# wischmcj/pyQSM

Measured on AMD Instinct MI355X. Metric: Mpoints/s DBSCAN (1M-pt synthetic forest, eps=0.1, min_neighbors=10), higher is better.
Workload: dtype f64; 1 GPU; 1000000-point synthetic tree cloud (configs[1]), DBSCAN eps=0.1 min_neighbors=10, 20 clusters; replicas at N>1; points_per_gpu=1000000, parallelism=replicas x1

## Files before the change

### include/pyqsm_hip.h

```cpp
#ifndef PYQSM_HIP_H
#define PYQSM_HIP_H

#include <stddef.h>
#include <stdint.h>

#ifdef __cplusplus
extern "C" {
#endif

#define PYQSM_OK 0
#define PYQSM_EINVAL (-1)
#define PYQSM_EHIP (-2)
#define PYQSM_ENODEV (-3)
#define PYQSM_ERANGE (-4)
#define PYQSM_ENOMEM (-5)
#define PYQSM_ENOCONV (-6)

#define PYQSM_MISS_PRIM 0xFFFFFFFFu


int pyqsm_device_count(void);
int pyqsm_init(int device);
int pyqsm_shutdown(void);
const char* pyqsm_last_error(void);
const char* pyqsm_version(void);
int pyqsm_sync(int device);
void* pyqsm_stream(int device);

int pyqsm_dev_malloc(int device, size_t bytes, void** out);
int pyqsm_dev_free(int device, void* p);
int pyqsm_h2d(int device, void* dst_dev, const void* src_host, size_t bytes);
int pyqsm_d2h(int device, void* dst_host, const void* src_dev, size_t bytes);
void pyqsm_free(void* p);
void* pyqsm_host_alloc(size_t bytes);

int pyqsm_prof_enable(int device, int on);
int pyqsm_prof_reset(int device);
int pyqsm_prof_get(int device, const char* name, double* total_ms, int64_t* launches);

int pyqsm_cast_rays(const float* verts, int64_t V, const int32_t* tris, int64_t T,
                    const float* rays, int64_t R,
                    float* t_hit, uint32_t* prim_id, float* uv, int32_t device);

int pyqsm_expand_tris_dev(const float* verts_dev, int64_t V, const int32_t* tris_dev,
                          int64_t T, float* tri12_dev, int32_t device);
int pyqsm_cast_rays_dev(const float* tri12_dev, int64_t T, const float* rays_dev, int64_t R,
                        float* t_hit_dev, uint32_t* prim_id_dev, float* uv_dev,
                        int32_t device);

int pyqsm_list_intersections(const float* verts, int64_t V, const int32_t* tris, int64_t T,
                             const float* rays, int64_t R, int32_t* counts,
                             uint32_t* ray_ids, uint32_t* prim_ids, float* t, float* uv,
                             int64_t hits_cap, int64_t* n_hits, int32_t device);

int pyqsm_point_mesh_distance(const float* verts, int64_t V, const int32_t* tris, int64_t T,
                              const float* qry, int64_t Q, float* dist, uint32_t* prim,
                              int32_t device);

int pyqsm_cast_rays_multi(const float* verts, int64_t V, const int32_t* tris, int64_t T,
                          const float* rays, int64_t R,
                          float* t_hit, uint32_t* prim_id, float* uv, int32_t n_devices);

int pyqsm_shard_bounds(int64_t n, int32_t world, int32_t rank, int64_t* begin, int64_t* end);

#define PYQSM_COMM_ID_BYTES 128
int pyqsm_comm_unique_id(uint8_t* id);
int pyqsm_comm_init_rank(const uint8_t* id, int32_t world, int32_t rank, int32_t device);
int pyqsm_comm_finalize(void);
int pyqsm_comm_info(int32_t* world, int32_t* rank, int32_t* device);
int pyqsm_comm_broadcast_dev(void* buf_dev, int64_t bytes, int32_t root);
int pyqsm_comm_all_gather_dev(const void* send_dev, void* recv_dev, int64_t bytes_per_rank);
int pyqsm_comm_all_reduce_max(double* value);

int pyqsm_dbscan(const double* xyz, int64_t n, double eps, int32_t min_pts,
                 int64_t* labels, uint8_t* is_core, int32_t device);
int pyqsm_dbscan_dev(const double* xyz_dev, int64_t n, double eps, int32_t min_pts,
                     int64_t* labels_dev, uint8_t* is_core_dev, int64_t* n_clusters,
                     int32_t device);
int pyqsm_dbscan_ex(const double* xyz, int64_t n, double eps, int32_t min_pts,
                    int32_t radius_inclusive, int64_t* labels, uint8_t* is_core, int32_t device);
int pyqsm_dbscan_dev_ex(const double* xyz_dev, int64_t n, double eps, int32_t min_pts,
                        int32_t radius_inclusive, int64_t* labels_dev, uint8_t* is_core_dev,
                        int64_t* n_clusters, int32_t device);

int pyqsm_knn(const double* xyz, int64_t n, int32_t k, int32_t exclude_self,
              int32_t* idx, double* d2, int32_t device);
int pyqsm_knn_dev(const double* xyz_dev, int64_t n, int32_t k, int32_t exclude_self,
                  int32_t* idx_dev, double* d2_dev, int32_t device);

int pyqsm_ransac(const double* pts, int64_t n, const int64_t* triples, int64_t H,
                 int32_t shape, double thresh, double center[3], double axis[3],
                 double* radius, int64_t* inliers, int64_t* n_inliers, int64_t* best,
                 int32_t device);
int pyqsm_ransac_models(const double* pts, int64_t n, const int64_t* triples, int64_t H,
                        double* models, int32_t device);
int pyqsm_ransac_count(const double* pts, int64_t n, const double* models, int64_t H,
                       int32_t shape, double thresh, int32_t* counts, int32_t device);
int pyqsm_ransac_batch(const double* pts, int64_t n, const int64_t* seg_start, int64_t n_seg,
                       const int64_t* triples, int64_t H, int32_t shape, double thresh,
                       double* centers, double* axes, double* radii, int64_t* inliers,
                       int64_t* n_inliers, int64_t* best, int32_t device);

int pyqsm_lbc_solve(const int32_t* indptr, const int32_t* indices, const double* vals,
                    int64_t n, const double* wl, const double* wh, const double* pts,
                    double rtol, int32_t max_it, double* out, int32_t* iters,
                    double* resid, int32_t device);
int pyqsm_spmv3(const int32_t* indptr, const int32_t* indices, const double* vals,
                int64_t n, const double* x, double* y, int32_t device);
int pyqsm_clamp(double* pts, int64_t n, const double lo[3], const double hi[3],
                int32_t device);

int pyqsm_ball_query(const double* xyz, int64_t n, const double center[3], double radius,
                     int64_t* out_idx, int64_t* count, int32_t device);
int pyqsm_radius_mark(const double* src, int64_t n, const double* qry, int64_t m, double radius,
                      int32_t k_cap, uint8_t* mark, int32_t* counts, int32_t device);
int pyqsm_radius_knn(const double* src, int64_t n, const double* qry, int64_t m, double radius,
                     int32_t k, int64_t* idx, double* dist, int32_t device);
int pyqsm_radius_reduce(const double* src, int64_t n, const double* qry, int64_t m, double radius, int32_t k,
                        const double* values, int32_t F, int32_t reducer, int64_t empty_row, double* out,
                        int32_t* counts, int32_t device);
int pyqsm_radius_label(const double* src, int64_t n, const double* qry, int64_t m,
                       const int32_t* qry_label, double radius, int32_t k_cap, int32_t* label,
                       int32_t* counts, int32_t device);
int pyqsm_grow_clusters(const double* src, int64_t n, const int32_t* owner_in, const double* seed_xyz,
                        const int32_t* seed_label, int64_t m, int32_t n_clusters, double radius,
                        int32_t k_cap, int32_t cycles, int32_t min_new, int32_t* owner_out,
                        int32_t* cycle_out, int32_t* finished, int64_t* stats, int32_t device);

#define PYQSM_ADJ_SAME_CLOUD 1
#define PYQSM_ADJ_WITNESS 2
#define PYQSM_ADJ_NO_CACHE 4
int pyqsm_cluster_adjacency(const double* src, const int32_t* src_label, int64_t n, int32_t n_src_labels,
                            const double* tgt, const int32_t* tgt_label, int64_t m, int32_t n_tgt_labels,
                            double threshold, int32_t flags, int64_t capacity, int32_t* a, int32_t* b,
                            double* min_d2, int64_t* pairs, int64_t* src_idx, int64_t* tgt_idx, int64_t* count,
                            int64_t* stats, int32_t device);

#define PYQSM_ALPHA_BOUNDARY 1
#define PYQSM_ALPHA_DEFAULT_MAX_TESTS 4000000000000LL
int pyqsm_alpha_area(const int32_t* ij, int64_t n, const int64_t* seg_start, int64_t n_seg, uint64_t a2,
                     int64_t max_tests, int32_t flags, int64_t* twice_area, int64_t* n_live, int64_t* n_boundary,
                     int64_t** edges, int64_t* stats, int32_t device);

int pyqsm_fps(const double* xyz, int64_t n, int64_t num_samples, int64_t start_index,
              int32_t* out_idx, int32_t device);

int pyqsm_pc_laplacian(const double* xyz, int64_t n, int32_t k, double moll,
                       int64_t* nnz, int32_t** indptr, int32_t** indices, double** vals,
                       double* mass, int32_t device);
int pyqsm_pc_laplacian_seg(const double* xyz, int64_t n, const int64_t* seg_start, int64_t n_seg,
                           int32_t k, double moll, int64_t* nnz, int32_t** indptr,
                           int32_t** indices, double** vals, double* mass, int32_t device);

int pyqsm_extract_skeleton(const double* xyz, int64_t n, const int64_t* seg_start, int64_t n_seg,
                           int32_t k, double moll, int32_t max_iter, double termination_ratio,
                           double contraction_factor, double attraction_factor,
                           double max_contraction, double max_attraction, const double* lo,
                           const double* hi, double rtol, int32_t solver_max_it, double* out_pts,
                           double* total_shift, double* steps, int32_t* n_steps,
                           int32_t* solve_iters, double* solve_resid, uint8_t* solve_ok,
                           int32_t* n_solves, int32_t device);

int pyqsm_extreme_points(const double* xyz, int64_t n, const double* dirs, int32_t n_dirs,
                         int64_t* idx, int32_t device);
int pyqsm_outside_halfspaces(const double* xyz, int64_t n, const double* eq, int32_t n_planes,
                             double margin, int64_t* idx, int64_t* count, int32_t device);

int pyqsm_mean_f64(const double* v, int64_t n, double* out);

int pyqsm_voxel_down_sample(const double* xyz, int64_t n, const double* colors, double voxel_size,
                            int64_t* m, double** out_xyz, double** out_colors, int64_t* inverse,
                            int64_t* offsets, int64_t* members, int32_t device);
int pyqsm_stat_outlier(const double* xyz, int64_t n, int32_t nb_neighbors, double std_ratio,
                       int64_t* keep, int64_t* n_keep, double* avg, double* stats, int32_t device);
int pyqsm_clean_cloud(const double* xyz, int64_t n, double voxel_size, double neighbors, double ratio,
                      int32_t iters, int64_t* m, double** out_xyz, int32_t device);

int pyqsm_estimate_normals(const double* xyz, int64_t n, double radius, int32_t max_nn,
                           const double* prev_normals, double* normals, int32_t device);
int pyqsm_orient_normals_tangent_plane(const double* xyz, int64_t n, const double* normals, int32_t k,
                                       double* oriented, int32_t* rounds, int32_t device);
int pyqsm_stem_cloud(const double* xyz, int64_t n, const double* prev_normals, double crop_offset,
                     double radius, int32_t max_nn, int32_t orient_k, double angle_cutoff,
                     int64_t* keep, double* normals, int64_t* m, int32_t device);

#define PYQSM_KMEANS_MAX_K 8
#define PYQSM_KMEANS_MAX_Q 4
#define PYQSM_SILHOUETTE_MAX_K 65536
int pyqsm_kmeans(const double* xyz, int64_t m, int32_t k, int32_t iters, const double* init,
                 double* centroids, int32_t* labels, int32_t device);
int pyqsm_silhouette(const double* xyz, int64_t m, const int32_t* labels, int32_t k, double* score,
                     int32_t* n_present, double* samples, int32_t device);
int pyqsm_kmeans_select(const double* xyz, int64_t m, int32_t k0, int32_t nk, int32_t iters,
                        const double* init, int32_t* labels, double* scores, int32_t* present,
                        int32_t device);
int pyqsm_kmeans_select_dev(const double* xyz_dev, int64_t m, int32_t k0, int32_t nk, int32_t iters,
                            const double* init, int32_t* labels, double* scores, int32_t* present,
                            int32_t device);
int pyqsm_ball_excl_dev(const double* xyz_dev, int64_t n, const uint8_t* found_dev, const double center[3],
                        double radius, int64_t* idx_dev, double* out_xyz_dev, int64_t* count,
                        int32_t device);
int pyqsm_mark_found_dev(uint8_t* found_dev, int64_t n, const int64_t* idx, int64_t cnt, int32_t device);

int pyqsm_geometric_features(const double* xyz, int64_t n, double radius, int32_t max_k, int32_t metric,
                             const int32_t* feature_ids, int32_t n_features, double* out, int32_t* counts,
                             int32_t device);
int pyqsm_smooth_values(const double* xyz, int64_t n, const double* qry, int64_t m, const double* values,
                        int32_t F, int32_t k, int32_t reducer, double* out, int32_t* idx, int32_t device);

#define PYQSM_FOREST_MAX_FEATURES 64
#define PYQSM_FOREST_MAX_CLASSES 32
#define PYQSM_FOREST_MAX_TREE_NODES 4194304u
int pyqsm_forest_create(const int64_t* tree_offsets, const int32_t* left, const int32_t* right,
                        const int32_t* feature, const double* threshold, const uint8_t* missing_left,
                        const double* value, int32_t T, int32_t C, int32_t F, int32_t device, void** forest);
int pyqsm_forest_free(void* forest);
int pyqsm_forest_info(const void* forest, int64_t info[8]);
int pyqsm_forest_stage(void* forest, int32_t staged_nodes);
int pyqsm_forest_predict(const void* forest, const float* X, int64_t n, double* proba, int32_t* label,
                         int32_t* leaves);

#define PYQSM_VOX_INVERT 1
int pyqsm_voxel_grid_create(const double* xyz, int64_t n, const double* colors, double voxel_size,
                            int32_t device, void** grid);
int pyqsm_voxel_grid_free(void* grid);
int pyqsm_voxel_grid_info(const void* grid, double origin[3], double* voxel_size, int64_t dims[3],
                          int64_t* n_voxels, int64_t* device_bytes);
int pyqsm_voxel_grid_voxels(const void* grid, int32_t* grid_index, double* colors);
int pyqsm_voxel_grid_query(const void* grid, const double* qry, int64_t m, int32_t flags,
                           uint8_t* included, int32_t* row, int64_t* idx, int64_t* count);
int pyqsm_voxel_grid_query_dev(const void* grid, const double* qry_dev, int64_t m, int32_t flags,
                               uint8_t* included_dev, int32_t* row_dev, int64_t* idx_dev, int64_t* count);

int pyqsm_skeletal_forest(const double* xyz, int64_t m, int32_t k, int32_t* edges, double* d2, int64_t* n_edges,
                          int32_t* rounds, int32_t device);
int pyqsm_skeletal_forest_dev(const double* xyz_dev, int64_t m, int32_t k, int32_t* edges_dev, double* d2_dev,
// ... 17 lines not shown
```

### pyqsm_amd/_lib.py

```python
from __future__ import annotations

import ctypes
import os

_HERE = os.path.dirname(os.path.abspath(__file__))
LIB_PATH = os.path.join(_HERE, "libpyqsm_hip.so")

i64, i32, u32, dbl = ctypes.c_int64, ctypes.c_int32, ctypes.c_uint32, ctypes.c_double
vp = ctypes.c_void_p

SIGNATURES = {
    "pyqsm_device_count": (ctypes.c_int, []),
    "pyqsm_init": (ctypes.c_int, [ctypes.c_int]),
    "pyqsm_shutdown": (ctypes.c_int, []),
    "pyqsm_last_error": (ctypes.c_char_p, []),
    "pyqsm_version": (ctypes.c_char_p, []),
    "pyqsm_sync": (ctypes.c_int, [ctypes.c_int]),
    "pyqsm_stream": (vp, [ctypes.c_int]),
    "pyqsm_dev_malloc": (ctypes.c_int, [ctypes.c_int, ctypes.c_size_t, ctypes.POINTER(vp)]),
    "pyqsm_dev_free": (ctypes.c_int, [ctypes.c_int, vp]),
    "pyqsm_h2d": (ctypes.c_int, [ctypes.c_int, vp, vp, ctypes.c_size_t]),
    "pyqsm_d2h": (ctypes.c_int, [ctypes.c_int, vp, vp, ctypes.c_size_t]),
    "pyqsm_free": (None, [vp]),
    "pyqsm_host_alloc": (vp, [ctypes.c_size_t]),
    "pyqsm_prof_enable": (ctypes.c_int, [ctypes.c_int, ctypes.c_int]),
    "pyqsm_prof_reset": (ctypes.c_int, [ctypes.c_int]),
    "pyqsm_prof_get": (ctypes.c_int, [ctypes.c_int, ctypes.c_char_p, ctypes.POINTER(dbl),
                                      ctypes.POINTER(i64)]),
    "pyqsm_cast_rays": (ctypes.c_int, [vp, i64, vp, i64, vp, i64, vp, vp, vp, i32]),
    "pyqsm_expand_tris_dev": (ctypes.c_int, [vp, i64, vp, i64, vp, i32]),
    "pyqsm_cast_rays_dev": (ctypes.c_int, [vp, i64, vp, i64, vp, vp, vp, i32]),
    "pyqsm_list_intersections": (ctypes.c_int, [vp, i64, vp, i64, vp, i64, vp, vp, vp, vp, vp,
                                                i64, ctypes.POINTER(i64), i32]),
    "pyqsm_point_mesh_distance": (ctypes.c_int, [vp, i64, vp, i64, vp, i64, vp, vp, i32]),
    "pyqsm_cast_rays_multi": (ctypes.c_int, [vp, i64, vp, i64, vp, i64, vp, vp, vp, i32]),
    "pyqsm_shard_bounds": (ctypes.c_int, [i64, i32, i32, ctypes.POINTER(i64), ctypes.POINTER(i64)]),
    "pyqsm_comm_unique_id": (ctypes.c_int, [vp]),
    "pyqsm_comm_init_rank": (ctypes.c_int, [vp, i32, i32, i32]),
    "pyqsm_comm_finalize": (ctypes.c_int, []),
    "pyqsm_comm_info": (ctypes.c_int, [ctypes.POINTER(i32), ctypes.POINTER(i32),
                                       ctypes.POINTER(i32)]),
    "pyqsm_comm_broadcast_dev": (ctypes.c_int, [vp, i64, i32]),
    "pyqsm_comm_all_gather_dev": (ctypes.c_int, [vp, vp, i64]),
    "pyqsm_comm_all_reduce_max": (ctypes.c_int, [ctypes.POINTER(dbl)]),
    "pyqsm_dbscan": (ctypes.c_int, [vp, i64, dbl, i32, vp, vp, i32]),
    "pyqsm_dbscan_dev": (ctypes.c_int, [vp, i64, dbl, i32, vp, vp, ctypes.POINTER(i64), i32]),
    "pyqsm_dbscan_ex": (ctypes.c_int, [vp, i64, dbl, i32, i32, vp, vp, i32]),
    "pyqsm_dbscan_dev_ex": (ctypes.c_int, [vp, i64, dbl, i32, i32, vp, vp, ctypes.POINTER(i64), i32]),
    "pyqsm_knn": (ctypes.c_int, [vp, i64, i32, i32, vp, vp, i32]),
    "pyqsm_knn_dev": (ctypes.c_int, [vp, i64, i32, i32, vp, vp, i32]),
    "pyqsm_ransac": (ctypes.c_int, [vp, i64, vp, i64, i32, dbl, vp, vp, ctypes.POINTER(dbl), vp,
                                    ctypes.POINTER(i64), ctypes.POINTER(i64), i32]),
    "pyqsm_ransac_models": (ctypes.c_int, [vp, i64, vp, i64, vp, i32]),
    "pyqsm_ransac_count": (ctypes.c_int, [vp, i64, vp, i64, i32, dbl, vp, i32]),
    "pyqsm_ransac_batch": (ctypes.c_int, [vp, i64, vp, i64, vp, i64, i32, dbl, vp, vp, vp, vp, vp, vp, i32]),
    "pyqsm_lbc_solve": (ctypes.c_int, [vp, vp, vp, i64, vp, vp, vp, dbl, i32, vp,
                                       ctypes.POINTER(i32), vp, i32]),
    "pyqsm_spmv3": (ctypes.c_int, [vp, vp, vp, i64, vp, vp, i32]),
    "pyqsm_clamp": (ctypes.c_int, [vp, i64, vp, vp, i32]),
    "pyqsm_ball_query": (ctypes.c_int, [vp, i64, vp, dbl, vp, ctypes.POINTER(i64), i32]),
    "pyqsm_radius_mark": (ctypes.c_int, [vp, i64, vp, i64, dbl, i32, vp, vp, i32]),
    "pyqsm_radius_label": (ctypes.c_int, [vp, i64, vp, i64, vp, dbl, i32, vp, vp, i32]),
    "pyqsm_grow_clusters": (ctypes.c_int, [vp, i64, vp, vp, vp, i64, i32, dbl, i32, i32, i32, vp, vp, vp, vp,
                                           i32]),
    "pyqsm_radius_knn": (ctypes.c_int, [vp, i64, vp, i64, dbl, i32, vp, vp, i32]),
    "pyqsm_cluster_adjacency": (ctypes.c_int, [vp, vp, i64, i32, vp, vp, i64, i32, dbl, i32, i64, vp, vp, vp, vp,
                                               vp, vp, ctypes.POINTER(i64), vp, i32]),
    "pyqsm_alpha_area": (ctypes.c_int, [vp, i64, vp, i64, ctypes.c_uint64, i64, i32, vp, vp, vp,
                                        ctypes.POINTER(vp), vp, i32]),
    "pyqsm_fps": (ctypes.c_int, [vp, i64, i64, i64, vp, i32]),
    "pyqsm_pc_laplacian": (ctypes.c_int, [vp, i64, i32, dbl, ctypes.POINTER(i64),
                                          ctypes.POINTER(vp), ctypes.POINTER(vp),
                                          ctypes.POINTER(vp), vp, i32]),
    "pyqsm_extract_skeleton": (ctypes.c_int, [vp, i64, vp, i64, i32, dbl, i32, dbl, dbl, dbl, dbl, dbl, vp, vp,
                                              dbl, i32, vp, vp, vp, vp, vp, vp, vp, ctypes.POINTER(i32), i32]),
    "pyqsm_pc_laplacian_seg": (ctypes.c_int, [vp, i64, vp, i64, i32, dbl, ctypes.POINTER(i64),
                                              ctypes.POINTER(vp), ctypes.POINTER(vp),
                                              ctypes.POINTER(vp), vp, i32]),
    "pyqsm_voxel_down_sample": (ctypes.c_int, [vp, i64, vp, dbl, ctypes.POINTER(i64), ctypes.POINTER(vp),
                                               ctypes.POINTER(vp), vp, vp, vp, i32]),
    "pyqsm_stat_outlier": (ctypes.c_int, [vp, i64, i32, dbl, vp, ctypes.POINTER(i64), vp, vp, i32]),
    "pyqsm_clean_cloud": (ctypes.c_int, [vp, i64, dbl, dbl, dbl, i32, ctypes.POINTER(i64),
                                         ctypes.POINTER(vp), i32]),
    "pyqsm_estimate_normals": (ctypes.c_int, [vp, i64, dbl, i32, vp, vp, i32]),
    "pyqsm_orient_normals_tangent_plane": (ctypes.c_int, [vp, i64, vp, i32, vp, ctypes.POINTER(i32), i32]),
    "pyqsm_stem_cloud": (ctypes.c_int, [vp, i64, vp, dbl, dbl, i32, i32, dbl, vp, vp, ctypes.POINTER(i64),
                                        i32]),
    "pyqsm_mean_f64": (ctypes.c_int, [vp, i64, ctypes.POINTER(dbl)]),
    "pyqsm_extreme_points": (ctypes.c_int, [vp, i64, vp, i32, vp, i32]),
    "pyqsm_outside_halfspaces": (ctypes.c_int, [vp, i64, vp, i32, dbl, vp, ctypes.POINTER(i64), i32]),
    "pyqsm_kmeans": (ctypes.c_int, [vp, i64, i32, i32, vp, vp, vp, i32]),
    "pyqsm_silhouette": (ctypes.c_int, [vp, i64, vp, i32, ctypes.POINTER(dbl), ctypes.POINTER(i32), vp, i32]),
    "pyqsm_kmeans_select": (ctypes.c_int, [vp, i64, i32, i32, i32, vp, vp, vp, vp, i32]),
    "pyqsm_kmeans_select_dev": (ctypes.c_int, [vp, i64, i32, i32, i32, vp, vp, vp, vp, i32]),
    "pyqsm_ball_excl_dev": (ctypes.c_int, [vp, i64, vp, vp, dbl, vp, vp, ctypes.POINTER(i64), i32]),
    "pyqsm_mark_found_dev": (ctypes.c_int, [vp, i64, vp, i64, i32]),
    "pyqsm_geometric_features": (ctypes.c_int, [vp, i64, dbl, i32, i32, vp, i32, vp, vp, i32]),
    "pyqsm_smooth_values": (ctypes.c_int, [vp, i64, vp, i64, vp, i32, i32, i32, vp, vp, i32]),
    "pyqsm_forest_create": (ctypes.c_int, [vp, vp, vp, vp, vp, vp, vp, i32, i32, i32, i32, ctypes.POINTER(vp)]),
    "pyqsm_forest_free": (ctypes.c_int, [vp]),
    "pyqsm_forest_info": (ctypes.c_int, [vp, vp]),
    "pyqsm_forest_stage": (ctypes.c_int, [vp, i32]),
    "pyqsm_forest_predict": (ctypes.c_int, [vp, vp, i64, vp, vp, vp]),
    "pyqsm_radius_reduce": (ctypes.c_int, [vp, i64, vp, i64, dbl, i32, vp, i32, i32, i64, vp, vp, i32]),
    "pyqsm_voxel_grid_create": (ctypes.c_int, [vp, i64, vp, dbl, i32, ctypes.POINTER(vp)]),
    "pyqsm_voxel_grid_free": (ctypes.c_int, [vp]),
    "pyqsm_voxel_grid_info": (ctypes.c_int, [vp, vp, ctypes.POINTER(dbl), vp, ctypes.POINTER(i64),
                                             ctypes.POINTER(i64)]),
    "pyqsm_voxel_grid_voxels": (ctypes.c_int, [vp, vp, vp]),
    "pyqsm_voxel_grid_query": (ctypes.c_int, [vp, vp, i64, i32, vp, vp, vp, ctypes.POINTER(i64)]),
    "pyqsm_voxel_grid_query_dev": (ctypes.c_int, [vp, vp, i64, i32, vp, vp, vp, ctypes.POINTER(i64)]),
    "pyqsm_skeletal_forest": (ctypes.c_int, [vp, i64, i32, vp, vp, ctypes.POINTER(i64), ctypes.POINTER(i32), i32]),
    "pyqsm_skeletal_forest_dev": (ctypes.c_int, [vp, i64, i32, vp, vp, ctypes.POINTER(i64), ctypes.POINTER(i32),
                                                 i32]),
    "pyqsm_collapse_chains": (ctypes.c_int, [vp, i64, i64, vp, vp, vp, vp, vp, i32]),
    "pyqsm_collapse_chains_dev": (ctypes.c_int, [vp, i64, i64, vp, vp, vp, vp, vp, i32]),
    "pyqsm_chain_radii": (ctypes.c_int, [vp, i64, vp, i64, vp, vp, i64, vp, i32]),
    "pyqsm_cylinder_surfaces": (ctypes.c_int, [vp, i64, vp, vp, ctypes.POINTER(vp), ctypes.POINTER(i64), i32]),
}

_lib = None


class PyQSMHipError(RuntimeError):

    def __init__(self, code: int, message: str):
        super().__init__(f"libpyqsm_hip error {code}: {message}")
        self.code = code


def load() -> ctypes.CDLL:
    global _lib
    if _lib is not None:
        return _lib
    if not os.path.exists(LIB_PATH):
        raise ImportError(
            f"{LIB_PATH} not found: the HIP library has not been built and there is no CPU "
            "fallback. Build it with `make -C pyqsm_amd/csrc`.")
    lib = ctypes.CDLL(LIB_PATH)
    for name, (res, args) in SIGNATURES.items():
        fn = getattr(lib, name)
        fn.restype = res
        fn.argtypes = args
    _lib = lib
    return lib


def check(code: int) -> None:
    if code != 0:
        msg = load().pyqsm_last_error()
        raise PyQSMHipError(code, msg.decode("utf-8", "replace") if msg else "")


def device_count() -> int:
    return int(load().pyqsm_device_count())


def logical_device_count() -> int:
    fake = os.environ.get("PYQSM_MULTI_FAKE_RANKS", "")
    return int(fake) if fake.isdigit() and int(fake) > 0 else device_count()


def physical_device(logical: int) -> int:
    fake = os.environ.get("PYQSM_MULTI_FAKE_RANKS", "")
    if fake.isdigit() and int(fake) > 0:
        return int(logical) % max(1, device_count())
    return int(logical)


def require_gpu(device: int = 0) -> None:
    check(load().pyqsm_init(int(device)))
```

### pyqsm_amd/csrc/dbscan.hip

```cpp
#include "grid.hpp"

#include <atomic>
#include <chrono>
#include <optional>
#include <vector>

namespace pyqsm {

static constexpr int kNoRoot = 0x7FFFFFFF;

__device__ __forceinline__ double sqdist(double ax, double ay, double az, double bx, double by,
                                         double bz) {
  double t0 = ax - bx, t1 = ay - by, t2 = az - bz;
  double d = t0 * t0;
  d = d + t1 * t1;
  d = d + t2 * t2;
  return d;
}


#define FOR_STENCIL(c, st, start, q, body)                         \
  for (int dz__ = -1; dz__ <= 1; ++dz__)                           \
    for (int dy__ = -1; dy__ <= 1; ++dy__) {                       \
      const int row__ = (c) + dy__ * (st).nx + dz__ * (st).nxy;    \
      const int qb__ = (start)[row__ - 1], qe__ = (start)[row__ + 2]; \
      for (int q = qb__; q < qe__; ++q) {                          \
        body                                                       \
      }                                                            \
    }

struct TileLds {
  double x[4][64], y[4][64], z[4][64];
};

static constexpr int kStragglers = 6;
static constexpr int kMaxChunks = 3;
static constexpr int kRestSegs = 64;
__device__ constexpr int kRunOrder[9] = {4, 3, 5, 1, 7, 0, 2, 6, 8};

template <class CO>
__global__ __launch_bounds__(256) void k_core_tiled(int n, const GridPlan* __restrict__ plan,
                                                    const int32_t* __restrict__ start,
                                                    const int32_t* __restrict__ cell_of, CO co, double r2,
                                                    int min_pts, uint8_t* __restrict__ core,
                                                    int32_t* __restrict__ rest,
                                                    int32_t* __restrict__ rest_cnt , int seg_cap,
                                                    int* __restrict__ parent, int* __restrict__ min_orig,
                                                    int32_t* __restrict__ flag , int max_chunks,
                                                    unsigned long long* __restrict__ tests ,
    unsigned long long* __restrict__ st ) {
  __shared__ TileLds L;
  stamped(st, [&] {
  const int lane = threadIdx.x & 63, w = __builtin_amdgcn_readfirstlane(threadIdx.x >> 6);
  const int p0 = (blockIdx.x * 4 + w) * 64;
  if (p0 >= n || !plan->ok) return;
  const Stencil st = plan_stencil(plan);
  const int ncell = plan->ncell;
  const int p = p0 + lane;
  const bool live = p < n;
  double x = 0.0, y = 0.0, z = 0.0;
  if (live) co.get(p, x, y, z);
  const Tile t = wave_tile(p0, n, st, ncell, start, cell_of);
  int cnt = 0;
  bool deferred = false;
  int chunks = 0;
  int staged = 0;
  if (t.total > kTileMax) {
    const int mycell = live ? cell_of[p] : -1;
    unsigned long long todo = __ballot(live);
    while (todo) {
      const int lead = __ffsll(todo) - 1;
      const int c = __builtin_amdgcn_readlane(mycell, lead);
      const bool mine = mycell == c;
      todo &= ~__ballot(mine);
      for (int dz = -1; dz <= 1; ++dz)
        for (int dy = -1; dy <= 1; ++dy) {
          const int row = c + dy * st.nx + dz * st.nxy;
          const int qb = __builtin_amdgcn_readfirstlane(start[row - 1]);
          const int qe = __builtin_amdgcn_readfirstlane(start[row + 2]);
          for (int base = qb; base < qe; base += 64) {
            const int q = base + lane;
            const int m = qe - base < 64 ? qe - base : 64;
            if (q < qe) co.get(q, L.x[w][lane], L.y[w][lane], L.z[w][lane]);
            __builtin_amdgcn_wave_barrier();
            staged += m;
            if (mine)
              for (int j = 0; j < m; ++j)
                cnt += sqdist(x, y, z, L.x[w][j], L.y[w][j], L.z[w][j]) <= r2;
            __builtin_amdgcn_wave_barrier();
          }
        }
    }
  } else {
#pragma unroll
    for (int ri = 0; ri < 9; ++ri) {
      const int r = kRunOrder[ri];
      for (int base = t.qb[r]; base < t.qe[r] && !deferred; base += 64) {
        const int q = base + lane;
        const int m = t.qe[r] - base < 64 ? t.qe[r] - base : 64;
        if (q < t.qe[r]) co.get(q, L.x[w][lane], L.y[w][lane], L.z[w][lane]);
        __builtin_amdgcn_wave_barrier();
        staged += m;
#pragma unroll 4
        for (int j = 0; j < m; ++j)
          cnt += sqdist(x, y, z, L.x[w][j], L.y[w][j], L.z[w][j]) <= r2;
        __builtin_amdgcn_wave_barrier();
        const unsigned long long und = __ballot(live && cnt < min_pts);
        ++chunks;
        if ((__popcll(und) <= kStragglers || chunks >= max_chunks) &&
            !(ri == 8 && base + 64 >= t.qe[r])) {
          if (und != 0) {
            int slot = 0;
            const int lead = __ffsll(und) - 1;
            const int seg = blockIdx.x % kRestSegs;
            if (lane == lead) slot = atomicAdd(rest_cnt + seg, __popcll(und));
            slot = __shfl(slot, lead, 64);
            if (live && cnt < min_pts) {
              rest[size_t(seg) * seg_cap + slot + __popcll(und & ((1ull << lane) - 1ull))] = p;
              cnt = -1;
            }
          }
          deferred = true;
          break;
        }
      }
    }
  }
  if (live && cnt >= 0) {
    core[p] = cnt >= min_pts;
    co.mark_core(p, cnt >= min_pts);
  }
  if (live) {
    parent[p] = p;
    min_orig[p] = 0x7F7F7F7F;
    flag[p] = 0;
    if (p == n - 1) flag[n] = 0;
  }
  if (tests && lane == 0) atomicAdd(tests + (blockIdx.x & 255), static_cast<unsigned long long>(staged));
  });
}

struct Runs9 {
  int qb[9];
  int pre[10];
  __device__ __forceinline__ int at(int g) const {
    int q = qb[0] + g;
#pragma unroll
    for (int r = 1; r < 9; ++r) q = g >= pre[r] ? qb[r] + (g - pre[r]) : q;
    return q;
  }
};
__device__ __forceinline__ Runs9 stencil_runs(int c, Stencil st, const int32_t* __restrict__ start) {
  Runs9 t;
  int qe[9];
#pragma unroll
  for (int r = 0; r < 9; ++r) {
    const int row = c + (kRunOrder[r] % 3 - 1) * st.nx + (kRunOrder[r] / 3 - 1) * st.nxy;
    t.qb[r] = start[row - 1];
    qe[r] = start[row + 2];
  }
  t.pre[0] = 0;
#pragma unroll
  for (int r = 0; r < 9; ++r) {
    t.qb[r] = __builtin_amdgcn_readfirstlane(t.qb[r]);
    t.pre[r + 1] = t.pre[r] + (__builtin_amdgcn_readfirstlane(qe[r]) - t.qb[r]);
  }
  return t;
}

template <class CO>
__global__ __launch_bounds__(256) void k_core_rest(const int32_t* __restrict__ rest,
                                                   const int32_t* __restrict__ rest_cnt ,
                                                   int seg_cap, const GridPlan* __restrict__ plan,
                                                   const int32_t* __restrict__ start,
                                                   const int32_t* __restrict__ cell_of, CO co, double r2,
                                                   int min_pts, uint8_t* __restrict__ core,
    unsigned long long* __restrict__ st ) {
  stamped(st, [&] {
  if (!plan->ok) return;
  const Stencil st = plan_stencil(plan);
  const int lane = threadIdx.x & 63;
  const int mine = rest_cnt[lane];
  int incl = mine;
#pragma unroll
  for (int off = 1; off < 64; off <<= 1) {
    const int v = __shfl_up(incl, off, 64);
    if (lane >= off) incl += v;
  }
  const int m = __shfl(incl, 63, 64);
  for (int i = blockIdx.x * 4 + (threadIdx.x >> 6); i < m; i += gridDim.x * 4) {
    const int seg = __popcll(__ballot(incl <= i));
    const int before = __shfl(incl - mine, seg, 64);
    const int p = rest[size_t(seg) * seg_cap + (i - before)];
    double x, y, z;
    co.get(p, x, y, z);
    const int c = __builtin_amdgcn_readfirstlane(cell_of[p]);
    const Runs9 t = stencil_runs(c, st, start);
    int cnt = 0;
    for (int g0 = 0; g0 < t.pre[9] && cnt < min_pts; g0 += 64) {
      const int g = g0 + lane;
      const bool hit = g < t.pre[9] && co.d2(t.at(g), x, y, z) <= r2;
      cnt += __popcll(__ballot(hit));
    }
    if (lane == 0) {
      core[p] = cnt >= min_pts;
      co.mark_core(p, cnt >= min_pts);
    }
  }
  });
}


__device__ __forceinline__ int ld_parent(const int* parent, int i) {
  return __hip_atomic_load(parent + i, __ATOMIC_RELAXED, __HIP_MEMORY_SCOPE_AGENT);
}
__device__ __forceinline__ void st_parent(int* parent, int i, int v) {
  __hip_atomic_store(parent + i, v, __ATOMIC_RELAXED, __HIP_MEMORY_SCOPE_AGENT);
}

__device__ __forceinline__ unsigned link_prio(int x) { return unsigned(x) * 0x9E3779B1u; }

__device__ __forceinline__ int find_root(int* parent, int x) {
  int cur = ld_parent(parent, x);
  if (cur != x) {
    int prev = x, next;
    while (cur != (next = ld_parent(parent, cur))) {
      st_parent(parent, prev, next);
      prev = cur;
      cur = next;
    }
  }
  return cur;
}

__device__ __forceinline__ void unite(int* parent, int a, int b) {
  int ra = find_root(parent, a), rb = find_root(parent, b);
  while (ra != rb) {
    if (link_prio(ra) < link_prio(rb)) {
      int t = ra;
      ra = rb;
      rb = t;
    }
    const int old = atomicCAS(parent + ra, ra, rb);
    if (old == ra) break;
    ra = find_root(parent, old);
    rb = find_root(parent, rb);
  }
}


__global__ __launch_bounds__(1024) void k_sub_rep(int n, const int32_t* __restrict__ sub_of,
                                                 const uint8_t* __restrict__ core,
                                                 const int32_t* __restrict__ order,
                                                 int* __restrict__ parent,
                                                 const int32_t* __restrict__ cell_of,
                                                 int4* __restrict__ rec,
                                                 int* __restrict__ run_min,
                                                 int4* __restrict__ list,
                                                 int32_t* __restrict__ list_cnt, const GridPlan* __restrict__ plan,
                                                 int4* __restrict__ list_xyz,
    unsigned long long* __restrict__ st ) {
  stamped(st, [&] {
  if (!plan->ok) return;
  const int nx = plan->nx, ny = plan->ny;
  const int lane = threadIdx.x & 63, w = threadIdx.x >> 6;
  const int base = blockIdx.x * 1024 + w * 64;
  const int p = base + lane;
  const bool live = p < n;
  int sid = 0, s = n, e = n, ord = 0x7FFFFFFF, cell = 0;
  bool c = false;
  const bool c_prev = base >= 64 && p - 64 < n && core[p - 64];
  const bool c_next = p + 64 < n && core[p + 64];
  const int o_next = c_next ? order[p + 64] : 0x7FFFFFFF;
  if (live) {
    sid = sub_of[p];
    c = core[p];
    if (c) ord = order[p];
    cell = cell_of[p];
    const int2 run = *reinterpret_cast<const int2*>(rec + sid);
    s = run.x;
    e = run.x + run.y;
  }
  const unsigned long long cb = __ballot(c);
  int lead = -1;
  const int s0 = __shfl(s, 0, 64);
  if (s0 < base && s0 >= base - 64) {
    const unsigned long long f = __ballot(c_prev && base - 64 + lane >= s0);
    if (f) lead = base - 64 + __ffsll(f) - 1;
  } else {
    for (int q0 = s0; q0 < base; q0 += 64) {
      const int q = q0 + lane;
      const unsigned long long f = __ballot(q < base && core[q]);
      if (f) {
        lead = q0 + __ffsll(f) - 1;
        break;
      }
    }
  }
  int rep = -1;
  if (c) {
    if (s < base && lead >= 0) {
      rep = lead;
    } else {
      const int lo = s > base ? s - base : 0;
      rep = base + __ffsll(cb & (~0ull << lo)) - 1;
    }
    parent[p] = rep;
  }
  const bool is_rep = c && rep == p;
  int mn = ord;
  const int seg_end = e - base < 64 ? e - base : 64;
#pragma unroll
  for (int off = 1; off < 64; off <<= 1) {
    const int o = __shfl_down(mn, off, 64);
    if (lane + off < seg_end) mn = o < mn ? o : mn;
  }
  const unsigned long long tail = __ballot(is_rep && e > base + 64);
  if (tail) {
    const int t = __ffsll(tail) - 1;
    const int et = __shfl(e, t, 64);
    int m2 = base + 64 + lane < et ? o_next : 0x7FFFFFFF;
    for (int q = base + 128 + lane; q < et; q += 64)
      if (core[q]) m2 = min(m2, order[q]);
#pragma unroll
    for (int off = 32; off > 0; off >>= 1) {
      const int o = __shfl_xor(m2, off, 64);
      m2 = o < m2 ? o : m2;
    }
    if (lane == t) mn = min(mn, m2);
  }
  if (is_rep) {
    rec[sid].z = rep;
    run_min[rep] = mn;
  }
  __shared__ int wcount[16], wbase[16];
  const unsigned long long b = __ballot(is_rep);
  if (lane == 0) wcount[w] = __popcll(b);
  __syncthreads();
  if (threadIdx.x == 0) {
    int tot = 0;
    for (int k = 0; k < 16; ++k) tot += wcount[k];
    int base2 = tot ? atomicAdd(list_cnt, tot) : 0;
    for (int k = 0; k < 16; ++k) {
      wbase[k] = base2;
      base2 += wcount[k];
    }
  }
  __syncthreads();
  if (is_rep) {
    const int slot = wbase[w] + __popcll(b & ((1ull << lane) - 1ull));
    const int c1 = cell;
    list[slot] = make_int4(rep, c1, sid, e - rep);
    list_xyz[slot] = make_int4(c1 % nx, (c1 / nx) % ny, c1 / (nx * ny), sid & 7);
  }
  });
}

__constant__ signed char kSubOffsets[62][3] = {{1,0,0}, {-1,1,0}, {0,1,0}, {1,1,0}, {-1,-1,1}, {0,-1,1}, {1,-1,1}, {-1,0,1}, {0,0,1}, {1,0,1}, {-1,1,1}, {0,1,1}, {1,1,1}, {2,0,0}, {-2,1,0}, {2,1,0}, {-2,2,0}, {-1,2,0}, {0,2,0}, {1,2,0}, {2,2,0}, {-2,-2,1}, {-1,-2,1}, {0,-2,1}, {1,-2,1}, {2,-2,1}, {-2,-1,1}, {2,-1,1}, {-2,0,1}, {2,0,1}, {-2,1,1}, {2,1,1}, {-2,2,1}, {-1,2,1}, {0,2,1}, {1,2,1}, {2,2,1}, {-2,-2,2}, {-1,-2,2}, {0,-2,2}, {1,-2,2}, {2,-2,2}, {-2,-1,2}, {-1,-1,2}, {0,-1,2}, {1,-1,2}, {2,-1,2}, {-2,0,2}, {-1,0,2}, {0,0,2}, {1,0,2}, {2,0,2}, {-2,1,2}, {-1,1,2}, {0,1,2}, {1,1,2}, {2,1,2}, {-2,2,2}, {-1,2,2}, {0,2,2}, {1,2,2}, {2,2,2}};

__global__ __launch_bounds__(256) void k_flatten_reps(const int4* __restrict__ list,
                                                      const int32_t* __restrict__ m_ptr,
                                                      int* __restrict__ parent, int max_steps,
                                                      int4* __restrict__ rec ) {
  const int m = *m_ptr;
  int s = blockIdx.x * 256 + threadIdx.x;
  if (s >= m) return;
  const int4 me = list[s];
  const int p = me.x;
  int r = p, steps = 0;
  for (int nx = parent[r]; nx != r && steps < max_steps; nx = parent[r], ++steps) r = nx;
  parent[p] = r;
  if (rec) {
    int* const word = reinterpret_cast<int*>(rec + (me.z & ~7)) + 3;
    const int old = atomicCAS(word, 0, r + 1);
    if (old != 0 && old != r + 1 && old != -1) *word = -1;
  }
}

static constexpr int kSubPerWave = 4;

struct SubNbr {
  int q0, n2, rep;
};
__device__ __forceinline__ SubNbr sub_neighbour(bool active, const int4 at, int dx, int dy, int dz, int nx, int ny,
                                                const int32_t* __restrict__ start,
                                                const int4* __restrict__ rec) {
  const int gx = 2 * (at.x - 1) + (at.w & 1) - dx, gy = 2 * (at.y - 1) + ((at.w >> 1) & 1) - dy,
            gz = 2 * (at.z - 1) + ((at.w >> 2) & 1) - dz;
  const int c2 = (((gz >> 1) + 1) * ny + ((gy >> 1) + 1)) * nx + ((gx >> 1) + 1);
  const int oct = (gx & 1) | ((gy & 1) << 1) | ((gz & 1) << 2);
  SubNbr out{0, 0, -1};
  int b2 = 0, e2 = 0;
  if (active) {
    b2 = start[c2];
    e2 = start[c2 + 1];
  }
  if (e2 != b2) {
    const int4 r = rec[b2 * 8 + oct];
    if (r.y > 0) {
      out.q0 = r.x;
      out.n2 = r.y;
      out.rep = r.z;
    }
  }
  return out;
}

template <class CO>
__global__ __launch_bounds__(256) void k_hook_sub(const int4* __restrict__ list,
                                                  const int4* __restrict__ list_xyz,
                                                  const int32_t* __restrict__ m_ptr,
                                                  const GridPlan* __restrict__ plan, const int32_t* __restrict__ start,
                                                  const int4* __restrict__ rec, CO co, double r2,
                                                  const uint8_t* __restrict__ core,
                                                  int* __restrict__ parent,
    unsigned long long* __restrict__ st ) {
  stamped(st, [&] {
  if (!plan->ok) return;
  const int nx = plan->nx, ny = plan->ny;
  const int m = *m_ptr;
  const int k = threadIdx.x & 63;
  const int t = k & 15, grp = k >> 4;
  const int o_dx = t < 13 ? kSubOffsets[t][0] : 0, o_dy = t < 13 ? kSubOffsets[t][1] : 0,
            o_dz = t < 13 ? kSubOffsets[t][2] : 0;
  for (int s0 = (blockIdx.x * 4 + (threadIdx.x >> 6)) * kSubPerWave; s0 < m; s0 += gridDim.x * 4 * kSubPerWave) {
    const bool live = s0 + grp < m;
    const int4 me = list[min(s0 + grp, m - 1)], at = list_xyz[min(s0 + grp, m - 1)];
    const SubNbr nb2 = sub_neighbour(live && t < 13, at, o_dx, o_dy, o_dz, nx, ny, start, rec);
    const int p = me.x, n1 = me.w;
    unsigned todo = unsigned(__ballot(nb2.rep >= 0) >> (16 * grp)) & 0xFFFFu;
    int base = 0, hooked = -1;
    while (__ballot(todo != 0)) {
      const int src = (k & 48) + (todo ? __ffs(todo) - 1 : 0);
      const int qb = __shfl(nb2.q0, src, 64), nb = __shfl(nb2.n2, src, 64), rb = __shfl(nb2.rep, src, 64);
      const int sh = nb > 1 ? 32 - __clz(nb - 1) : 0;
      const int pairs = n1 << sh;
      const int idx = base + t;
      const int j = idx & ((1 << sh) - 1);
      bool hit = false;
      if (todo && idx < pairs && j < nb) hit = co.core_pair_within(p + (idx >> sh), qb + j, core, r2);
      const bool found = ((__ballot(hit) >> (16 * grp)) & 0xFFFFull) != 0;
      if (found) {
        hooked = rb;
        todo = 0;
      } else if (todo) {
        base += 16;
        if (base >= pairs) {
          todo &= todo - 1;
          base = 0;
        }
      }
    }
    if (hooked >= 0 && t == 0) parent[p] = parent[hooked];
  }
  });
}

template <class CO>
__device__ __forceinline__ bool wave_pair_within(const CO& co, int p, int n1, int qb, int nb, int k,
                                                 const uint8_t* __restrict__ core, double r2) {
  const int sh = nb > 1 ? 32 - __clz(nb - 1) : 0;
  const int pairs = n1 << sh;
  bool found = false;
  for (int base = 0; base < pairs && !found; base += 64) {
    const int idx = base + k;
    const int j = idx & ((1 << sh) - 1);
    bool hit = false;
    if (idx < pairs && j < nb) hit = co.core_pair_within(p + (idx >> sh), qb + j, core, r2);
    found = __ballot(hit) != 0;
  }
  return found;
}

template <class CO>
__device__ __forceinline__ void seam_unite(const int4 me, const int4 at, int k, int o_dx, int o_dy, int o_dz,
                                           int nx, int ny, const int32_t* __restrict__ start,
                                           const int4* __restrict__ rec, const CO& co, double r2,
                                           const uint8_t* __restrict__ core, int* parent) {
  const SubNbr nb2 = sub_neighbour(k < 62, at, o_dx, o_dy, o_dz, nx, ny, start, rec);
  const int p = me.x, n1 = me.w, rep2 = nb2.rep;
  const int* vparent = parent;
  int a1 = 0, a2 = 0;
  if (rep2 >= 0) {
    a1 = vparent[p];
    a2 = vparent[rep2];
  }
  bool need = rep2 >= 0 && !(a1 == a2 || a2 == p || a1 == rep2);
  int root2 = -1;
  if (need) {
    int ra = a1, rb = a2;
    for (;;) {
      const int pa = ld_parent(parent, ra), pb = ld_parent(parent, rb);
      if (pa == ra && pb == rb) break;
      ra = pa;
      rb = pb;
    }
    need = ra != rb;
    root2 = rb;
  }
  unsigned long long todo = __ballot(need);
  while (todo) {
    const int src = __ffsll(todo) - 1;
    todo &= todo - 1;
    const int qb = __shfl(nb2.q0, src, 64), nb = __shfl(nb2.n2, src, 64), rb = __shfl(rep2, src, 64);
    const int tree = __shfl(root2, src, 64);
    if (wave_pair_within(co, p, n1, qb, nb, k, core, r2)) {
      if (k == 0) unite(parent, p, rb);
      todo &= ~__ballot(root2 == tree);
    }
  }
}

template <class CO>
__global__ __launch_bounds__(256) void k_union_sub(const int4* __restrict__ list,
                                                   const int4* __restrict__ list_xyz,
                                                   const int32_t* __restrict__ m_ptr,
                                                   const GridPlan* __restrict__ plan, const int32_t* __restrict__ start,
                                                   const int4* __restrict__ rec, CO co, double r2,
                                                   const uint8_t* __restrict__ core, int* parent,
                                                   unsigned long long* __restrict__ seam_cnt ,
    unsigned long long* __restrict__ st ) {
  stamped(st, [&] {
  if (!plan->ok) return;
  const int nx = plan->nx, ny = plan->ny;
  const int m = *m_ptr;
  const int k = threadIdx.x & 63;
  const int t = k & 15, grp = k >> 4;
  const int o_dx = k < 62 ? kSubOffsets[k][0] : 0, o_dy = k < 62 ? kSubOffsets[k][1] : 0,
            o_dz = k < 62 ? kSubOffsets[k][2] : 0;
  const int c_off = t < 9 ? (t % 3 - 1) + (t / 3 - 1) * nx : 0;
  const int layer = nx * ny;
  for (int s0 = (blockIdx.x * 4 + (threadIdx.x >> 6)) * kSubPerWave; s0 < m; s0 += gridDim.x * 4 * kSubPerWave) {
    const bool live = s0 + grp < m;
    const int4 me = list[min(s0 + grp, m - 1)];
    const int* vparent = parent;
    const int r_s = vparent[me.x];
    const int c2 = me.y + c_off;
    int b2[2] = {0, 0}, e2[2] = {0, 0}, word[2] = {0, 0};
    if (live && t < 9) {
#pragma unroll
      for (int l = 0; l < 2; ++l) {
        b2[l] = start[c2 - l * layer];
        e2[l] = start[c2 - l * layer + 1];
      }
    }
#pragma unroll
    for (int l = 0; l < 2; ++l)
      if (e2[l] != b2[l]) word[l] = rec[b2[l] * 8].w;
    const unsigned long long seams =
        __ballot((word[0] != 0 && word[0] != r_s + 1) || (word[1] != 0 && word[1] != r_s + 1));
    if (!seams) continue;
    for (int u = 0; u < kSubPerWave; ++u) {
      if (!((seams >> (16 * u)) & 0xFFFFull)) continue;
      if (seam_cnt && k == 0) atomicAdd(seam_cnt, 1ull);
      seam_unite(list[s0 + u], list_xyz[s0 + u], k, o_dx, o_dy, o_dz, nx, ny, start, rec, co, r2, core, parent);
    }
  }
  });
}

template <class CO>
__global__ __launch_bounds__(256) void k_union_points(int n, Stencil st,
                                                      const int32_t* __restrict__ start,
                                                      const int32_t* __restrict__ cell_of, CO co, double r2,
                                                      const uint8_t* __restrict__ core, int* parent) {
  int p = blockIdx.x * 256 + threadIdx.x;
  if (p >= n || !core[p]) return;
  double x, y, z;
  co.get(p, x, y, z);
  const int c = cell_of[p];
  const volatile int* vparent = parent;
  int rp = find_root(parent, p);
  FOR_STENCIL(c, st, start, q, {
    if (q < p && core[q] && co.d2(q, x, y, z) <= r2) {
      if (vparent[q] != rp) {
        unite(parent, p, q);
        rp = find_root(parent, p);
      }
    }
  })
}

__global__ __launch_bounds__(256) void k_flatten(int n, const uint8_t* __restrict__ core,
                                                 int* __restrict__ parent, const GridPlan* __restrict__ plan) {
  int p = blockIdx.x * 256 + threadIdx.x;
  if (!plan->ok || p >= n || !core[p]) return;
  int r = p;
  for (int nx = parent[r]; nx != r; nx = parent[r]) r = nx;
  parent[p] = r;
}

template <int kThreads>
__device__ __forceinline__ void block_append(bool take, int value, int32_t* __restrict__ list,
                                             int32_t* __restrict__ cnt) {
  constexpr int kWaves = kThreads / 64;
  __shared__ int wcount[kWaves], wbase[kWaves];
  const unsigned long long b = __ballot(take);
  const int lane = threadIdx.x & 63, w = threadIdx.x >> 6;
  if (lane == 0) wcount[w] = __popcll(b);
  __syncthreads();
  if (threadIdx.x == 0) {
    int tot = 0;
    for (int k = 0; k < kWaves; ++k) tot += wcount[k];
    int base = tot ? atomicAdd(cnt, tot) : 0;
    for (int k = 0; k < kWaves; ++k) {
      wbase[k] = base;
      base += wcount[k];
    }
  }
  __syncthreads();
  if (take) list[wbase[w] + __popcll(b & ((1ull << lane) - 1ull))] = value;
}

static constexpr int kFlagsThreads = 256, kFlagsPer = 16, kFlagsPerBlock = kFlagsThreads * kFlagsPer;
__device__ __forceinline__ void flags_role(int b, int n, const uint8_t* __restrict__ core,
                                           int32_t* __restrict__ rest, int32_t* __restrict__ rest_cnt) {
  constexpr int kWaves = kFlagsThreads / 64;
  __shared__ int fcount[kWaves], fbase[kWaves];
  const int lane = threadIdx.x & 63, w = threadIdx.x >> 6;
  const int p0 = b * kFlagsPerBlock + threadIdx.x;
  unsigned take = 0;
#pragma unroll
  for (int k = 0; k < kFlagsPer; ++k) {
    const int p = p0 + k * kFlagsThreads;
    take |= unsigned(p < n && !core[p]) << k;
  }
  int mine = __popc(take);
#pragma unroll
  for (int off = 32; off > 0; off >>= 1) mine += __shfl_xor(mine, off, 64);
  if (lane == 0) fcount[w] = mine;
  __syncthreads();
  if (threadIdx.x == 0) {
    int tot = 0;
    for (int k = 0; k < kWaves; ++k) tot += fcount[k];
    int base = tot ? atomicAdd(rest_cnt, tot) : 0;
    for (int k = 0; k < kWaves; ++k) {
      fbase[k] = base;
      base += fcount[k];
    }
  }
  __syncthreads();
  int at = fbase[w];
#pragma unroll
  for (int k = 0; k < kFlagsPer; ++k) {
    const bool t = (take >> k) & 1u;
    const unsigned long long bal = __ballot(t);
    if (t) rest[at + __popcll(bal & ((1ull << lane) - 1ull))] = p0 + k * kFlagsThreads;
    at += __popcll(bal);
  }
}

__global__ __launch_bounds__(kFlagsThreads) void k_noncore_list(int n, const uint8_t* __restrict__ core,
                                                                int32_t* __restrict__ rest,
                                                                int32_t* __restrict__ rest_cnt,
                                                                const GridPlan* __restrict__ plan) {
  if (!plan->ok) return;
  flags_role(blockIdx.x, n, core, rest, rest_cnt);
}

__global__ __launch_bounds__(256) void k_point_min(int n, const uint8_t* __restrict__ core,
                                                   const int* __restrict__ parent,
                                                   const int32_t* __restrict__ order,
                                                   int* __restrict__ min_orig,
                                                   int32_t* __restrict__ roots,
                                                   int32_t* __restrict__ roots_cnt,
                                                   const GridPlan* __restrict__ plan) {
  int p = blockIdx.x * 256 + threadIdx.x;
  const bool is_c = plan->ok && p < n && core[p];
  if (is_c) atomicMin(min_orig + parent[p], order[p]);
  block_append<256>(is_c && parent[p] == p, p, roots, roots_cnt);
}

static constexpr int kRepRootThreads = kFlagsThreads;
static_assert(kRepRootThreads == 256, "gl, the grid of the representatives' blocks, is cut in 256s");
__global__ __launch_bounds__(kRepRootThreads) void k_rep_root(const int4* __restrict__ list,
                                                  const int32_t* __restrict__ m_ptr,
                                                  int* __restrict__ parent,
                                                  const int* __restrict__ run_min,
                                                  int* __restrict__ min_orig,
                                                  int32_t* __restrict__ roots,
                                                  int32_t* __restrict__ roots_cnt, int rep_blocks, int n,
                                                  const uint8_t* __restrict__ core, int32_t* __restrict__ rest,
                                                  int32_t* __restrict__ rest_cnt,
                                                  const GridPlan* __restrict__ plan) {
  if (int(blockIdx.x) >= rep_blocks) {
    if (plan->ok) flags_role(blockIdx.x - rep_blocks, n, core, rest, rest_cnt);
    return;
  }
  const int m = *m_ptr;
  int s = blockIdx.x * kRepRootThreads + threadIdx.x;
  const bool active = s < m;
  int p = -1, r = -1, v = 0x7FFFFFFF;
  if (active) {
    p = list[s].x;
    r = p;
    for (int nx = parent[r]; nx != r; nx = parent[r]) r = nx;
    if (r != p) parent[p] = r;
    v = run_min[p];
  }
  const volatile int* vmin = min_orig;
  const int lane = threadIdx.x & 63;
  unsigned long long rem = __ballot(active);
  while (rem) {
    const int lead = __ffsll(rem) - 1;
    const int r0 = __shfl(r, lead, 64);
    const bool mine = active && r == r0;
    int mn = mine ? v : 0x7FFFFFFF;
#pragma unroll
    for (int off = 32; off > 0; off >>= 1) {
      const int o = __shfl_xor(mn, off, 64);
      mn = o < mn ? o : mn;
    }
    if (lane == lead && mn < vmin[r0]) atomicMin(min_orig + r0, mn);
    rem &= ~__ballot(mine);
  }
  block_append<256>(active && r == p, p, roots, roots_cnt);
}

static constexpr int kRankCap = 4096;
static constexpr int kNumberThreads = 1024;

__global__ __launch_bounds__(kNumberThreads) void k_number(int n, const int32_t* __restrict__ roots,
                                                           const int32_t* __restrict__ roots_cnt,
                                                           int* __restrict__ min_orig,
                                                           uint32_t* __restrict__ bits ,
                                                           int32_t* __restrict__ wpre ,
                                                           int32_t* __restrict__ done ,
                                                           const GridPlan* __restrict__ plan,
    unsigned long long* __restrict__ st ) {
  stamped(st, [&] {
  if (!plan->ok) return;
  const int R = *roots_cnt;
  const int t = threadIdx.x;
  if (R <= kRankCap) {
    if (blockIdx.x != 0) return;
    __shared__ unsigned long long key[kRankCap];
    int P = 2;
    while (P < R) P <<= 1;
    for (int i = t; i < P; i += kNumberThreads) {
      unsigned long long k = ~0ull;
      if (i < R) {
        const int r = roots[i];
        k = (static_cast<unsigned long long>(min_orig[r]) << 32) | static_cast<uint32_t>(r);
      }
      key[i] = k;
    }
    __syncthreads();
    for (int k = 2; k <= P; k <<= 1)
      for (int j = k >> 1; j > 0; j >>= 1) {
        for (int i = t; i < P; i += kNumberThreads) {
          const int l = i ^ j;
          if (l > i) {
            const unsigned long long a = key[i], b = key[l];
            if ((a > b) == ((i & k) == 0)) {
              key[i] = b;
              key[l] = a;
            }
          }
        }
        __syncthreads();
      }
    for (int i = t; i < R; i += kNumberThreads) min_orig[static_cast<uint32_t>(key[i])] = i;
    return;
  }
  for (int i = blockIdx.x * kNumberThreads + t; i < R; i += gridDim.x * kNumberThreads) {
    const int v = min_orig[roots[i]];
    __hip_atomic_fetch_or(bits + (v >> 5), 1u << (v & 31), __ATOMIC_RELAXED, __HIP_MEMORY_SCOPE_AGENT);
  }
  __shared__ int last;
  __threadfence();
  __syncthreads();
  if (t == 0) last = atomicAdd(done, 1) == int(gridDim.x) - 1;
  __syncthreads();
  if (!last) return;
  __threadfence();
  __shared__ int wsum[kNumberThreads / 64];
  const int lane = t & 63, wv = t >> 6;
  const int nw = n / 32 + 1;
  int carry = 0;
  for (int w0 = 0; w0 < nw; w0 += 16 * kNumberThreads) {
    const int i0 = w0 + 16 * t;
    int cnt[16], sum = 0;
#pragma unroll
    for (int k = 0; k < 16; ++k) {
      cnt[k] = i0 + k < nw ? __popc(__hip_atomic_load(bits + i0 + k, __ATOMIC_RELAXED, __HIP_MEMORY_SCOPE_AGENT)) : 0;
      sum += cnt[k];
    }
    int incl = sum;
#pragma unroll
    for (int off = 1; off < 64; off <<= 1) {
      const int o = __shfl_up(incl, off, 64);
      if (lane >= off) incl += o;
    }
    if (lane == 63) wsum[wv] = incl;
    __syncthreads();
    int before = carry, total = 0;
    for (int k = 0; k < kNumberThreads / 64; ++k) {
      before += k < wv ? wsum[k] : 0;
      total += wsum[k];
    }
    int run = before + incl - sum;
#pragma unroll
    for (int k = 0; k < 16; ++k)
      if (i0 + k < nw) {
        wpre[i0 + k] = run;
        run += cnt[k];
      }
    carry += total;
    __syncthreads();
  }
  });
}

__device__ __forceinline__ int cluster_number(int v, int n_roots, const uint32_t* __restrict__ bits,
                                              const int32_t* __restrict__ wpre) {
  if (n_roots <= kRankCap) return v;
  return wpre[v >> 5] + __popc(bits[v >> 5] & ((1u << (v & 31)) - 1u));
}

static constexpr int kLabelThreads = 256;
template <class CO>
__global__ __launch_bounds__(kLabelThreads) void k_labels(int n, const int32_t* __restrict__ rest,
                                                          const int32_t* __restrict__ rest_cnt,
                                                          const GridPlan* __restrict__ plan,
                                                          const int32_t* __restrict__ start,
                                                          const int32_t* __restrict__ cell_of, CO co, double r2,
                                                          const uint8_t* __restrict__ core,
                                                          const int* __restrict__ parent,
                                                          const int* __restrict__ min_orig,
                                                          const int32_t* __restrict__ roots_cnt,
                                                          const uint32_t* __restrict__ bits,
                                                          const int32_t* __restrict__ wpre,
                                                          const int32_t* __restrict__ order,
                                                          int64_t* __restrict__ labels,
                                                          uint8_t* __restrict__ is_core,
    unsigned long long* __restrict__ st ) {
  stamped(st, [&] {
  if (!plan->ok) return;
  constexpr int kWaves = kLabelThreads / 64;
  const int n_roots = *roots_cnt;
  const int lane = threadIdx.x & 63;
  {
    const int p = blockIdx.x * kLabelThreads + threadIdx.x;
    const bool is_c = p < n && core[p];
    if (is_c) {
      const int v = min_orig[parent[parent[p]]];
      labels[order[p]] = int64_t(cluster_number(v, n_roots, bits, wpre));
    }
    if (p < n && is_core) is_core[order[p]] = is_c;
  }
  const int m = *rest_cnt;
  const Stencil sten = plan_stencil(plan);
  const int first = blockIdx.x * kWaves + __builtin_amdgcn_readfirstlane(threadIdx.x >> 6);
  for (int i = first; i < m; i += gridDim.x * kWaves) {
    const int p = rest[i];
    double x, y, z;
    co.get(p, x, y, z);
    const int c = __builtin_amdgcn_readfirstlane(cell_of[p]);
    const Runs9 t = stencil_runs(c, sten, start);
    int best = kNoRoot;
    for (int g0 = 0; g0 < t.pre[9]; g0 += 64) {
      const int g = g0 + lane;
      if (g < t.pre[9]) {
        const int q = t.at(g);
        if (core[q] && co.d2(q, x, y, z) <= r2) {
          const int mo = min_orig[parent[parent[q]]];
          best = mo < best ? mo : best;
        }
      }
    }
#pragma unroll
    for (int off = 32; off > 0; off >>= 1) {
      const int o = __shfl_xor(best, off, 64);
      best = o < best ? o : best;
    }
    if (lane == 0)
      labels[order[p]] = best == kNoRoot ? int64_t(-1) : int64_t(cluster_number(best, n_roots, bits, wpre));
  }
  });
}

static int cluster_binned(Ctx* c, int64_t n, double eps, int32_t min_pts, bool radius_inclusive, const DevGrid& g,
                          const SubCells& sub, const GridPlan* d_plan, int64_t* labels, uint8_t* is_core,
                          const int32_t** count_out) {
  const bool fine = g.cell <= eps * (1.0 + 1.0 / 524288.0);
  const int N = int(n);
  const dim3 grid(ceil_div(n, 256)), block(256);
  const Stencil st{g.nx, g.nx * g.ny};
  const double r2 = radius_inclusive ? eps * eps : nextafter(eps * eps, 0.0);
  uint8_t* core;
  int *parent, *min_orig;
  int32_t* flag;
  PQ_TRY(c->arena.get(size_t(n), &core));
  PQ_TRY(c->arena.get(size_t(n), &parent));
  PQ_TRY(c->arena.get(size_t(n), &min_orig));
  PQ_TRY(c->arena.get(size_t(n) + 1, &flag));
  uint32_t* const bits = reinterpret_cast<uint32_t*>(flag);
  int32_t *roots, *wpre;
  PQ_TRY(c->arena.get(size_t(n), &roots));
  PQ_TRY(c->arena.get(size_t(n / 32) + 1, &wpre));
  int4* list;
  int32_t* list_cnt;
  int* run_min;
  PQ_TRY(c->arena.get(size_t(n), &run_min));
  PQ_TRY(c->arena.get(size_t(n), &list));
  int4* list_xyz;
  PQ_TRY(c->arena.get(size_t(n), &list_xyz));
  list_cnt = sub.zeroed4;
  int32_t* const roots_cnt = list_cnt + 1;
  int32_t* rest;
  const int core_blocks = int(ceil_div(n, 256));
  const int seg_cap = ceil_div(core_blocks, kRestSegs) * 256;
  PQ_TRY(c->arena.get(std::max<size_t>(size_t(n), size_t(seg_cap) * kRestSegs), &rest));
  int32_t* const rest_segs = list_cnt + 4;
  {
    StampScope ps(c, "dbscan_core");
    unsigned long long* d_tests = nullptr;
    if (c->prof >= 2) {
      PQ_TRY(c->arena.get(256, &d_tests));
      PQ_HIP(hipMemsetAsync(d_tests, 0, 256 * 8, c->stream));
    }
    const int max_chunks = std::min(32, std::max(kMaxChunks, (kMaxChunks * min_pts + 9) / 10));
    {
      const StampKernel pk(c, "k_core_tiled", grid.x);
      on_coords(g, [&](auto co) {
        hipLaunchKernelGGL(k_core_tiled<decltype(co)>, grid, block, 0, c->stream, N, d_plan, g.start, g.cell_of, co, r2,
                           min_pts, core, rest, rest_segs, seg_cap, parent, min_orig, flag, max_chunks, d_tests,
                           pk.slots);
      });
    }
    if (d_tests) {
      unsigned long long h[256];
      PQ_HIP(hipMemcpyAsync(h, d_tests, sizeof(h), hipMemcpyDeviceToHost, c->stream));
      PQ_HIP(hipStreamSynchronize(c->stream));
      unsigned long long tot = 0;
      for (unsigned long long v : h) tot += v;
      c->timers["core_pair_tests"].launches += int64_t(tot) * 64;
    }
    const dim3 gr(std::min<int64_t>(8192, ceil_div(n, 64)));
    unsigned long long* const st_rest = stamp_slots(c, gr.x);
    on_coords(g, [&](auto co) {
      hipLaunchKernelGGL(k_core_rest<decltype(co)>, gr, block, 0, c->stream, rest, rest_segs, seg_cap, d_plan, g.start,
                         g.cell_of, co, r2, min_pts, core, st_rest);
    });
    PQ_HIP(hipGetLastError());
    if (getenv("PYQSM_DBSCAN_TRACE")) {
      int32_t h[kRestSegs];
      PQ_HIP(hipMemcpyAsync(h, rest_segs, sizeof(h), hipMemcpyDeviceToHost, c->stream));
      PQ_HIP(hipStreamSynchronize(c->stream));
      long long tot = 0;
      for (int32_t v : h) tot += v;
      fprintf(stderr, "core pass: %lld stragglers\n", tot);
    }
  }
  {
    StampScope ps(c, "dbscan_union");
    const dim3 gf(ceil_div(n, kFlagsPerBlock));
    if (fine) {
      hipLaunchKernelGGL(k_sub_rep, dim3(ceil_div(n, 1024)), dim3(1024), 0, c->stream, N, sub.sub_of, core,
                         g.order, parent, g.cell_of, sub.rec, run_min, list, list_cnt, d_plan, list_xyz,
                         stamp_slots(c, ceil_div(n, 1024)));
      {
        int per_cu[2] = {16, 32};
        if (const char* e_cu = getenv("PYQSM_UNION_BLOCKS_PER_CU")) {
          per_cu[0] = per_cu[1] = atoi(e_cu);
          if (const char* comma = strchr(e_cu, ',')) per_cu[1] = atoi(comma + 1);
        }
        const int64_t full = ceil_div(n, 4 * kSubPerWave);
        const dim3 gh(per_cu[0] > 0 ? std::min<int64_t>(full, int64_t(c->cu_count) * per_cu[0]) : full),
            gu(per_cu[1] > 0 ? std::min<int64_t>(full, int64_t(c->cu_count) * per_cu[1]) : full),
            gl(ceil_div(n, 256));
        const bool trace = getenv("PYQSM_DBSCAN_TRACE") != nullptr;
        {
          const StampKernel pk(c, "k_hook_sub", gh.x);
          on_coords(g, [&](auto co) {
            hipLaunchKernelGGL(k_hook_sub<decltype(co)>, gh, block, 0, c->stream, list, list_xyz, list_cnt, d_plan,
                               g.start, sub.rec, co, r2, core, parent, pk.slots);
          });
        }
        if (trace) {
          int32_t m = 0;
          PQ_HIP(hipMemcpyAsync(&m, list_cnt, 4, hipMemcpyDeviceToHost, c->stream));
          PQ_HIP(hipStreamSynchronize(c->stream));
          std::vector<int32_t> hp(static_cast<size_t>(n), 0);
          std::vector<int4> hl(static_cast<size_t>(m), make_int4(0, 0, 0, 0));
          PQ_HIP(hipMemcpy(hp.data(), parent, size_t(n) * 4, hipMemcpyDeviceToHost));
          PQ_HIP(hipMemcpy(hl.data(), list, size_t(m) * 16, hipMemcpyDeviceToHost));
          std::vector<int64_t> hist(66, 0);
          int64_t roots = 0;
          for (int32_t s2 = 0; s2 < m; ++s2) {
            int d = 0, r = hl[size_t(s2)].x;
            while (hp[size_t(r)] != r && d < 65) {
              r = hp[size_t(r)];
              ++d;
            }
            hist[size_t(d)]++;
            roots += d == 0;
          }
          fprintf(stderr, "hook pass: %d sub-cells, %lld roots; chain depth histogram:", m, (long long)roots);
          for (int d = 0; d < 66; ++d)
            if (hist[size_t(d)]) fprintf(stderr, " %d:%lld", d, (long long)hist[size_t(d)]);
          fprintf(stderr, "\n");
        }
        static const int jump = [] {
          const char* e = getenv("PYQSM_FLATTEN_JUMP");
          return e ? atoi(e) : 12;
        }();
        if (jump > 0)
          hipLaunchKernelGGL(k_flatten_reps, gl, block, 0, c->stream, list, list_cnt, parent, jump,
                             static_cast<int4*>(nullptr));
        hipLaunchKernelGGL(k_flatten_reps, gl, block, 0, c->stream, list, list_cnt, parent, 0x7fffffff, sub.rec);
        unsigned long long* d_seams = nullptr;
        if (trace) {
          PQ_TRY(c->arena.get(1, &d_seams));
          PQ_HIP(hipMemsetAsync(d_seams, 0, 8, c->stream));
        }
        {
          const StampKernel pk(c, "k_union_sub", gu.x);
          on_coords(g, [&](auto co) {
            hipLaunchKernelGGL(k_union_sub<decltype(co)>, gu, block, 0, c->stream, list, list_xyz, list_cnt, d_plan,
                               g.start, sub.rec, co, r2, core, parent, d_seams, pk.slots);
          });
        }
        if (trace) {
          unsigned long long h = 0;
          PQ_HIP(hipMemcpyAsync(&h, d_seams, 8, hipMemcpyDeviceToHost, c->stream));
          PQ_HIP(hipStreamSynchronize(c->stream));
          fprintf(stderr, "seam union: %llu sub-cells took the 62-offset path\n", h);
        }
        hipLaunchKernelGGL(k_rep_root, dim3(gl.x + gf.x), dim3(kRepRootThreads), 0, c->stream, list, list_cnt, parent,
                           run_min, min_orig, roots, roots_cnt, int(gl.x), N, core, rest, list_cnt + 3, d_plan);
      }
      PQ_HIP(hipGetLastError());
    } else {
      PQ_TRY(stamp_mark(c));
      on_coords(g, [&](auto co) {
        hipLaunchKernelGGL(k_union_points<decltype(co)>, grid, block, 0, c->stream, N, st, g.start, g.cell_of, co,
                           r2, core, parent);
      });
      hipLaunchKernelGGL(k_flatten, grid, block, 0, c->stream, N, core, parent, d_plan);
      hipLaunchKernelGGL(k_point_min, grid, block, 0, c->stream, N, core, parent, g.order, min_orig, roots,
                         roots_cnt, d_plan);
      hipLaunchKernelGGL(k_noncore_list, gf, dim3(kFlagsThreads), 0, c->stream, N, core, rest,
                         list_cnt + 3, d_plan);
    }
    const dim3 gn(std::min<int64_t>(ceil_div(n, kNumberThreads), c->cu_count));
    hipLaunchKernelGGL(k_number, gn, dim3(kNumberThreads), 0, c->stream, N, roots, roots_cnt, min_orig, bits, wpre,
                       list_cnt + 2, d_plan, stamp_slots(c, gn.x));
    PQ_HIP(hipGetLastError());
  }
  {
    StampScope ps(c, "dbscan_label");
    const dim3 gb(ceil_div(n, kLabelThreads));
    unsigned long long* const st_labels = stamp_slots(c, gb.x);
    on_coords(g, [&](auto co) {
      hipLaunchKernelGGL(k_labels<decltype(co)>, gb, dim3(kLabelThreads), 0, c->stream, N, rest, list_cnt + 3, d_plan,
                         g.start, g.cell_of, co, r2, core, parent, min_orig, roots_cnt, bits, wpre, g.order, labels,
                         is_core, st_labels);
    });
    PQ_HIP(hipGetLastError());
    if (getenv("PYQSM_DBSCAN_TRACE")) {
      int32_t h = 0;
      PQ_HIP(hipMemcpyAsync(&h, list_cnt + 3, 4, hipMemcpyDeviceToHost, c->stream));
      PQ_HIP(hipStreamSynchronize(c->stream));
      fprintf(stderr, "label pass: %d non-core points listed\n", h);
    }
  }
  *count_out = roots_cnt;
  return 0;
}


static constexpr double kPlanPollMs = 20.0;
static int wait_plan(Ctx* c, const GridPlan* h_plan, unsigned seq) {
  const volatile unsigned* const s = &h_plan->seq;
  const auto t0 = std::chrono::steady_clock::now();
  while (*s != seq) {
    if (std::chrono::duration<double, std::milli>(std::chrono::steady_clock::now() - t0).count() > kPlanPollMs) {
      PQ_HIP(hipStreamSynchronize(c->stream));
      if (*s != seq) return fail(PYQSM_EHIP, "DBSCAN: the grid plan was not written (sequence %u)", seq);
      break;
    }
  }
  std::atomic_thread_fence(std::memory_order_acquire);
  return 0;
}

static int dbscan_device(Ctx* c, const double* xyz, int64_t n, double eps, int32_t min_pts,
                         bool radius_inclusive, int64_t* labels, uint8_t* is_core, int64_t* n_clusters) {
  if (!(eps > 0) || !std::isfinite(eps)) return fail(PYQSM_EINVAL, "eps must be positive");
  if (n == 0) {
    if (n_clusters) *n_clusters = 0;
    return 0;
  }
  const double cell = eps * (1.0 + 1.0 / 1048576.0);
  const int64_t max_cells = int64_t(1) << 28;
  if (!c->plan_pinned) {
    PQ_HIP(hipHostMalloc(&c->plan_pinned, 2 * sizeof(GridPlan), hipHostMallocMapped | hipHostMallocCoherent));
    memset(c->plan_pinned, 0, 2 * sizeof(GridPlan));
  }
  GridPlan* const h_plan = static_cast<GridPlan*>(c->plan_pinned);
  GridPlan* h_plan_dev;
  PQ_HIP(hipHostGetDevicePointer(reinterpret_cast<void**>(&h_plan_dev), c->plan_pinned, 0));
  if (++c->plan_seq == 0) c->plan_seq = 1;
  const unsigned seq = c->plan_seq;
  GridPlan* d_plan;
  int32_t* zeroed;
  PQ_TRY(c->arena.get(2, &d_plan));
  PQ_TRY(c->arena.get(size_t(octant_zeroed_ints()), &zeroed));
  const char* plan_env = getenv("PYQSM_DBSCAN_PLAN");
  const char* bin_env = getenv("PYQSM_DBSCAN_BIN");
  const char* f32_env = getenv("PYQSM_COORD_F32");
  const bool speculate = c->plan_hint.valid && !(plan_env && !strcmp(plan_env, "host")) && !bin_env &&
                         !(f32_env && !strcmp(f32_env, "0")) && n <= (int64_t(1) << 25);
  const PlanHint hint = speculate ? c->plan_hint : PlanHint{};
  DevGrid g;
  SubCells sub;
  const int32_t* count = nullptr;
  std::optional<StampScope> bin_scope(std::in_place, c, "dbscan_bin");
  PQ_TRY(plan_grid_device(c, xyz, n, cell, max_cells, hint, d_plan, h_plan_dev, seq, zeroed, octant_zeroed_ints()));
  const Arena::Mark mark = c->arena.mark();
  if (speculate) {
    PQ_TRY(bin_octants_planned(c, xyz, n, cell, hint, d_plan, zeroed, &g, &sub));
    bin_scope.reset();
    PQ_TRY(cluster_binned(c, n, eps, min_pts, radius_inclusive, g, sub, d_plan, labels, is_core, &count));
  }
  PQ_TRY(wait_plan(c, h_plan, seq));
  const bool hit = speculate && h_plan[0].ok;
  if (!hit) {
    c->arena.rewind(mark);
    PlanHint next;
    if (!bin_scope) bin_scope.emplace(c, "dbscan_bin");
    PQ_TRY(stamp_mark(c));
    PQ_TRY(bin_octants_host(c, xyz, n, cell, max_cells, h_plan[0], zeroed, &h_plan[1], d_plan + 1, &g, &sub, &next));
    PQ_TRY(stamp_mark(c));
    bin_scope.reset();
    if (next.valid) c->plan_hint = next;
    PQ_TRY(cluster_binned(c, n, eps, min_pts, radius_inclusive, g, sub, d_plan + 1, labels, is_core, &count));
  }
  if (c->prof >= 1) {
    c->timers["dbscan_f32_records"].launches += g.p4 ? 1 : 0;
    c->timers[hit ? "dbscan_plan_hit" : "dbscan_plan_miss"].launches += 1;
  }
  if (n_clusters) {
    int32_t h = 0;
    PQ_HIP(hipMemcpyAsync(&h, count, 4, hipMemcpyDeviceToHost, c->stream));
    PQ_HIP(hipStreamSynchronize(c->stream));
    *n_clusters = h;
  }
  return 0;
}

}

using namespace pyqsm;

extern "C" {

int pyqsm_dbscan_dev_ex(const double* xyz_dev, int64_t n, double eps, int32_t min_pts,
                        int32_t radius_inclusive, int64_t* labels_dev, uint8_t* is_core_dev,
                        int64_t* n_clusters, int32_t device) {
  PQ_API_RANGE("pyqsm_dbscan_dev");
  if (n < 0) return fail(PYQSM_EINVAL, "negative size");
  if (n > 0 && (!xyz_dev || !labels_dev)) return fail(PYQSM_EINVAL, "pyqsm_dbscan_dev: NULL pointer");
  Ctx* c = ctx_for(device);
  if (!c) return PYQSM_ENODEV;
  std::lock_guard<std::mutex> lk(c->mu);
  c->arena.reset();
  StampScope ps(c, "dbscan_total");
  return dbscan_device(c, xyz_dev, n, eps, min_pts, radius_inclusive != 0, labels_dev, is_core_dev,
                       n_clusters);
}

int pyqsm_dbscan_dev(const double* xyz_dev, int64_t n, double eps, int32_t min_pts,
                     int64_t* labels_dev, uint8_t* is_core_dev, int64_t* n_clusters,
                     int32_t device) {
  return pyqsm_dbscan_dev_ex(xyz_dev, n, eps, min_pts, 1, labels_dev, is_core_dev, n_clusters, device);
}

int pyqsm_dbscan(const double* xyz, int64_t n, double eps, int32_t min_pts, int64_t* labels,
                 uint8_t* is_core, int32_t device) {
  return pyqsm_dbscan_ex(xyz, n, eps, min_pts, 1, labels, is_core, device);
}

int pyqsm_dbscan_ex(const double* xyz, int64_t n, double eps, int32_t min_pts, int32_t radius_inclusive,
                    int64_t* labels, uint8_t* is_core, int32_t device) {
  PQ_API_RANGE("pyqsm_dbscan");
  if (n < 0) return fail(PYQSM_EINVAL, "negative size");
  if (n == 0) return 0;
  if (!xyz || !labels) return fail(PYQSM_EINVAL, "pyqsm_dbscan: NULL pointer");
  Ctx* c = ctx_for(device);
  if (!c) return PYQSM_ENODEV;
  std::lock_guard<std::mutex> lk(c->mu);
  c->arena.reset();
  double* d_xyz;
  int64_t* d_lab;
  uint8_t* d_core;
  PQ_TRY(c->arena.get(size_t(n) * 3, &d_xyz));
  PQ_TRY(c->arena.get(size_t(n), &d_lab));
  PQ_TRY(c->arena.get(size_t(n), &d_core));
  PQ_HIP(hipMemcpyAsync(d_xyz, xyz, size_t(n) * 24, hipMemcpyHostToDevice, c->stream));
  PQ_TRY(dbscan_device(c, d_xyz, n, eps, min_pts, radius_inclusive != 0, d_lab, d_core, nullptr));
  PQ_HIP(hipMemcpyAsync(labels, d_lab, size_t(n) * 8, hipMemcpyDeviceToHost, c->stream));
  if (is_core) PQ_HIP(hipMemcpyAsync(is_core, d_core, size_t(n), hipMemcpyDeviceToHost, c->stream));
  PQ_HIP(hipStreamSynchronize(c->stream));
  return 0;
}

}
```

### pyqsm_amd/csrc/grid.hip

```cpp
#include "grid.hpp"

#include <atomic>
#include <cmath>
#include <type_traits>

namespace pyqsm {

__device__ __forceinline__ unsigned long long ord_key(double x) {
  unsigned long long b = static_cast<unsigned long long>(__double_as_longlong(x));
  return (b >> 63) ? ~b : (b | 0x8000000000000000ull);
}
static double ord_val(unsigned long long k) {
  unsigned long long b = (k >> 63) ? (k & 0x7FFFFFFFFFFFFFFFull) : ~k;
  double d;
  memcpy(&d, &b, 8);
  return d;
}

static constexpr int kBoxVals = 7;
__global__ __launch_bounds__(256) void k_bbox(const double* __restrict__ xyz, int64_t n,
                                              unsigned long long* __restrict__ part ,
    unsigned long long* __restrict__ st ) {
  __shared__ unsigned long long red[4][6];
  __shared__ int red_f32[4];
// ... 773 lines not shown
  __shared__ int32_t wsum[16];
  if (plan) {
    if (!plan->ok) return;
    nbk = plan->nbk;
  }
  const int per = (nbk + 1023) / 1024;
  const int b0 = threadIdx.x * per;
  int32_t v[16], s = 0;
  for (int k = 0; k < per; ++k) {
    v[k] = b0 + k < nbk ? tot[b0 + k] : 0;
    s += v[k];
  }
  const int lane = threadIdx.x & 63, w = threadIdx.x >> 6;
  int32_t incl = s;
#pragma unroll
  for (int off = 1; off < 64; off <<= 1) {
    const int32_t t = __shfl_up(incl, off, 64);
    if (lane >= off) incl += t;
  }
  if (lane == 63) wsum[w] = incl;
  __syncthreads();
  int32_t run = incl - s;
  for (int q = 0; q < w; ++q) run += wsum[q];
  for (int k = 0; k < per; ++k) {
    if (b0 + k < nbk) bstart[b0 + k] = run;
    run += v[k];
  }
  if (threadIdx.x == 1023) bstart[nbk] = run;
}

template <bool F32>
__global__ __launch_bounds__(256) void k_bk_scatter(const double* __restrict__ xyz, int64_t n, int nbk,
                                                    int bits, const int32_t* __restrict__ key_tmp,
                                                    const int32_t* __restrict__ tot,
                                                    int32_t* __restrict__ cursor ,
                                                    int32_t* __restrict__ bstart ,
                                                    int fused,
                                                    typename BkRec<F32>::type* __restrict__ bucketed,
                                                    int32_t* __restrict__ keyb ,
                                                    const GridPlan* __restrict__ plan) {
  extern __shared__ __attribute__((aligned(16))) int32_t h[];
  const int64_t base = int64_t(blockIdx.x) * kBkPts;
  using Coord = typename std::conditional<F32, float, double>::type;
  int key[kBkPts / 256], lr[kBkPts / 256];
  Coord px[kBkPts / 256], py[kBkPts / 256], pz[kBkPts / 256];
#pragma unroll
  for (int k = 0; k < kBkPts / 256; ++k) {
    const int64_t i = base + k * 256 + threadIdx.x;
    key[k] = -1;
    px[k] = py[k] = pz[k] = Coord(0);
    if (i < n) {
      key[k] = key_tmp[i];
      px[k] = Coord(xyz[3 * i]);
      py[k] = Coord(xyz[3 * i + 1]);
      pz[k] = Coord(xyz[3 * i + 2]);
    }
  }
  if (plan) {
    if (!plan->ok) return;
    nbk = plan->nbk;
    bits = plan->bits;
  }
  int32_t* pre = h + nbk;
  __shared__ int32_t wsum[4];
  for (int b = threadIdx.x; b < nbk; b += 256) h[b] = 0;
  if (fused) {
    constexpr int kPer = kBkFusedScan / 256;
    const int b0 = threadIdx.x * kPer;
    int32_t v[kPer], s = 0;
#pragma unroll
    for (int k = 0; k < kPer; ++k) {
      v[k] = b0 + k < nbk ? tot[b0 + k] : 0;
      s += v[k];
    }
    const int lane = threadIdx.x & 63, w = threadIdx.x >> 6;
    int32_t incl = s;
#pragma unroll
    for (int off = 1; off < 64; off <<= 1) {
      const int32_t t = __shfl_up(incl, off, 64);
      if (lane >= off) incl += t;
    }
    if (lane == 63) wsum[w] = incl;
    __syncthreads();
    int32_t run = incl - s;
    for (int q = 0; q < w; ++q) run += wsum[q];
#pragma unroll
    for (int k = 0; k < kPer; ++k) {
      if (b0 + k < nbk) {
        pre[b0 + k] = run;
        if (blockIdx.x == 0) bstart[b0 + k] = run;
      }
      run += v[k];
    }
    if (blockIdx.x == 0 && threadIdx.x == 255) bstart[nbk] = run;
  }
  __syncthreads();
#pragma unroll
  for (int k = 0; k < kBkPts / 256; ++k) {
    lr[k] = key[k] >= 0 ? atomicAdd(&h[key[k] >> (3 + bits)], 1) : 0;
  }
  __syncthreads();
  for (int bb = 0; bb < nbk; bb += 16 * 256) {
    int32_t v[16], a[16];
#pragma unroll
    for (int k = 0; k < 16; ++k) {
      const int b = bb + k * 256 + threadIdx.x;
      v[k] = b < nbk ? h[b] : 0;
    }
#pragma unroll
    for (int k = 0; k < 16; ++k) {
      a[k] = 0;
      if (v[k]) a[k] = atomicAdd(&cursor[bb + k * 256 + threadIdx.x], v[k]);
    }
#pragma unroll
    for (int k = 0; k < 16; ++k) {
      const int b = bb + k * 256 + threadIdx.x;
      if (v[k]) h[b] = (fused ? pre[b] : bstart[b]) + a[k];
    }
  }
  __syncthreads();
#pragma unroll
  for (int k = 0; k < kBkPts / 256; ++k) {
    if (key[k] < 0) continue;
    const int64_t i = base + k * 256 + threadIdx.x;
    const int pos = h[key[k] >> (3 + bits)] + lr[k];
    keyb[pos] = key[k];
    if constexpr (F32) {
      bucketed[pos] = make_float4(px[k], py[k], pz[k], __int_as_float(int(i)));
    } else {
      PointRec r;
      r.x = px[k];
      r.y = py[k];
      r.z = pz[k];
      r.idx = int(i);
      r.key = key[k];
      bucketed[pos] = r;
    }
  }
}

__device__ __forceinline__ int bytes_below(unsigned long long x, int o) {
  x &= (1ull << (8 * o)) - 1ull;
  x = (x & 0x00FF00FF00FF00FFull) + ((x >> 8) & 0x00FF00FF00FF00FFull);
  x = (x & 0x0000FFFF0000FFFFull) + ((x >> 16) & 0x0000FFFF0000FFFFull);
  return int((x + (x >> 32)) & 0xFFFFull);
}

template <int BITS>
struct BkLds {
  unsigned long long oct[1 << BITS];
  int32_t cnt[1 << BITS];
  uint32_t big[(1 << BITS) / 32];
  int32_t wsum[16];
  int32_t any_big;
  int32_t btot[8], bbase[8];
  int32_t bw[(1 << BITS) / 512][8];
};

__device__ __forceinline__ uint32_t bk_word(int lk, int rr, int r8) {
  return (uint32_t(lk) << 16) | (uint32_t(rr < 255 ? rr : 255) << 8) | uint32_t(r8);
}

template <bool F32>
static constexpr int kBkGrp = F32 ? 2 : 1;

template <int BITS, bool F32>
__global__ __launch_bounds__((1 << BITS) / 8, BITS == 12 ? 6 : 4) void k_bk_sort(
    int64_t ncell1 , const int32_t* __restrict__ bstart,
    const typename BkRec<F32>::type* __restrict__ bucketed, const int32_t* __restrict__ keyb,
    uint32_t* __restrict__ word_tmp, int32_t* __restrict__ rank_tmp, int32_t* __restrict__ start,
    int32_t* __restrict__ order, int32_t* __restrict__ cell_of, int32_t* __restrict__ sub_of,
    double* __restrict__ sx, double* __restrict__ sy, double* __restrict__ sz,
    float4* __restrict__ p4 , int4* __restrict__ rec,
    PointRec* __restrict__ keyed ,
    const GridPlan* __restrict__ plan ,
    unsigned long long* __restrict__ st ) {
  constexpr int CELLS = 1 << BITS, T = CELLS / 8, CAP = T * kBkPer, G = kBkGrp<F32>;
  using Rec = typename BkRec<F32>::type;
  static_assert(kBkPer % G == 0, "whole groups");
  __shared__ BkLds<BITS> L;
  stamped(st, [&] {
  const int bk = blockIdx.x, t = threadIdx.x;
  if (!plan->ok || bk >= plan->nbk) return;
  ncell1 = int64_t(plan->ncell) + 1;
  const int s = bstart[bk], e = bstart[bk + 1];
  const int64_t c0 = int64_t(bk) << BITS;
  if (s == e) {
#pragma unroll
    for (int k = 0; k < 2; ++k) {
      const int64_t cidx = c0 + int64_t(k * T + t) * 4;
      if (cidx + 3 < ncell1) {
        *reinterpret_cast<int4*>(start + cidx) = make_int4(s, s, s, s);
      } else {
        for (int u = 0; u < 4; ++u)
          if (cidx + u < ncell1) start[cidx + u] = s;
      }
    }
    return;
  }
  if (e - s <= 64) {
    int32_t* const cells = L.cnt;
    const int m = e - s;
    if (t < 64) {
      const bool live = t < m;
      const int lk = live ? keyb[s + t] & (8 * CELLS - 1) : 0;
      Rec p = {};
      if (live) p = bucketed[s + t];
      int below_key = 0, below_cell = 0;
      unsigned long long oc = 0ull;
      for (int q = 0; q < m; ++q) {
        const int kq = __builtin_amdgcn_readlane(lk, q);
        below_key += (kq < lk || (kq == lk && q < t)) ? 1 : 0;
        below_cell += (kq >> 3) < (lk >> 3) ? 1 : 0;
        if ((kq >> 3) == (lk >> 3)) oc += 1ull << (8 * (kq & 7));
      }
      if (live) {
        const int cl = lk >> 3, o = lk & 7, b = s + below_cell, f = s + below_key;
        cells[t] = cl;
        cell_of[f] = int(c0) + cl;
        sub_of[f] = b * 8 + o;
        if constexpr (F32) {
          order[f] = __float_as_int(p.w);
          p4[f] = make_float4(p.x, p.y, p.z, 0.f);
        } else {
          order[f] = p.idx;
          sx[f] = p.x;
          sy[f] = p.y;
          sz[f] = p.z;
        }
        if (below_key == below_cell) {
          int r2 = b;
#pragma unroll
          for (int o2 = 0; o2 < 8; ++o2) {
            const int cnt = int((oc >> (8 * o2)) & 255ull);
            rec[size_t(b) * 8 + o2] = make_int4(r2, cnt, -1, 0);
            r2 += cnt;
          }
        }
      }
    }
    __syncthreads();
    int32_t pre[8] = {s, s, s, s, s, s, s, s};
    for (int q = 0; q < m; ++q) {
      const int d = cells[q] - 8 * t;
#pragma unroll
      for (int k = 0; k < 8; ++k) pre[k] += d < k ? 1 : 0;
    }
    const int64_t cidx = c0 + 8 * t;
    if (cidx + 7 < ncell1) {
      *reinterpret_cast<int4*>(start + cidx) = make_int4(pre[0], pre[1], pre[2], pre[3]);
      *reinterpret_cast<int4*>(start + cidx + 4) = make_int4(pre[4], pre[5], pre[6], pre[7]);
    } else {
#pragma unroll
      for (int k = 0; k < 8; ++k)
        if (cidx + k < ncell1) start[cidx + k] = pre[k];
    }
    return;
  }
  uint32_t wd[kBkPer];
#pragma unroll
  for (int k = 0; k < kBkPer; ++k) {
    const int j = s + k * T + t;
    wd[k] = j < e ? uint32_t(keyb[j]) : 0u;
  }
  Rec cur[G] = {};
#pragma unroll
  for (int k = 0; k < G; ++k) {
    const int j = s + k * T + t;
    if (j < e) cur[k] = bucketed[j];
  }
#pragma unroll
  for (int k = 0; k < 8; ++k) {
    L.oct[k * T + t] = 0ull;
    L.cnt[k * T + t] = 0;
  }
  if (t < CELLS / 32) L.big[t] = 0u;
  if (t == 0) L.any_big = 0;
  __syncthreads();
  auto rank_of = [&](uint32_t ky, int j) {
    const int lk = int(ky) & (8 * CELLS - 1), cl = lk >> 3, o = lk & 7;
    const int rr = atomicAdd(&L.cnt[cl], 1);
    const int r8 = int((atomicAdd(&L.oct[cl], 1ull << (8 * o)) >> (8 * o)) & 255ull);
    if (rr >= 255) rank_tmp[j] = rr;
    return bk_word(lk, rr, r8);
  };
#pragma unroll
  for (int k = 0; k < kBkPer; ++k) {
    const int j = s + k * T + t;
    if (j < e) wd[k] = rank_of(wd[k], j);
  }
  for (int base = s + CAP; base < e; base += CAP) {
    uint32_t kk[kBkPer];
#pragma unroll
    for (int k = 0; k < kBkPer; ++k) {
      const int j = base + k * T + t;
      kk[k] = j < e ? uint32_t(keyb[j]) : 0u;
    }
#pragma unroll
    for (int k = 0; k < kBkPer; ++k) {
      const int j = base + k * T + t;
      if (j < e) word_tmp[j] = rank_of(kk[k], j);
    }
  }
  __syncthreads();
  int32_t v[8], tot = 0;
  {
    const int4 a = *reinterpret_cast<const int4*>(&L.cnt[8 * t]);
    const int4 b = *reinterpret_cast<const int4*>(&L.cnt[8 * t + 4]);
    v[0] = a.x; v[1] = a.y; v[2] = a.z; v[3] = a.w;
    v[4] = b.x; v[5] = b.y; v[6] = b.z; v[7] = b.w;
#pragma unroll
    for (int k = 0; k < 8; ++k) tot += v[k];
  }
  const int lane = t & 63, w = t >> 6;
  int32_t incl = tot;
#pragma unroll
  for (int off = 1; off < 64; off <<= 1) {
    const int32_t u = __shfl_up(incl, off, 64);
    if (lane >= off) incl += u;
  }
  if (lane == 63) L.wsum[w] = incl;
  __syncthreads();
  int32_t run = incl - tot;
  for (int q = 0; q < w; ++q) run += L.wsum[q];
  int32_t pre[8];
#pragma unroll
  for (int k = 0; k < 8; ++k) {
    pre[k] = run;
    run += v[k];
  }
  {
    const int64_t cidx = c0 + 8 * t;
    if (cidx + 7 < ncell1) {
      *reinterpret_cast<int4*>(start + cidx) = make_int4(s + pre[0], s + pre[1], s + pre[2], s + pre[3]);
      *reinterpret_cast<int4*>(start + cidx + 4) = make_int4(s + pre[4], s + pre[5], s + pre[6], s + pre[7]);
    } else {
#pragma unroll
      for (int k = 0; k < 8; ++k)
        if (cidx + k < ncell1) start[cidx + k] = s + pre[k];
    }
  }
#pragma unroll
  for (int k = 0; k < 8; ++k) {
    const int cl = 8 * t + k;
    L.cnt[cl] = pre[k];
    if (v[k] == 0) continue;
    const int b = s + pre[k];
    if (v[k] > kBkBig) {
      atomicOr(&L.big[cl >> 5], 1u << (cl & 31));
      L.any_big = 1;
      continue;
    }
    const unsigned long long c64 = L.oct[cl];
    int r2 = b;
#pragma unroll
    for (int o = 0; o < 8; ++o) {
      const int cnt = int((c64 >> (8 * o)) & 255ull);
      rec[size_t(b) * 8 + o] = make_int4(r2, cnt, -1, 0);
      r2 += cnt;
    }
  }
  __syncthreads();
  auto place = [&](const Rec& p, uint32_t w, int j) {
    const int lk = int(w >> 16), cl = lk >> 3, o = lk & 7, arr = int((w >> 8) & 255u);
    const int b = s + L.cnt[cl];
    if ((L.big[cl >> 5] >> (cl & 31)) & 1u) {
      PointRec q;
      q.x = p.x;
      q.y = p.y;
      q.z = p.z;
      q.key = int(c0 << 3) + lk;
      if constexpr (F32)
        q.idx = __float_as_int(p.w);
      else
        q.idx = p.idx;
      keyed[b + (arr < 255 ? arr : rank_tmp[j])] = q;
      return;
    }
    const int f = b + bytes_below(L.oct[cl], o) + int(w & 255u);
    cell_of[f] = int(c0) + cl;
    sub_of[f] = b * 8 + o;
    if constexpr (F32) {
      order[f] = __float_as_int(p.w);
      p4[f] = make_float4(p.x, p.y, p.z, 0.f);
    } else {
      order[f] = p.idx;
      sx[f] = p.x;
      sy[f] = p.y;
      sz[f] = p.z;
    }
  };
#pragma unroll
  for (int g = 0; g < kBkPer / G; ++g) {
    if (s + g * G * T >= e) break;
    Rec nxt[G] = {};
    if (g + 1 < kBkPer / G) {
#pragma unroll
      for (int k = 0; k < G; ++k) {
        const int j = s + ((g + 1) * G + k) * T + t;
        if (j < e) nxt[k] = bucketed[j];
      }
    }
#pragma unroll
    for (int k = 0; k < G; ++k) {
      const int j = s + (g * G + k) * T + t;
      if (j < e) place(cur[k], wd[g * G + k], j);
    }
#pragma unroll
    for (int k = 0; k < G; ++k) cur[k] = nxt[k];
  }
  for (int base = s + CAP; base < e; base += CAP) {
#pragma unroll
    for (int g = 0; g < kBkPer / G; ++g) {
      if (base + g * G * T >= e) break;
      Rec r[G] = {};
      uint32_t w[G];
#pragma unroll
      for (int k = 0; k < G; ++k) {
        const int j = base + (g * G + k) * T + t;
        w[k] = 0u;
        if (j < e) {
          r[k] = bucketed[j];
          w[k] = word_tmp[j];
        }
      }
#pragma unroll
      for (int k = 0; k < G; ++k) {
        const int j = base + (g * G + k) * T + t;
        if (j < e) place(r[k], w[k], j);
      }
    }
  }
  __syncthreads();
  if (!L.any_big) return;
  for (int wd = 0; wd < CELLS / 32; ++wd) {
    for (uint32_t bm = L.big[wd]; bm; bm &= bm - 1u) {
      const int cl = wd * 32 + __ffs(bm) - 1;
      const int b = s + L.cnt[cl], e2 = s + (cl + 1 < CELLS ? L.cnt[cl + 1] : e - s);
      int loc[8] = {0, 0, 0, 0, 0, 0, 0, 0};
      for (int q = b + t; q < e2; q += T) {
        const int oq = keyed[q].key & 7;
#pragma unroll
        for (int k = 0; k < 8; ++k) loc[k] += oq == k;
      }
      if (t < 8) L.btot[t] = 0;
      __syncthreads();
#pragma unroll
      for (int k = 0; k < 8; ++k) {
        int cnt = loc[k];
        for (int off = 32; off > 0; off >>= 1) cnt += __shfl_down(cnt, off, 64);
        if (lane == 0 && cnt) atomicAdd(&L.btot[k], cnt);
      }
      __syncthreads();
      if (t == 0) {
        int r2 = b;
        for (int k = 0; k < 8; ++k) {
          L.bbase[k] = r2;
          rec[size_t(b) * 8 + k] = make_int4(r2, L.btot[k], -1, 0);
          r2 += L.btot[k];
        }
      }
      __syncthreads();
      for (int q0 = b; q0 < e2; q0 += T) {
        const int q = q0 + t;
        const bool live = q < e2;
        PointRec pr;
        pr.key = 0;
        if (live) pr = keyed[q];
        const int o = pr.key & 7;
        int before = 0;
#pragma unroll
        for (int k = 0; k < 8; ++k) {
          const unsigned long long m = __ballot(live && o == k);
          if (lane == 0) L.bw[w][k] = __popcll(m);
          if (o == k) before = __popcll(m & ((1ull << lane) - 1ull));
        }
        __syncthreads();
        if (live) {
          int f = L.bbase[o] + before;
          for (int ww = 0; ww < w; ++ww) f += L.bw[ww][o];
          order[f] = pr.idx;
          cell_of[f] = pr.key >> 3;
          sub_of[f] = b * 8 + o;
          if (p4) {
            p4[f] = make_float4(float(pr.x), float(pr.y), float(pr.z), 0.f);
          } else {
            sx[f] = pr.x;
            sy[f] = pr.y;
            sz[f] = pr.z;
          }
        }
        __syncthreads();
        if (t < 8) {
          int add = 0;
          for (int ww = 0; ww < T / 64; ++ww) add += L.bw[ww][t];
          L.bbase[t] += add;
        }
        __syncthreads();
      }
    }
// ... 180 lines not shown
}

static bool bucketed_fits(const DevGrid& g) {
  const int bits = g.ncell + 1 <= (int64_t(kBkMax) << 12) ? 12 : 13;
  const int64_t nbk = (g.ncell + (int64_t(1) << bits)) >> bits;
  const char* env = getenv("PYQSM_GRID_BIN");
  return nbk <= kBkMax && !(env && !strcmp(env, "atomic"));
}

static void enqueue_bk_a(Ctx* c, int mode, bool f32, const double* xyz, int64_t n, const GridParams& gp,
                         const int raw[3], AxisMap am, int64_t nbk, int bits, int32_t* key_tmp, int32_t* tot,
                         int32_t* cursor, int32_t* bstart, void* bucketed, int32_t* keyb, const GridPlan* d_plan) {
  const dim3 ga(ceil_div(n, kBkPts)), blk(256);
  const size_t lds = size_t(nbk) * 4;
  const int fused = nbk <= kBkFusedScan;
#define PQ_BK_HIST(MODE)                                                                                         \
  hipLaunchKernelGGL(k_bk_hist<MODE>, ga, blk, lds, c->stream, xyz, n, gp, raw[0], raw[1], raw[2], am, int(nbk), \
                     bits, key_tmp, tot, d_plan)
  if (mode == 0)
    PQ_BK_HIST(0);
  else if (mode == 1)
    PQ_BK_HIST(1);
  else
    PQ_BK_HIST(2);
#undef PQ_BK_HIST
  if (!fused) hipLaunchKernelGGL(k_bk_scan, dim3(1), dim3(1024), 0, c->stream, int(nbk), tot, bstart, d_plan);
  if (f32)
    hipLaunchKernelGGL(k_bk_scatter<true>, ga, blk, fused ? 2 * lds : lds, c->stream, xyz, n, int(nbk), bits,
                       key_tmp, tot, cursor, bstart, fused, static_cast<float4*>(bucketed), keyb, d_plan);
  else
    hipLaunchKernelGGL(k_bk_scatter<false>, ga, blk, fused ? 2 * lds : lds, c->stream, xyz, n, int(nbk), bits,
                       key_tmp, tot, cursor, bstart, fused, static_cast<PointRec*>(bucketed), keyb, d_plan);
}

template <int BITS, bool F32>
static void launch_bk_sort_plain(Ctx* c, int64_t nbk, const int32_t* bstart, const void* bucketed, const int32_t* keyb,
                                 uint32_t* word_tmp, int32_t* rank_tmp, DevGrid* g) {
  hipLaunchKernelGGL((k_bk_sort_plain<BITS, F32>), dim3(unsigned(nbk)), dim3((1 << BITS) / 8), 0, c->stream,
                     g->ncell + 1, bstart, static_cast<const typename BkRec<F32>::type*>(bucketed), keyb, word_tmp,
                     rank_tmp, g->start, g->order, g->cell_of, g->sx, g->sy, g->sz, g->p4, g->occ_part);
}

static int build_grid_bucketed(Ctx* c, const double* xyz, int64_t n, DevGrid* g) {
  const int bits = g->ncell + 1 <= (int64_t(kBkMax) << 12) ? 12 : 13;
  const int64_t nbk = (g->ncell + (int64_t(1) << bits)) >> bits;
  const bool f32 = g->p4 != nullptr;
  int32_t *tot, *bstart, *cursor, *key_tmp, *keyb, *rank_tmp;
  uint32_t* word_tmp;
  void* bucketed;
  PQ_TRY(c->arena.get(size_t(nbk) * 2, &tot));
  cursor = tot + nbk;
  PQ_TRY(c->arena.get(size_t(nbk) + 1, &bstart));
  PQ_TRY(c->arena.get(size_t(n), &key_tmp));
  PQ_TRY(c->arena.get(size_t(n), &keyb));
  PQ_TRY(c->arena.get(size_t(n), &word_tmp));
  PQ_TRY(c->arena.get(size_t(n), &rank_tmp));
  if (f32) {
    float4* b4;
    PQ_TRY(c->arena.get(size_t(n), &b4));
    bucketed = b4;
  } else {
    PointRec* b8;
    PQ_TRY(c->arena.get(size_t(n), &b8));
    bucketed = b8;
  }
  g->occ_blocks = int(nbk);
  PQ_TRY(c->arena.get(size_t(nbk), &g->occ_part));
  PQ_HIP(hipMemsetAsync(tot, 0, size_t(nbk) * 8, c->stream));
  const int raw[3] = {0, 0, 0};
  enqueue_bk_a(c, 2, f32, xyz, n, grid_params(*g), raw, AxisMap{nullptr, nullptr, nullptr}, nbk, bits, key_tmp, tot,
               cursor, bstart, bucketed, keyb, nullptr);
  if (bits == 12) {
    if (f32)
      launch_bk_sort_plain<12, true>(c, nbk, bstart, bucketed, keyb, word_tmp, rank_tmp, g);
    else
      launch_bk_sort_plain<12, false>(c, nbk, bstart, bucketed, keyb, word_tmp, rank_tmp, g);
  } else {
    if (f32)
      launch_bk_sort_plain<13, true>(c, nbk, bstart, bucketed, keyb, word_tmp, rank_tmp, g);
    else
      launch_bk_sort_plain<13, false>(c, nbk, bstart, bucketed, keyb, word_tmp, rank_tmp, g);
  }
  PQ_HIP(hipGetLastError());
  return 0;
}


__device__ __forceinline__ double ord_val_dev(unsigned long long k) {
  const unsigned long long b = (k >> 63) ? (k & 0x7FFFFFFFFFFFFFFFull) : ~k;
  return __longlong_as_double(static_cast<long long>(b));
}

__device__ void write_plan(const unsigned long long* box, const PlanIn& in, GridPlan* __restrict__ plan) {
  GridPlan p;
  bool ok = in.hint.valid != 0;
  for (int a = 0; a < 3; ++a) {
    p.mn[a] = ord_val_dev(box[a]);
    p.mx[a] = ord_val_dev(box[3 + a]);
    ok = ok && isfinite(p.mn[a]) && isfinite(p.mx[a]);
  }
  p.all_f32 = box[6] != 0 ? 1 : 0;
  ok = ok && p.all_f32;
  double tot = 1.0;
  int raw[3];
  for (int a = 0; a < 3; ++a) {
    const double d = floor((p.mx[a] - p.mn[a]) / in.cell) + 1.0;
    if (!(d < 2.0e9)) ok = false;
    raw[a] = ok ? int(d) : 0;
    tot *= d + 2.0;
  }
  ok = ok && tot <= double(in.max_cells);
  p.inv_cell = 1.0 / in.cell;
  p.rx = raw[0];
  p.ry = raw[1];
  p.rz = raw[2];
  p.nx = raw[0] + 2;
  p.ny = raw[1] + 2;
  p.nz = raw[2] + 2;
  const int64_t ncell = ok ? int64_t(p.nx) * p.ny * p.nz : 0;
  const int64_t nbk = (ncell + 4096) >> 12;
  ok = ok && ncell + 1 <= (int64_t(kBkMax) << 12) && ncell <= in.hint.ncell && nbk <= in.hint.nbk &&
       (nbk <= kBkFusedScan) == (in.hint.fused != 0);
  p.ncell = ok ? int(ncell) : 0;
  p.nbk = ok ? int(nbk) : 0;
  p.bits = 12;
  p.ok = ok ? 1 : 0;
  p.seq = in.seq;
  *plan = p;
  if (in.host) {
    p.seq = 0;
    *in.host = p;
    __threadfence_system();
    *reinterpret_cast<volatile unsigned*>(&in.host->seq) = in.seq;
  }
}

int plan_grid_device(Ctx* c, const double* xyz, int64_t n, double cell, int64_t max_cells, const PlanHint& hint,
                     GridPlan* d_plan, GridPlan* h_plan, unsigned seq, int32_t* zero_buf, int zero_n) {
  if (n <= 0) return fail(PYQSM_EINVAL, "bounding box of an empty cloud");
  const int blocks = int(std::min<int64_t>(ceil_div(n, 256), int64_t(c->cu_count) * 4));
  unsigned long long *d_box = nullptr, *d_part = nullptr;
  PQ_TRY(c->arena.get(kBoxVals, &d_box));
  PQ_TRY(c->arena.get(size_t(blocks) * kBoxVals, &d_part));
  hipLaunchKernelGGL(k_bbox, dim3(blocks), dim3(256), 0, c->stream, xyz, n, d_part, stamp_slots(c, blocks));
  hipLaunchKernelGGL(k_bbox_fold, dim3(1), dim3(256), 0, c->stream, d_part, blocks, d_box, zero_buf, zero_n,
                     PlanIn{cell, max_cells, hint, h_plan, seq}, d_plan);
  PQ_HIP(hipGetLastError());
  return 0;
}

int octant_zeroed_ints() { return 2 * kBkMax + 5 + kZeroedExtra; }

template <int BITS, bool F32>
static void launch_bk_sort(Ctx* c, int64_t ncell, int64_t nbk, const int32_t* bstart, const void* bucketed,
                           const int32_t* keyb, uint32_t* word_tmp, int32_t* rank_tmp, PointRec* keyed,
                           const GridPlan* d_plan, DevGrid* g, SubCells* sub) {
  unsigned long long* const st_sort = stamp_slots(c, nbk);
  hipLaunchKernelGGL((k_bk_sort<BITS, F32>), dim3(unsigned(nbk)), dim3((1 << BITS) / 8), 0, c->stream, ncell + 1, bstart,
                     static_cast<const typename BkRec<F32>::type*>(bucketed), keyb, word_tmp, rank_tmp, g->start, g->order,
                     g->cell_of, sub->sub_of, g->sx, g->sy, g->sz, g->p4, sub->rec, keyed, d_plan, st_sort);
}

static int enqueue_bucketed(Ctx* c, const double* xyz, int64_t n, const GridParams& gp, const int raw[3],
                            AxisMap am, bool mapped, int64_t ncell, int64_t nbk, int bits, bool f32,
                            int32_t* zeroed, const GridPlan* d_plan, DevGrid* g, SubCells* sub) {
  int32_t *cell_tmp, *keyb, *rank_tmp, *bstart;
  uint32_t* word_tmp;
  int32_t *tot = zeroed, *cursor = zeroed + kBkMax;
  PointRec* keyed;
  void* bucketed;
  g->p4 = nullptr;
  g->sx = g->sy = g->sz = nullptr;
  sub->sub_cnt = sub->sub_beg = nullptr;
  PQ_TRY(c->arena.get(size_t(ncell) + 1, &g->start));
  PQ_TRY(c->arena.get(size_t(n), &g->order));
  PQ_TRY(c->arena.get(size_t(n), &g->cell_of));
  if (f32) {
    float4* b4;
    PQ_TRY(c->arena.get(size_t(n), &g->p4));
    PQ_TRY(c->arena.get(size_t(n), &b4));
    bucketed = b4;
  } else {
    PointRec* b8;
    PQ_TRY(c->arena.get(size_t(n), &g->sx));
    PQ_TRY(c->arena.get(size_t(n), &g->sy));
    PQ_TRY(c->arena.get(size_t(n), &g->sz));
    PQ_TRY(c->arena.get(size_t(n), &b8));
    bucketed = b8;
  }
  PQ_TRY(c->arena.get(size_t(n), &cell_tmp));
  PQ_TRY(c->arena.get(size_t(n), &keyb));
  PQ_TRY(c->arena.get(size_t(n), &word_tmp));
  PQ_TRY(c->arena.get(size_t(n), &rank_tmp));
  PQ_TRY(c->arena.get(size_t(n), &keyed));
  PQ_TRY(c->arena.get(size_t(n), &sub->sub_of));
  PQ_TRY(c->arena.get(size_t(n) * 8, &sub->rec));
  PQ_TRY(c->arena.get(size_t(nbk) + 1, &bstart));
  enqueue_bk_a(c, mapped ? 1 : 0, f32, xyz, n, gp, raw, am, nbk, bits, cell_tmp, tot, cursor, bstart, bucketed, keyb,
               d_plan);
  if (bits == 12) {
    if (f32)
      launch_bk_sort<12, true>(c, ncell, nbk, bstart, bucketed, keyb, word_tmp, rank_tmp, keyed, d_plan, g, sub);
    else
      launch_bk_sort<12, false>(c, ncell, nbk, bstart, bucketed, keyb, word_tmp, rank_tmp, keyed, d_plan, g, sub);
  } else {
    if (f32)
      launch_bk_sort<13, true>(c, ncell, nbk, bstart, bucketed, keyb, word_tmp, rank_tmp, keyed, d_plan, g, sub);
    else
      launch_bk_sort<13, false>(c, ncell, nbk, bstart, bucketed, keyb, word_tmp, rank_tmp, keyed, d_plan, g, sub);
  }
  PQ_HIP(hipGetLastError());
  return 0;
}

int bin_octants_planned(Ctx* c, const double* xyz, int64_t n, double cell, const PlanHint& hint,
                        const GridPlan* d_plan, int32_t* zeroed, DevGrid* g, SubCells* sub) {
  g->minx = g->miny = g->minz = 0.0;
  g->cell = cell;
  g->inv_cell = 1.0 / cell;
  g->nx = g->ny = g->nz = 0;
  g->ncell = hint.ncell;
  sub->zeroed4 = zeroed + 2 * kBkMax + 1;
  const int raw[3] = {0, 0, 0};
  return enqueue_bucketed(c, xyz, n, GridParams{}, raw, AxisMap{nullptr, nullptr, nullptr}, false, hint.ncell,
                          hint.nbk, 12, true, zeroed, d_plan, g, sub);
}

static int upload_plan(Ctx* c, const GridPlan& p, GridPlan* h_up, GridPlan* d_plan) {
  *h_up = p;
  PQ_HIP(hipMemcpyAsync(d_plan, h_up, sizeof(GridPlan), hipMemcpyHostToDevice, c->stream));
  return 0;
}

int bin_octants_host(Ctx* c, const double* xyz, int64_t n, double min_cell, int64_t max_cells, const GridPlan& box,
                     int32_t* zeroed, GridPlan* h_up, GridPlan* d_plan, DevGrid* g, SubCells* sub,
                     PlanHint* hint_out) {
  *hint_out = PlanHint{};
  if (n <= 0) return fail(PYQSM_EINVAL, "build_grid_octants: empty cloud");
  if (n > (int64_t(1) << 27)) return fail(PYQSM_ERANGE, "octant sub-cells: more than 2^27 points");
  if (max_cells > (int64_t(1) << 28)) max_cells = int64_t(1) << 28;
  if (!(min_cell > 0) || !std::isfinite(min_cell))
    return fail(PYQSM_EINVAL, "cell edge must be positive and finite");
  double mn[3], mx[3];
  for (int a = 0; a < 3; ++a) {
    mn[a] = box.mn[a];
    mx[a] = box.mx[a];
    if (!std::isfinite(mn[a]) || !std::isfinite(mx[a])) return fail(PYQSM_EINVAL, "point coordinates must be finite");
  }
  bool all_f32 = box.all_f32 != 0;
  sub->zeroed4 = zeroed + 2 * kBkMax + 1;
  GridPlan hp{};
  {
    const char* f32_env = getenv("PYQSM_COORD_F32");
    if (f32_env && !strcmp(f32_env, "0")) all_f32 = false;
  }
  const char* bin_env = getenv("PYQSM_DBSCAN_BIN");
  if (bin_env && !strcmp(bin_env, "2pass")) {
    const double bbox[6] = {mn[0], mn[1], mn[2], mx[0], mx[1], mx[2]};
    PQ_TRY(build_grid(c, xyz, n, min_cell, max_cells, g, bbox));
    int32_t* zeroed4 = sub->zeroed4;
    PQ_TRY(subsort_octants(c, g, n, sub));
    sub->zeroed4 = zeroed4;
    hp.nx = g->nx;
    hp.ny = g->ny;
    hp.nz = g->nz;
    hp.ncell = int(g->ncell);
    hp.ok = 1;
    return upload_plan(c, hp, h_up, d_plan);
  }
  const dim3 grid(ceil_div(n, 256)), blk(256);
  double cell = min_cell;
  int raw[3], dims[3];
  AxisMap am{nullptr, nullptr, nullptr};
  bool mapped = false;
  for (;;) {
    double tot = 1.0;
    bool ok = true;
    for (int a = 0; a < 3; ++a) {
      const double d = std::floor((mx[a] - mn[a]) / cell) + 1.0;
      if (!(d < 2.0e9)) ok = false;
      raw[a] = ok ? int(d) : 0;
      dims[a] = raw[a] + 2;
      tot *= d + 2.0;
    }
    if (ok && tot <= double(max_cells)) break;
    const int64_t raw_sum = ok ? int64_t(raw[0]) + raw[1] + raw[2] : int64_t(1) << 40;
    if (raw_sum <= (int64_t(1) << 27)) {
      GridParams gp{mn[0], mn[1], mn[2], 1.0 / cell, 0, 0, 0};
      int32_t* occ[3];
      int32_t* map[3];
      for (int a = 0; a < 3; ++a) {
        PQ_TRY(c->arena.get(size_t(raw[a]) + 1, &occ[a]));
        PQ_TRY(c->arena.get(size_t(raw[a]) + 1, &map[a]));
        PQ_HIP(hipMemsetAsync(occ[a], 0, (size_t(raw[a]) + 1) * 4, c->stream));
      }
      hipLaunchKernelGGL(k_axis_occ, grid, blk, 0, c->stream, xyz, n, gp, raw[0], raw[1], raw[2], occ[0],
                         occ[1], occ[2]);
      double ctot = 1.0;
      for (int a = 0; a < 3; ++a) {
        hipLaunchKernelGGL(k_axis_keep, dim3(ceil_div(raw[a] + 1, 256)), blk, 0, c->stream, raw[a], occ[a],
                           map[a]);
        PQ_HIP(hipGetLastError());
        PQ_TRY(exclusive_scan_i32(c, map[a], int64_t(raw[a]) + 1));
        int32_t kept = 0;
        PQ_HIP(hipMemcpyAsync(&kept, map[a] + raw[a], 4, hipMemcpyDeviceToHost, c->stream));
        PQ_HIP(hipStreamSynchronize(c->stream));
        hipLaunchKernelGGL(k_axis_shift, dim3(ceil_div(raw[a], 256)), blk, 0, c->stream, raw[a], map[a]);
        dims[a] = kept + 2;
        ctot *= double(dims[a]);
      }
      PQ_HIP(hipGetLastError());
      if (ctot <= double(max_cells)) {
        am = AxisMap{map[0], map[1], map[2]};
        mapped = true;
        break;
      }
    }
    cell *= 2.0;
  }
  g->minx = mn[0];
  g->miny = mn[1];
  g->minz = mn[2];
  g->cell = cell;
  g->inv_cell = 1.0 / cell;
  g->nx = dims[0];
  g->ny = dims[1];
  g->nz = dims[2];
  g->ncell = int64_t(dims[0]) * dims[1] * dims[2];
  const int bits = g->ncell + 1 <= (int64_t(kBkMax) << 12) ? 12 : 13;
  const int64_t nbk = (g->ncell + (int64_t(1) << bits)) >> bits;
  const bool bucketed_path = nbk <= kBkMax && !(bin_env && !strcmp(bin_env, "atomic"));
  for (int a = 0; a < 3; ++a) {
    hp.mn[a] = mn[a];
    hp.mx[a] = mx[a];
  }
  hp.inv_cell = g->inv_cell;
  hp.nx = dims[0];
  hp.ny = dims[1];
  hp.nz = dims[2];
  hp.rx = raw[0];
  hp.ry = raw[1];
  hp.rz = raw[2];
  hp.ncell = int(g->ncell);
  hp.nbk = int(nbk);
  hp.bits = bits;
  hp.all_f32 = all_f32 && bucketed_path;
  hp.ok = 1;
  PQ_TRY(upload_plan(c, hp, h_up, d_plan));
  const GridParams gp = grid_params(*g);
  if (bucketed_path) {
    PQ_TRY(enqueue_bucketed(c, xyz, n, gp, raw, am, mapped, g->ncell, nbk, bits, hp.all_f32, zeroed, d_plan, g, sub));
    if (!mapped && cell == min_cell && bits == 12 && hp.all_f32) {
      int64_t ncell_h = std::min<int64_t>(g->ncell + g->ncell / 16, (int64_t(kBkMax) << 12) - 1);
      if (nbk <= kBkFusedScan) ncell_h = std::min<int64_t>(ncell_h, (int64_t(kBkFusedScan) << 12) - 1);
      hint_out->valid = 1;
      hint_out->ncell = int(ncell_h);
      hint_out->nbk = int((ncell_h + 4096) >> 12);
      hint_out->fused = nbk <= kBkFusedScan;
    }
    return 0;
  }
  int32_t *cell_tmp, *rank_tmp, *big_list, *big_cnt = zeroed + 2 * kBkMax;
  PointRec* keyed;
  g->p4 = nullptr;
  PQ_TRY(c->arena.get(size_t(g->ncell) + 1, &g->start));
  PQ_TRY(c->arena.get(size_t(n), &g->order));
  PQ_TRY(c->arena.get(size_t(n), &g->cell_of));
  PQ_TRY(c->arena.get(size_t(n), &g->sx));
  PQ_TRY(c->arena.get(size_t(n), &g->sy));
  PQ_TRY(c->arena.get(size_t(n), &g->sz));
  PQ_TRY(c->arena.get(size_t(n), &cell_tmp));
  PQ_TRY(c->arena.get(size_t(n), &rank_tmp));
  PQ_TRY(c->arena.get(size_t(n), &keyed));
  PQ_TRY(c->arena.get(size_t(n) * 8, &sub->sub_cnt));
  PQ_TRY(c->arena.get(size_t(n) * 8, &sub->sub_beg));
  PQ_TRY(c->arena.get(size_t(n), &sub->sub_of));
  PQ_TRY(c->arena.get(size_t(n) * 8, &sub->rec));
  PQ_TRY(c->arena.get(size_t(n) / kBigCell + 2, &big_list));
  PQ_HIP(hipMemsetAsync(g->start, 0, (size_t(g->ncell) + 1) * 4, c->stream));
  if (mapped)
    hipLaunchKernelGGL(k_cell_count_oct<true>, grid, blk, 0, c->stream, xyz, n, gp, raw[0], raw[1], raw[2],
                       am, g->start, cell_tmp, rank_tmp);
  else
    hipLaunchKernelGGL(k_cell_count_oct<false>, grid, blk, 0, c->stream, xyz, n, gp, raw[0], raw[1], raw[2],
                       am, g->start, cell_tmp, rank_tmp);
  PQ_HIP(hipGetLastError());
  PQ_TRY(exclusive_scan_i32(c, g->start, g->ncell + 1));
  hipLaunchKernelGGL(k_scatter_keys, grid, blk, 0, c->stream, xyz, n, g->start, cell_tmp, rank_tmp, keyed);
  hipLaunchKernelGGL(k_order_cells, grid, blk, 0, c->stream, int(n), g->start, keyed, g->order,
                     g->cell_of, sub->sub_of, g->sx, g->sy, g->sz, sub->sub_cnt, sub->sub_beg, sub->rec,
                     big_list, big_cnt);
  PQ_HIP(hipGetLastError());
  hipLaunchKernelGGL(k_order_big, dim3(unsigned(std::min<int64_t>(n / kBigCell + 1, 2048))), blk, 0,
                     c->stream, big_list, big_cnt, g->start, keyed, g->order, g->cell_of, sub->sub_of,
                     g->sx, g->sy, g->sz, g->p4, sub->sub_cnt, sub->sub_beg, sub->rec, d_plan);
  PQ_HIP(hipGetLastError());
  return 0;
}


struct Pyr {
  int fnx, fny, fnz, cnx, cny, cnz, factor;
};

__device__ __forceinline__ int coarse_of(const Pyr& P, int f) {
  const int fx = f % P.fnx, fy = (f / P.fnx) % P.fny, fz = f / (P.fnx * P.fny);
  auto m = [&](int i, int fn, int cn) {
    if (i <= 0) return 0;
    if (i >= fn - 1) return cn - 1;
    return (i - 1) / P.factor + 1;
  };
  const int cx = m(fx, P.fnx, P.cnx), cy = m(fy, P.fny, P.cny), cz = m(fz, P.fnz, P.cnz);
  return (cz * P.cny + cy) * P.cnx + cx;
}

__global__ __launch_bounds__(256) void k_pyr_counts(Pyr P, const int32_t* __restrict__ fstart,
                                                    int32_t* __restrict__ ccount,
                                                    int32_t* __restrict__ foff) {
  const int C = blockIdx.x * 256 + threadIdx.x;
  if (C >= P.cnx * P.cny * P.cnz) return;
  const int cx = C % P.cnx, cy = (C / P.cnx) % P.cny, cz = C / (P.cnx * P.cny);
  int run = 0;
  if (cx >= 1 && cy >= 1 && cz >= 1 && cx <= P.cnx - 2 && cy <= P.cny - 2 && cz <= P.cnz - 2) {
    const int x0 = (cx - 1) * P.factor + 1, y0 = (cy - 1) * P.factor + 1, z0 = (cz - 1) * P.factor + 1;
    if (P.factor == 4) {
#pragma unroll
      for (int dz = 0; dz < 4; ++dz)
#pragma unroll
        for (int dy = 0; dy < 4; ++dy) {
          const int z = z0 + dz, y = y0 + dy;
          if (z > P.fnz - 2 || y > P.fny - 2) continue;
          const int f0 = (z * P.fny + y) * P.fnx + x0;
          const int nxr = min(4, P.fnx - 1 - x0);
          int s[5];
#pragma unroll
          for (int u = 0; u < 5; ++u) s[u] = fstart[f0 + min(u, nxr)];
#pragma unroll
          for (int u = 0; u < 4; ++u)
            if (u < nxr) foff[f0 + u] = run + (s[u] - s[0]);
          run += s[4] - s[0];
        }
    } else {
      for (int z = z0; z < z0 + P.factor && z <= P.fnz - 2; ++z)
        for (int y = y0; y < y0 + P.factor && y <= P.fny - 2; ++y)
          for (int x = x0; x < x0 + P.factor && x <= P.fnx - 2; ++x) {
            const int f = (z * P.fny + y) * P.fnx + x;
            foff[f] = run;
            run += fstart[f + 1] - fstart[f];
          }
    }
  }
  ccount[C] = run;
}

__global__ __launch_bounds__(256) void k_pyr_scatter(int n, Pyr P, const int32_t* __restrict__ fstart,
                                                     const int32_t* __restrict__ cstart,
                                                     const int32_t* __restrict__ foff,
                                                     const int32_t* __restrict__ f_cell_of,
                                                     const int32_t* __restrict__ f_order,
                                                     const double* __restrict__ fx,
                                                     const double* __restrict__ fy,
                                                     const double* __restrict__ fz,
                                                     const float4* __restrict__ fp4,
                                                     int32_t* __restrict__ order,
                                                     int32_t* __restrict__ cell_of,
                                                     double* __restrict__ sx,
                                                     double* __restrict__ sy,
                                                     double* __restrict__ sz, float4* __restrict__ p4) {
  const int p = blockIdx.x * 256 + threadIdx.x;
  if (p >= n) return;
  const int f = f_cell_of[p];
  const int C = coarse_of(P, f);
  const int q = cstart[C] + foff[f] + (p - fstart[f]);
  order[q] = f_order[p];
  cell_of[q] = C;
  if (fp4) {
    p4[q] = fp4[p];
  } else {
    sx[q] = fx[p];
    sy[q] = fy[p];
    sz[q] = fz[p];
  }
}

int coarsen_grid(Ctx* c, const DevGrid& fine, int64_t n, int factor, DevGrid* g) {
  if (factor < 2) return fail(PYQSM_EINVAL, "coarsen_grid: factor must be >= 2");
  Pyr P;
  P.factor = factor;
  P.fnx = fine.nx;
  P.fny = fine.ny;
  P.fnz = fine.nz;
  P.cnx = (fine.nx - 2 + factor - 1) / factor + 2;
  P.cny = (fine.ny - 2 + factor - 1) / factor + 2;
  P.cnz = (fine.nz - 2 + factor - 1) / factor + 2;
  *g = fine;
  g->occ_part = nullptr;
  g->occ_blocks = 0;
  g->nx = P.cnx;
  g->ny = P.cny;
  g->nz = P.cnz;
  g->cell = fine.cell * factor;
  g->inv_cell = 1.0 / g->cell;
  g->ncell = int64_t(P.cnx) * P.cny * P.cnz;
  int32_t* foff = nullptr;
  PQ_TRY(c->arena.get(size_t(fine.ncell) + 1, &foff));
  PQ_TRY(c->arena.get(size_t(g->ncell) + 1, &g->start));
  PQ_TRY(c->arena.get(size_t(n), &g->order));
  PQ_TRY(c->arena.get(size_t(n), &g->cell_of));
  if (fine.p4) {
    PQ_TRY(c->arena.get(size_t(n), &g->p4));
  } else {
    PQ_TRY(c->arena.get(size_t(n), &g->sx));
    PQ_TRY(c->arena.get(size_t(n), &g->sy));
    PQ_TRY(c->arena.get(size_t(n), &g->sz));
  }
  PQ_HIP(hipMemsetAsync(g->start + g->ncell, 0, 4, c->stream));
  hipLaunchKernelGGL(k_pyr_counts, dim3(ceil_div(g->ncell, 256)), dim3(256), 0, c->stream, P,
                     fine.start, g->start, foff);
  PQ_HIP(hipGetLastError());
  PQ_TRY(exclusive_scan_i32(c, g->start, g->ncell + 1));
  hipLaunchKernelGGL(k_pyr_scatter, dim3(ceil_div(n, 256)), dim3(256), 0, c->stream, int(n), P,
                     fine.start, g->start, foff, fine.cell_of, fine.order, fine.sx, fine.sy, fine.sz,
                     static_cast<const float4*>(fine.p4), g->order, g->cell_of, g->sx, g->sy, g->sz, g->p4);
  PQ_HIP(hipGetLastError());
  return 0;
}

int count_occupied(Ctx* c, const DevGrid& g, int64_t* occupied) {
  if (g.occ_part) {
    std::vector<int32_t> h(size_t(g.occ_blocks));
    PQ_HIP(hipMemcpyAsync(h.data(), g.occ_part, h.size() * 4, hipMemcpyDeviceToHost, c->stream));
    PQ_HIP(hipStreamSynchronize(c->stream));
    int64_t t = 0;
    for (int32_t v : h) t += v;
    *occupied = t;
    return 0;
  }
  int32_t* d = nullptr;
  PQ_TRY(c->arena.get(1, &d));
  PQ_HIP(hipMemsetAsync(d, 0, 4, c->stream));
  const int blocks = int(std::min<int64_t>(ceil_div(g.ncell, 256), int64_t(c->cu_count) * 8));
  hipLaunchKernelGGL(k_count_occupied, dim3(blocks), dim3(256), 0, c->stream, g.start, g.ncell, d);
  PQ_HIP(hipGetLastError());
  int32_t h = 0;
  PQ_HIP(hipMemcpyAsync(&h, d, 4, hipMemcpyDeviceToHost, c->stream));
  PQ_HIP(hipStreamSynchronize(c->stream));
  *occupied = h;
  return 0;
}

// ... 84 lines not shown
```

### pyqsm_amd/csrc/grid.hpp

```cpp
#pragma once
#include "common.hpp"

namespace pyqsm {

struct DevGrid {
  double minx, miny, minz;
  double inv_cell;
  double cell;
  int nx, ny, nz;
  int64_t ncell;
  int32_t* start;
  int32_t* order;
  int32_t* cell_of;
  double *sx, *sy, *sz;
  float4* p4 = nullptr;
  int32_t* occ_part = nullptr;
  int occ_blocks = 0;
};

struct GridParams {
  double minx, miny, minz, inv_cell;
  int nx, ny, nz;
};
inline GridParams grid_params(const DevGrid& g) { return GridParams{g.minx, g.miny, g.minz, g.inv_cell, g.nx, g.ny, g.nz}; }

__device__ __forceinline__ void clamped_cell(const GridParams& g, double x, double y, double z, int* cx, int* cy,
                                             int* cz) {
  const double fx = floor((x - g.minx) * g.inv_cell), fy = floor((y - g.miny) * g.inv_cell),
               fz = floor((z - g.minz) * g.inv_cell);
  *cx = int(fmin(fmax(fx, 0.0), double(g.nx - 3))) + 1;
  *cy = int(fmin(fmax(fy, 0.0), double(g.ny - 3))) + 1;
  *cz = int(fmin(fmax(fz, 0.0), double(g.nz - 3))) + 1;
}

__device__ __forceinline__ int cell_index(const GridParams& g, double x, double y, double z) {
  int cx, cy, cz;
  clamped_cell(g, x, y, z, &cx, &cy, &cz);
  return (cz * g.ny + cy) * g.nx + cx;
}

struct StencilRuns {
  int qb[9], qe[9];
};

__device__ __forceinline__ void point_stencil_runs(const GridParams& g, const int32_t* __restrict__ start, double x,
                                                   double y, double z, StencilRuns* rr) {
  int cx, cy, cz;
  clamped_cell(g, x, y, z, &cx, &cy, &cz);
  int w = 0;
  for (int dz = -1; dz <= 1; ++dz)
    for (int dy = -1; dy <= 1; ++dy, ++w) {
      const int zz = cz + dz, yy = cy + dy;
      rr->qb[w] = rr->qe[w] = 0;
      if (zz < 0 || zz >= g.nz || yy < 0 || yy >= g.ny) continue;
      const int x0 = cx - 1 < 0 ? 0 : cx - 1, x1 = cx + 1 >= g.nx ? g.nx - 1 : cx + 1;
      const int row = (zz * g.ny + yy) * g.nx;
      rr->qb[w] = start[row + x0];
      rr->qe[w] = start[row + x1 + 1];
    }
}

int build_grid(Ctx* c, const double* xyz, int64_t n, double min_cell, int64_t max_cells,
               DevGrid* g, const double* bbox = nullptr, bool f32_records = false);

int cloud_bbox(Ctx* c, const double* xyz, int64_t n, double mn[3], double mx[3], bool* all_f32 = nullptr,
               int32_t* zero_buf = nullptr, int zero_n = 0);
int robust_box(Ctx* c, const double* xyz, int64_t n, int budget, double box[6], int64_t* outside);

int probe_occupancy(Ctx* c, const double* xyz, int64_t n, const double box[6], double cell,
                    double* cell_used, double* per_cell);

struct Stencil {
  int nx, nxy;
};

__device__ __forceinline__ double sqdist3(double ax, double ay, double az, double bx, double by, double bz) {
  const double t0 = ax - bx, t1 = ay - by, t2 = az - bz;
  double d = t0 * t0;
  d = d + t1 * t1;
  d = d + t2 * t2;
  return d;
}
struct CoordsF64 {
  const double *x, *y, *z;
  __device__ __forceinline__ void get(int q, double& a, double& b, double& c) const {
    a = x[q];
    b = y[q];
    c = z[q];
  }
  __device__ __forceinline__ double d2(int q, double px, double py, double pz) const {
    return sqdist3(px, py, pz, x[q], y[q], z[q]);
  }
  __device__ __forceinline__ double d2(int a, int q) const {
    return sqdist3(x[a], y[a], z[a], x[q], y[q], z[q]);
  }
  __device__ __forceinline__ void mark_core(int, bool) const {}
  __device__ __forceinline__ bool core_pair_within(int a, int q, const uint8_t* __restrict__ core, double r2) const {
    return core[a] && core[q] && d2(a, q) <= r2;
  }
};
struct CoordsF32 {
  float4* p;
  __device__ __forceinline__ void get(int q, double& a, double& b, double& c) const {
    const float4 v = p[q];
    a = double(v.x);
    b = double(v.y);
    c = double(v.z);
  }
  __device__ __forceinline__ double d2(int q, double px, double py, double pz) const {
    const float4 v = p[q];
    return sqdist3(px, py, pz, double(v.x), double(v.y), double(v.z));
  }
  __device__ __forceinline__ double d2(int a, int q) const {
    const float4 u = p[a], v = p[q];
    return sqdist3(double(u.x), double(u.y), double(u.z), double(v.x), double(v.y), double(v.z));
  }
  __device__ __forceinline__ void mark_core(int q, bool is_core) const {
    reinterpret_cast<float*>(p)[size_t(q) * 4 + 3] = is_core ? 1.0f : 0.0f;
  }
  __device__ __forceinline__ bool core_pair_within(int a, int q, const uint8_t* __restrict__, double r2) const {
    const float4 u = p[a], v = p[q];
    return u.w != 0.0f && v.w != 0.0f &&
           sqdist3(double(u.x), double(u.y), double(u.z), double(v.x), double(v.y), double(v.z)) <= r2;
  }
};


static constexpr int kTileMax = 16384;

struct Tile {
  int qb[9], qe[9];
  int total;
};

__device__ __forceinline__ Tile wave_tile(int p0, int n, Stencil st, int ncell,
                                          const int32_t* __restrict__ start,
                                          const int32_t* __restrict__ cell_of) {
  Tile t;
  const int plast = p0 + 63 < n ? p0 + 63 : n - 1;
  const int c_first = __builtin_amdgcn_readfirstlane(cell_of[p0]);
  const int c_last = __builtin_amdgcn_readfirstlane(cell_of[plast]);
  int lo[9], hi[9];
  int w = 0;
  for (int dz = -1; dz <= 1; ++dz)
    for (int dy = -1; dy <= 1; ++dy) {
      const int o = dy * st.nx + dz * st.nxy;
      int a = c_first + o - 1, b = c_last + o + 1;
      a = a < 0 ? 0 : a;
      b = b > ncell - 1 ? ncell - 1 : b;
      int k = w++;
      while (k > 0 && lo[k - 1] > a) {
        lo[k] = lo[k - 1];
        hi[k] = hi[k - 1];
        --k;
      }
      lo[k] = a;
      hi[k] = b;
    }
  t.total = 0;
  int prev_hi = -1;
  for (int r = 0; r < 9; ++r) {
    const int a = lo[r] <= prev_hi ? prev_hi + 1 : lo[r];
    if (a <= hi[r]) {
      t.qb[r] = __builtin_amdgcn_readfirstlane(start[a]);
      t.qe[r] = __builtin_amdgcn_readfirstlane(start[hi[r] + 1]);
      prev_hi = hi[r];
    } else {
      t.qb[r] = t.qe[r] = 0;
    }
    t.total += t.qe[r] - t.qb[r];
  }
  return t;
}

template <class F>
inline void on_coords(const DevGrid& g, F&& fn) {
  if (g.p4)
    fn(CoordsF32{g.p4});
  else
    fn(CoordsF64{g.sx, g.sy, g.sz});
}

struct SubCells {
  int32_t* sub_cnt;
  int32_t* sub_beg;
  int32_t* sub_of;
  int4* rec;
  int32_t* zeroed4 = nullptr;
};
static constexpr int kZeroedExtra = 64;

int subsort_octants(Ctx* c, DevGrid* g, int64_t n, SubCells* sub);


struct GridPlan {
  double mn[3], mx[3];
  double inv_cell;
  int nx, ny, nz;
  int rx, ry, rz;
  int ncell;
  int nbk, bits;
  int all_f32;
  int ok;
  unsigned seq;
};
__device__ __forceinline__ Stencil plan_stencil(const GridPlan* p) { return Stencil{p->nx, p->nx * p->ny}; }

int plan_grid_device(Ctx* c, const double* xyz, int64_t n, double cell, int64_t max_cells, const PlanHint& hint,
                     GridPlan* d_plan, GridPlan* h_plan, unsigned seq, int32_t* zero_buf, int zero_n);
int octant_zeroed_ints();
int bin_octants_planned(Ctx* c, const double* xyz, int64_t n, double cell, const PlanHint& hint,
                        const GridPlan* d_plan, int32_t* zeroed, DevGrid* g, SubCells* sub);
int bin_octants_host(Ctx* c, const double* xyz, int64_t n, double min_cell, int64_t max_cells, const GridPlan& box,
                     int32_t* zeroed, GridPlan* h_up, GridPlan* d_plan, DevGrid* g, SubCells* sub,
                     PlanHint* hint_out);

int coarsen_grid(Ctx* c, const DevGrid& fine, int64_t n, int factor, DevGrid* coarse);

int radius_grid(Ctx* c, const double* d_src, int64_t n, double radius, DevGrid* g);
int query_order(Ctx* c, const double* d_qry, int64_t m, const GridParams& rg, int64_t ncell, int32_t** perm);

int count_occupied(Ctx* c, const DevGrid& g, int64_t* occupied);

}
```

### pyqsm_amd/hip.py

```python
from __future__ import annotations

import ctypes
import weakref
from typing import NamedTuple

import numpy as np

from . import _lib
from ._lib import check, i64, i32, dbl, vp

MISS_PRIM = np.uint32(0xFFFFFFFF)


def _p(a):
    return None if a is None else a.ctypes.data_as(ctypes.c_void_p)


def _points(points) -> np.ndarray:
    pts = np.ascontiguousarray(np.asarray(points), dtype=np.float64)
    if pts.ndim != 2 or pts.shape[1] != 3:
        raise ValueError(f"expected points of shape [n,3], got {pts.shape}")
    return pts


# ... 24 lines not shown
        out = np.empty(shape, dtype=dtype)
        if out.nbytes > self.nbytes:
            raise ValueError("requested more bytes than the device buffer holds")
        check(_lib.load().pyqsm_d2h(self.device, _p(out), self.ptr, out.nbytes))
        return out

    def free(self) -> None:
        if self.ptr:
            _lib.load().pyqsm_dev_free(self.device, self.ptr)
            self.ptr = None

    def __del__(self):
        try:
            self.free()
        except Exception:
            pass


def sync(device: int = 0) -> None:
    check(_lib.load().pyqsm_sync(int(device)))


def prof_enable(on, device: int = 0) -> None:
    check(_lib.load().pyqsm_prof_enable(int(device), int(on)))


def prof_reset(device: int = 0) -> None:
    check(_lib.load().pyqsm_prof_reset(int(device)))


def prof_get(name: str, device: int = 0):
    ms, cnt = dbl(0.0), i64(0)
    check(_lib.load().pyqsm_prof_get(int(device), name.encode(), ctypes.byref(ms),
                                     ctypes.byref(cnt)))
    return ms.value, cnt.value



def _mesh(verts, tris):
    v = np.ascontiguousarray(np.asarray(verts), dtype=np.float32).reshape(-1, 3)
    t = np.ascontiguousarray(np.asarray(tris), dtype=np.int32).reshape(-1, 3)
    return v, t


def cast_rays(verts, tris, rays, device: int = 0):
    v, t = _mesh(verts, tris)
    r = np.ascontiguousarray(np.asarray(rays), dtype=np.float32)
    if r.shape[-1] != 6:
        raise ValueError(f"rays must have last dimension 6, got {r.shape}")
    lead = r.shape[:-1]
    r2 = r.reshape(-1, 6)
    R = r2.shape[0]
    t_hit = np.empty(R, dtype=np.float32)
    prim = np.empty(R, dtype=np.uint32)
    uv = np.empty((R, 2), dtype=np.float32)
    check(_lib.load().pyqsm_cast_rays(_p(v), v.shape[0], _p(t), t.shape[0], _p(r2), R,
                                      _p(t_hit), _p(prim), _p(uv), int(device)))
    return t_hit.reshape(lead), prim.reshape(lead), uv.reshape(lead + (2,))


def cast_rays_multi(verts, tris, rays, n_devices: int = 0, with_uv: bool = True):
    v, t = _mesh(verts, tris)
    r = np.ascontiguousarray(np.asarray(rays), dtype=np.float32)
    if r.shape[-1] != 6:
        raise ValueError(f"rays must have last dimension 6, got {r.shape}")
    lead = r.shape[:-1]
    r2 = r.reshape(-1, 6)
    R = r2.shape[0]
    t_hit = np.empty(R, dtype=np.float32)
    prim = np.empty(R, dtype=np.uint32)
    uv = np.empty((R, 2), dtype=np.float32) if with_uv else None
    check(_lib.load().pyqsm_cast_rays_multi(_p(v), v.shape[0], _p(t), t.shape[0], _p(r2), R,
                                            _p(t_hit), _p(prim), _p(uv) if with_uv else None,
                                            int(n_devices)))
    return t_hit.reshape(lead), prim.reshape(lead), uv.reshape(lead + (2,)) if with_uv else None


def list_intersections(verts, tris, rays, device: int = 0):
    v, t = _mesh(verts, tris)
    r = np.ascontiguousarray(np.asarray(rays), dtype=np.float32).reshape(-1, 6)
    R = r.shape[0]
    lib = _lib.load()
    counts = np.zeros(R, dtype=np.int32)
    total = i64(0)
    check(lib.pyqsm_list_intersections(_p(v), v.shape[0], _p(t), t.shape[0], _p(r), R, _p(counts),
                                       None, None, None, None, 0, ctypes.byref(total),
                                       int(device)))
    n = int(total.value)
    ray_ids = np.empty(n, dtype=np.uint32)
    prim = np.empty(n, dtype=np.uint32)
    ts = np.empty(n, dtype=np.float32)
    uv = np.empty((n, 2), dtype=np.float32)
    if n:
        check(lib.pyqsm_list_intersections(_p(v), v.shape[0], _p(t), t.shape[0], _p(r), R,
                                           _p(counts), _p(ray_ids), _p(prim), _p(ts), _p(uv), n,
                                           ctypes.byref(total), int(device)))
    return {"ray_ids": ray_ids, "primitive_ids": prim, "t_hit": ts, "primitive_uvs": uv,
            "counts": counts}


def point_mesh_distance(verts, tris, queries, device: int = 0):
    v, t = _mesh(verts, tris)
    q = np.ascontiguousarray(queries, dtype=np.float32).reshape(-1, 3)
    dist = np.empty(q.shape[0], dtype=np.float32)
    prim = np.empty(q.shape[0], dtype=np.uint32)
    check(_lib.load().pyqsm_point_mesh_distance(_p(v), v.shape[0], _p(t), t.shape[0], _p(q), q.shape[0],
                                                _p(dist), _p(prim), int(device)))
    return dist, prim


class DeviceMesh:

    def __init__(self, verts, tris, device: int = 0):
        v, t = _mesh(verts, tris)
        self.device = int(device)
        self.n_tris = t.shape[0]
        dv = DeviceBuffer.from_array(v, device) if v.size else None
        dt = DeviceBuffer.from_array(t, device) if t.size else None
        self.records = DeviceBuffer(max(1, self.n_tris) * 48, device)
        if self.n_tris:
            check(_lib.load().pyqsm_expand_tris_dev(dv.ptr, v.shape[0], dt.ptr, self.n_tris,
                                                    self.records.ptr, self.device))
            sync(device)
        for b in (dv, dt):
            if b is not None:
                b.free()


def cast_rays_dev(mesh: DeviceMesh, rays_ptr: int, n_rays: int, t_hit_ptr: int, prim_ptr: int,
                  uv_ptr: int | None = None) -> None:
    check(_lib.load().pyqsm_cast_rays_dev(mesh.records.ptr, mesh.n_tris, rays_ptr, int(n_rays),
                                          t_hit_ptr, prim_ptr, uv_ptr, mesh.device))



def dbscan(points, eps: float, min_pts: int, device: int = 0, radius_inclusive: bool = True):
    pts = _points(points)
    n = pts.shape[0]
    labels = np.empty(n, dtype=np.int64)
    core = np.zeros(n, dtype=np.uint8)
    check(_lib.load().pyqsm_dbscan_ex(_p(pts), n, float(eps), int(min_pts), int(bool(radius_inclusive)),
                                      _p(labels), _p(core), int(device)))
    return labels, core.astype(bool)


def dbscan_dev(xyz_ptr: int, n: int, eps: float, min_pts: int, labels_ptr: int,
               core_ptr: int | None = None, device: int = 0, want_count: bool = False,
               radius_inclusive: bool = True):
    cnt = i64(0)
    check(_lib.load().pyqsm_dbscan_dev_ex(xyz_ptr, int(n), float(eps), int(min_pts),
                                          int(bool(radius_inclusive)), labels_ptr, core_ptr,
                                          ctypes.byref(cnt) if want_count else None, int(device)))
    return int(cnt.value) if want_count else None


def knn(points, k: int, exclude_self: bool = True, device: int = 0):
    pts = _points(points)
    n = pts.shape[0]
    idx = np.empty((n, int(k)), dtype=np.int32)
    d2 = np.empty((n, int(k)), dtype=np.float64)
    check(_lib.load().pyqsm_knn(_p(pts), n, int(k), int(bool(exclude_self)), _p(idx), _p(d2),
                                int(device)))
    return idx, d2


def knn_dev(xyz_ptr: int, n: int, k: int, exclude_self: bool, idx_ptr: int, d2_ptr: int,
            device: int = 0) -> None:
    check(_lib.load().pyqsm_knn_dev(xyz_ptr, int(n), int(k), int(bool(exclude_self)), idx_ptr,
                                    d2_ptr, int(device)))



SHAPES = {"circle": 0, "cylinder": 1}


def ransac(points, triples, shape: str = "circle", thresh: float = 0.2, device: int = 0):
    pts = _points(points)
    tri = np.ascontiguousarray(np.asarray(triples), dtype=np.int64).reshape(-1, 3)
    n, H = pts.shape[0], tri.shape[0]
    if H and (tri.min() < 0 or tri.max() >= n):
        raise ValueError("sample index outside the point set")
    center = np.zeros(3)
    axis = np.zeros(3)
    radius = dbl(0.0)
    inl = np.empty(max(n, 1), dtype=np.int64)
    n_in, best = i64(0), i64(-1)
    check(_lib.load().pyqsm_ransac(_p(pts), n, _p(tri), H, SHAPES[shape], float(thresh),
                                   _p(center), _p(axis), ctypes.byref(radius), _p(inl),
                                   ctypes.byref(n_in), ctypes.byref(best), int(device)))
    return center, axis, radius.value, inl[:n_in.value].copy(), int(best.value)


def ransac_batch(points, seg_start, triples, shape: str = "circle", thresh: float = 0.2, device: int = 0):
    pts = _points(points)
    ss = np.ascontiguousarray(seg_start, dtype=np.int64)
    S = len(ss) - 1
    tri = np.ascontiguousarray(np.asarray(triples), dtype=np.int64).reshape(S, -1, 3)
    H = tri.shape[1]
    sizes = np.diff(ss)
    if H and S:
        ok = (tri >= 0).all(axis=(1, 2)) | (sizes < 3)
        if not ok.all() or (tri.max(axis=(1, 2)) >= np.maximum(sizes, 1))[sizes >= 3].any():
            raise ValueError("sample index outside its point set")
    centers = np.zeros((S, 3))
    axes = np.zeros((S, 3))
    radii = np.zeros(S)
    inl = np.empty(max(pts.shape[0], 1), dtype=np.int64)
    n_in = np.zeros(S, dtype=np.int64)
    best = np.full(S, -1, dtype=np.int64)
    check(_lib.load().pyqsm_ransac_batch(_p(pts), pts.shape[0], _p(ss), S, _p(tri), H, SHAPES[shape],
                                         float(thresh), _p(centers), _p(axes), _p(radii), _p(inl), _p(n_in),
                                         _p(best), int(device)))
    ends = np.cumsum(n_in)
    inliers = [inl[e - c:e].copy() for c, e in zip(n_in, ends)]
    return centers, axes, radii, inliers, best


def ransac_models(points, triples, device: int = 0):
    pts = _points(points)
    tri = np.ascontiguousarray(np.asarray(triples), dtype=np.int64).reshape(-1, 3)
    models = np.zeros((tri.shape[0], 8))
    check(_lib.load().pyqsm_ransac_models(_p(pts), pts.shape[0], _p(tri), tri.shape[0],
                                          _p(models), int(device)))
    return models


def ransac_count(points, models, shape: str = "circle", thresh: float = 0.2, device: int = 0):
    pts = _points(points)
    m = np.ascontiguousarray(models, dtype=np.float64).reshape(-1, 8)
    counts = np.zeros(m.shape[0], dtype=np.int32)
    check(_lib.load().pyqsm_ransac_count(_p(pts), pts.shape[0], _p(m), m.shape[0], SHAPES[shape],
                                         float(thresh), _p(counts), int(device)))
    return counts



def _csr(L):
    if isinstance(L, tuple):
        indptr, indices, data = L
    else:
        L = L.tocsr()
        L.sort_indices()
        indptr, indices, data = L.indptr, L.indices, L.data
    indptr = np.ascontiguousarray(indptr, dtype=np.int32)
    indices = np.ascontiguousarray(indices, dtype=np.int32)
    data = np.ascontiguousarray(data, dtype=np.float64)
    return indptr, indices, data, indptr.shape[0] - 1


def lbc_solve(L, wl, wh, pts, rtol: float = 1e-10, max_it: int = 20000, device: int = 0):
    indptr, indices, data, n = _csr(L)
    p = _points(pts)
    if p.shape[0] != n:
        raise ValueError("L and pts disagree on n")
    wl = np.ascontiguousarray(np.broadcast_to(np.asarray(wl, dtype=np.float64), (n,)))
    wh = np.ascontiguousarray(np.broadcast_to(np.asarray(wh, dtype=np.float64), (n,)))
    out = np.empty_like(p)
    iters = i32(0)
    resid = np.zeros(3)
    rc = _lib.load().pyqsm_lbc_solve(_p(indptr), _p(indices), _p(data), n, _p(wl), _p(wh), _p(p),
                                     float(rtol), int(max_it), _p(out), ctypes.byref(iters),
                                     _p(resid), int(device))
    if rc not in (0, -6):
        check(rc)
    return out, int(iters.value), resid, rc == 0


def spmv3(L, x, device: int = 0):
    indptr, indices, data, n = _csr(L)
    x = _points(x)
    y = np.empty_like(x)
    check(_lib.load().pyqsm_spmv3(_p(indptr), _p(indices), _p(data), n, _p(x), _p(y), int(device)))
    return y


def clamp(pts: np.ndarray, lo, hi, device: int = 0) -> np.ndarray:
    if not (isinstance(pts, np.ndarray) and pts.dtype == np.float64 and pts.flags.c_contiguous):
        raise ValueError("clamp works in place on a C-contiguous float64 array")
    lo = np.ascontiguousarray(lo, dtype=np.float64)
    hi = np.ascontiguousarray(hi, dtype=np.float64)
    check(_lib.load().pyqsm_clamp(_p(pts), pts.shape[0], _p(lo), _p(hi), int(device)))
    return pts



def ball_query(points, center, radius: float, device: int = 0) -> np.ndarray:
    pts = _points(points)
    ctr = np.ascontiguousarray(center, dtype=np.float64).reshape(3)
    out = np.empty(max(pts.shape[0], 1), dtype=np.int64)
    cnt = i64(0)
    check(_lib.load().pyqsm_ball_query(_p(pts), pts.shape[0], _p(ctr), float(radius), _p(out),
                                       ctypes.byref(cnt), int(device)))
    return out[:cnt.value].copy()


def radius_mark(src, queries, radius: float, k: int = 500, device: int = 0):
    s = _points(src)
    q = _points(queries)
    mark = np.zeros(s.shape[0], dtype=np.uint8)
    counts = np.zeros(q.shape[0], dtype=np.int32)
    check(_lib.load().pyqsm_radius_mark(_p(s), s.shape[0], _p(q), q.shape[0], float(radius),
                                        int(k), _p(mark), _p(counts), int(device)))
    return mark.astype(bool), counts



# ... 948 lines not shown
```

Before: 3208 Mpoints/s.

## Replace dense cell start array with compressed bitmap directory for DBSCAN lookups

Builds a compressed cell directory (32-cell bitmap words plus packed begin slots) from the dense start array, and switches DBSCAN kernels to query it via popcount instead of indexing the dense array. It also batches stencil-bound loads in the tiled and rest core kernels, lets several lanes compute bounds for multiple rest points at once, and replaces the insertion sort in wave_tile with an unrolled branchless network. The aim is a smaller cache footprint for sparse grids and fewer serialized scalar loads. The cost is an extra build kernel, a two-level indirection on each lookup, and more register pressure. A debugging entry point that exports the directory is added as well.

```diff
diff --git a/include/pyqsm_hip.h b/include/pyqsm_hip.h
--- a/include/pyqsm_hip.h
+++ b/include/pyqsm_hip.h
@@ -82,6 +82,8 @@
 int pyqsm_dbscan_dev_ex(const double* xyz_dev, int64_t n, double eps, int32_t min_pts,
                         int32_t radius_inclusive, int64_t* labels_dev, uint8_t* is_core_dev,
                         int64_t* n_clusters, int32_t device);
+int pyqsm_octant_directory(const double* xyz, int64_t n, double eps, int32_t* dims_out,
+                           int32_t* begin_out, int64_t cap, int32_t device);
 
 int pyqsm_knn(const double* xyz, int64_t n, int32_t k, int32_t exclude_self,
               int32_t* idx, double* d2, int32_t device);
diff --git a/pyqsm_amd/_lib.py b/pyqsm_amd/_lib.py
--- a/pyqsm_amd/_lib.py
+++ b/pyqsm_amd/_lib.py
@@ -47,6 +47,7 @@
     "pyqsm_dbscan_dev": (ctypes.c_int, [vp, i64, dbl, i32, vp, vp, ctypes.POINTER(i64), i32]),
     "pyqsm_dbscan_ex": (ctypes.c_int, [vp, i64, dbl, i32, i32, vp, vp, i32]),
     "pyqsm_dbscan_dev_ex": (ctypes.c_int, [vp, i64, dbl, i32, i32, vp, vp, ctypes.POINTER(i64), i32]),
+    "pyqsm_octant_directory": (ctypes.c_int, [vp, i64, dbl, vp, vp, i64, i32]),
     "pyqsm_knn": (ctypes.c_int, [vp, i64, i32, i32, vp, vp, i32]),
     "pyqsm_knn_dev": (ctypes.c_int, [vp, i64, i32, i32, vp, vp, i32]),
     "pyqsm_ransac": (ctypes.c_int, [vp, i64, vp, i64, i32, dbl, vp, vp, ctypes.POINTER(dbl), vp,
diff --git a/pyqsm_amd/csrc/dbscan.hip b/pyqsm_amd/csrc/dbscan.hip
--- a/pyqsm_amd/csrc/dbscan.hip
+++ b/pyqsm_amd/csrc/dbscan.hip
@@ -19,11 +19,11 @@
 }
 
 
-#define FOR_STENCIL(c, st, start, q, body)                         \
+#define FOR_STENCIL(c, st, dir, q, body)                           \
   for (int dz__ = -1; dz__ <= 1; ++dz__)                           \
     for (int dy__ = -1; dy__ <= 1; ++dy__) {                       \
       const int row__ = (c) + dy__ * (st).nx + dz__ * (st).nxy;    \
-      const int qb__ = (start)[row__ - 1], qe__ = (start)[row__ + 2]; \
+      const int qb__ = (dir).begin(row__ - 1), qe__ = (dir).begin(row__ + 2); \
       for (int q = qb__; q < qe__; ++q) {                          \
         body                                                       \
       }                                                            \
@@ -38,9 +38,26 @@
 static constexpr int kRestSegs = 64;
 __device__ constexpr int kRunOrder[9] = {4, 3, 5, 1, 7, 0, 2, 6, 8};
 
+__device__ __forceinline__ void stencil_bounds(int c, Stencil st, const CellDir& dir, int (&qb)[9], int (&qe)[9]) {
+  int cells[18], q[18];
+#pragma unroll
+  for (int r = 0; r < 9; ++r) {
+    const int row = c + (kRunOrder[r] % 3 - 1) * st.nx + (kRunOrder[r] / 3 - 1) * st.nxy;
+    cells[2 * r] = row - 1;
+    cells[2 * r + 1] = row + 2;
+  }
+  dir.begins(cells, q);
+#pragma unroll
+  for (int r = 0; r < 9; ++r) {
+    qb[r] = q[2 * r];
+    qe[r] = q[2 * r + 1];
+  }
+}
+
 template <class CO>
 __global__ __launch_bounds__(256) void k_core_tiled(int n, const GridPlan* __restrict__ plan,
-                                                    const int32_t* __restrict__ start,
+                                                    const DirWord* __restrict__ dwords,
+                                                    const int32_t* __restrict__ dslots,
                                                     const int32_t* __restrict__ cell_of, CO co, double r2,
                                                     int min_pts, uint8_t* __restrict__ core,
                                                     int32_t* __restrict__ rest,
@@ -51,6 +68,7 @@
     unsigned long long* __restrict__ st ) {
   __shared__ TileLds L;
   stamped(st, [&] {
+  const CellDir dir{dwords, dslots};
   const int lane = threadIdx.x & 63, w = __builtin_amdgcn_readfirstlane(threadIdx.x >> 6);
   const int p0 = (blockIdx.x * 4 + w) * 64;
   if (p0 >= n || !plan->ok) return;
@@ -60,7 +78,7 @@
   const bool live = p < n;
   double x = 0.0, y = 0.0, z = 0.0;
   if (live) co.get(p, x, y, z);
-  const Tile t = wave_tile(p0, n, st, ncell, start, cell_of);
+  const Tile t = wave_tile(p0, n, st, ncell, dir, cell_of);
   int cnt = 0;
   bool deferred = false;
   int chunks = 0;
@@ -73,23 +91,24 @@
       const int c = __builtin_amdgcn_readlane(mycell, lead);
       const bool mine = mycell == c;
       todo &= ~__ballot(mine);
-      for (int dz = -1; dz <= 1; ++dz)
-        for (int dy = -1; dy <= 1; ++dy) {
-          const int row = c + dy * st.nx + dz * st.nxy;
-          const int qb = __builtin_amdgcn_readfirstlane(start[row - 1]);
-          const int qe = __builtin_amdgcn_readfirstlane(start[row + 2]);
-          for (int base = qb; base < qe; base += 64) {
-            const int q = base + lane;
-            const int m = qe - base < 64 ? qe - base : 64;
-            if (q < qe) co.get(q, L.x[w][lane], L.y[w][lane], L.z[w][lane]);
-            __builtin_amdgcn_wave_barrier();
-            staged += m;
-            if (mine)
-              for (int j = 0; j < m; ++j)
-                cnt += sqdist(x, y, z, L.x[w][j], L.y[w][j], L.z[w][j]) <= r2;
-            __builtin_amdgcn_wave_barrier();
-          }
+      int rqb[9], rqe[9];
+      stencil_bounds(c, st, dir, rqb, rqe);
+#pragma unroll
+      for (int r = 0; r < 9; ++r) {
+        const int qb = __builtin_amdgcn_readfirstlane(rqb[r]);
+        const int qe = __builtin_amdgcn_readfirstlane(rqe[r]);
+        for (int base = qb; base < qe; base += 64) {
+          const int q = base + lane;
+          const int m = qe - base < 64 ? qe - base : 64;
+          if (q < qe) co.get(q, L.x[w][lane], L.y[w][lane], L.z[w][lane]);
+          __builtin_amdgcn_wave_barrier();
+          staged += m;
+          if (mine)
+            for (int j = 0; j < m; ++j)
+              cnt += sqdist(x, y, z, L.x[w][j], L.y[w][j], L.z[w][j]) <= r2;
+          __builtin_amdgcn_wave_barrier();
         }
+      }
     }
   } else {
 #pragma unroll
@@ -150,20 +169,24 @@
     return q;
   }
 };
-__device__ __forceinline__ Runs9 stencil_runs(int c, Stencil st, const int32_t* __restrict__ start) {
+static constexpr int kRunBatch = 3;
+__device__ __forceinline__ int lane_bound(bool act, int c, int j, Stencil st, const CellDir& dir) {
+  const int r = int((0x862071534ull >> (4 * (j >> 1))) & 15ull);
+  const int cell = c + (r % 3 - 1) * st.nx + (r / 3 - 1) * st.nxy + ((j & 1) ? 2 : -1);
+  int b = 0;
+  if (act) {
+    const DirWord w = dir.words[cell >> 5];
+    b = dir.slots[CellDir::slot_of(w, cell)];
+  }
+  return b;
+}
+__device__ __forceinline__ Runs9 runs_of_lanes(int bound, int k) {
   Runs9 t;
-  int qe[9];
+  t.pre[0] = 0;
 #pragma unroll
   for (int r = 0; r < 9; ++r) {
-    const int row = c + (kRunOrder[r] % 3 - 1) * st.nx + (kRunOrder[r] / 3 - 1) * st.nxy;
-    t.qb[r] = start[row - 1];
-    qe[r] = start[row + 2];
-  }
-  t.pre[0] = 0;
-#pragma unroll
-  for (int r = 0; r < 9; ++r) {
-    t.qb[r] = __builtin_amdgcn_readfirstlane(t.qb[r]);
-    t.pre[r + 1] = t.pre[r] + (__builtin_amdgcn_readfirstlane(qe[r]) - t.qb[r]);
+    t.qb[r] = __builtin_amdgcn_readlane(bound, 18 * k + 2 * r);
+    t.pre[r + 1] = t.pre[r] + (__builtin_amdgcn_readlane(bound, 18 * k + 2 * r + 1) - t.qb[r]);
   }
   return t;
 }
@@ -172,11 +195,13 @@
 __global__ __launch_bounds__(256) void k_core_rest(const int32_t* __restrict__ rest,
                                                    const int32_t* __restrict__ rest_cnt ,
                                                    int seg_cap, const GridPlan* __restrict__ plan,
-                                                   const int32_t* __restrict__ start,
+                                                   const DirWord* __restrict__ dwords,
+                                                   const int32_t* __restrict__ dslots,
                                                    const int32_t* __restrict__ cell_of, CO co, double r2,
                                                    int min_pts, uint8_t* __restrict__ core,
     unsigned long long* __restrict__ st ) {
   stamped(st, [&] {
+  const CellDir dir{dwords, dslots};
   if (!plan->ok) return;
   const Stencil st = plan_stencil(plan);
   const int lane = threadIdx.x & 63;
@@ -188,23 +213,41 @@
     if (lane >= off) incl += v;
   }
   const int m = __shfl(incl, 63, 64);
-  for (int i = blockIdx.x * 4 + (threadIdx.x >> 6); i < m; i += gridDim.x * 4) {
-    const int seg = __popcll(__ballot(incl <= i));
-    const int before = __shfl(incl - mine, seg, 64);
-    const int p = rest[size_t(seg) * seg_cap + (i - before)];
-    double x, y, z;
-    co.get(p, x, y, z);
-    const int c = __builtin_amdgcn_readfirstlane(cell_of[p]);
-    const Runs9 t = stencil_runs(c, st, start);
-    int cnt = 0;
-    for (int g0 = 0; g0 < t.pre[9] && cnt < min_pts; g0 += 64) {
-      const int g = g0 + lane;
-      const bool hit = g < t.pre[9] && co.d2(t.at(g), x, y, z) <= r2;
-      cnt += __popcll(__ballot(hit));
-    }
-    if (lane == 0) {
-      core[p] = cnt >= min_pts;
-      co.mark_core(p, cnt >= min_pts);
+  const int grp = lane / 18, j = lane % 18;
+  for (int i0 = (blockIdx.x * 4 + (threadIdx.x >> 6)) * kRunBatch; i0 < m; i0 += gridDim.x * 4 * kRunBatch) {
+    int p = 0;
+#pragma unroll
+    for (int k = 0; k < kRunBatch; ++k) {
+      if (i0 + k >= m) break;
+      const int seg = __popcll(__ballot(incl <= i0 + k));
+      const int before = __shfl(incl - mine, seg, 64);
+      const int pk = rest[size_t(seg) * seg_cap + (i0 + k - before)];
+      p = grp == k ? pk : p;
+    }
+    const bool act = grp < kRunBatch && i0 + grp < m;
+    double x = 0.0, y = 0.0, z = 0.0;
+    int c = 0;
+    if (act) {
+      co.get(p, x, y, z);
+      c = cell_of[p];
+    }
+    const int bound = lane_bound(act, c, j, st, dir);
+#pragma unroll
+    for (int k = 0; k < kRunBatch; ++k) {
+      if (i0 + k >= m) break;
+      const Runs9 t = runs_of_lanes(bound, k);
+      const int pk = __builtin_amdgcn_readlane(p, 18 * k);
+      const double xk = __shfl(x, 18 * k, 64), yk = __shfl(y, 18 * k, 64), zk = __shfl(z, 18 * k, 64);
+      int cnt = 0;
+      for (int g0 = 0; g0 < t.pre[9] && cnt < min_pts; g0 += 64) {
+        const int g = g0 + lane;
+        const bool hit = g < t.pre[9] && co.d2(t.at(g), xk, yk, zk) <= r2;
+        cnt += __popcll(__ballot(hit));
+      }
+      if (lane == 0) {
+        core[pk] = cnt >= min_pts;
+        co.mark_core(pk, cnt >= min_pts);
+      }
     }
   }
   });
@@ -383,19 +426,16 @@
   int q0, n2, rep;
 };
 __device__ __forceinline__ SubNbr sub_neighbour(bool active, const int4 at, int dx, int dy, int dz, int nx, int ny,
-                                                const int32_t* __restrict__ start,
-                                                const int4* __restrict__ rec) {
+                                                const CellDir& dir, const int4* __restrict__ rec) {
   const int gx = 2 * (at.x - 1) + (at.w & 1) - dx, gy = 2 * (at.y - 1) + ((at.w >> 1) & 1) - dy,
             gz = 2 * (at.z - 1) + ((at.w >> 2) & 1) - dz;
   const int c2 = (((gz >> 1) + 1) * ny + ((gy >> 1) + 1)) * nx + ((gx >> 1) + 1);
   const int oct = (gx & 1) | ((gy & 1) << 1) | ((gz & 1) << 2);
   SubNbr out{0, 0, -1};
-  int b2 = 0, e2 = 0;
-  if (active) {
-    b2 = start[c2];
-    e2 = start[c2 + 1];
-  }
-  if (e2 != b2) {
+  DirWord w{0u, 0u};
+  if (active) w = dir.words[c2 >> 5];
+  if ((w.bits >> (c2 & 31)) & 1u) {
+    const int b2 = dir.slots[CellDir::slot_of(w, c2)];
     const int4 r = rec[b2 * 8 + oct];
     if (r.y > 0) {
       out.q0 = r.x;
@@ -410,12 +450,15 @@
 __global__ __launch_bounds__(256) void k_hook_sub(const int4* __restrict__ list,
                                                   const int4* __restrict__ list_xyz,
                                                   const int32_t* __restrict__ m_ptr,
-                                                  const GridPlan* __restrict__ plan, const int32_t* __restrict__ start,
+                                                  const GridPlan* __restrict__ plan,
+                                                  const DirWord* __restrict__ dwords,
+                                                  const int32_t* __restrict__ dslots,
                                                   const int4* __restrict__ rec, CO co, double r2,
                                                   const uint8_t* __restrict__ core,
                                                   int* __restrict__ parent,
     unsigned long long* __restrict__ st ) {
   stamped(st, [&] {
+  const CellDir dir{dwords, dslots};
   if (!plan->ok) return;
   const int nx = plan->nx, ny = plan->ny;
   const int m = *m_ptr;
@@ -426,7 +469,7 @@
   for (int s0 = (blockIdx.x * 4 + (threadIdx.x >> 6)) * kSubPerWave; s0 < m; s0 += gridDim.x * 4 * kSubPerWave) {
     const bool live = s0 + grp < m;
     const int4 me = list[min(s0 + grp, m - 1)], at = list_xyz[min(s0 + grp, m - 1)];
-    const SubNbr nb2 = sub_neighbour(live && t < 13, at, o_dx, o_dy, o_dz, nx, ny, start, rec);
+    const SubNbr nb2 = sub_neighbour(live && t < 13, at, o_dx, o_dy, o_dz, nx, ny, dir, rec);
     const int p = me.x, n1 = me.w;
     unsigned todo = unsigned(__ballot(nb2.rep >= 0) >> (16 * grp)) & 0xFFFFu;
     int base = 0, hooked = -1;
@@ -474,10 +517,10 @@
 
 template <class CO>
 __device__ __forceinline__ void seam_unite(const int4 me, const int4 at, int k, int o_dx, int o_dy, int o_dz,
-                                           int nx, int ny, const int32_t* __restrict__ start,
+                                           int nx, int ny, const CellDir& dir,
                                            const int4* __restrict__ rec, const CO& co, double r2,
                                            const uint8_t* __restrict__ core, int* parent) {
-  const SubNbr nb2 = sub_neighbour(k < 62, at, o_dx, o_dy, o_dz, nx, ny, start, rec);
+  const SubNbr nb2 = sub_neighbour(k < 62, at, o_dx, o_dy, o_dz, nx, ny, dir, rec);
   const int p = me.x, n1 = me.w, rep2 = nb2.rep;
   const int* vparent = parent;
   int a1 = 0, a2 = 0;
@@ -515,12 +558,15 @@
 __global__ __launch_bounds__(256) void k_union_sub(const int4* __restrict__ list,
                                                    const int4* __restrict__ list_xyz,
                                                    const int32_t* __restrict__ m_ptr,
-                                                   const GridPlan* __restrict__ plan, const int32_t* __restrict__ start,
+                                                   const GridPlan* __restrict__ plan,
+                                                   const DirWord* __restrict__ dwords,
+                                                   const int32_t* __restrict__ dslots,
                                                    const int4* __restrict__ rec, CO co, double r2,
                                                    const uint8_t* __restrict__ core, int* parent,
                                                    unsigned long long* __restrict__ seam_cnt ,
     unsigned long long* __restrict__ st ) {
   stamped(st, [&] {
+  const CellDir dir{dwords, dslots};
   if (!plan->ok) return;
   const int nx = plan->nx, ny = plan->ny;
   const int m = *m_ptr;
@@ -536,24 +582,29 @@
     const int* vparent = parent;
     const int r_s = vparent[me.x];
     const int c2 = me.y + c_off;
-    int b2[2] = {0, 0}, e2[2] = {0, 0}, word[2] = {0, 0};
+    int word[2] = {0, 0};
+    DirWord dw[2] = {{0u, 0u}, {0u, 0u}};
     if (live && t < 9) {
 #pragma unroll
-      for (int l = 0; l < 2; ++l) {
-        b2[l] = start[c2 - l * layer];
-        e2[l] = start[c2 - l * layer + 1];
-      }
+      for (int l = 0; l < 2; ++l) dw[l] = dir.words[(c2 - l * layer) >> 5];
+    }
+    int b2[2] = {0, 0};
+    bool occ[2];
+#pragma unroll
+    for (int l = 0; l < 2; ++l) {
+      occ[l] = (dw[l].bits >> ((c2 - l * layer) & 31)) & 1u;
+      if (occ[l]) b2[l] = dir.slots[CellDir::slot_of(dw[l], c2 - l * layer)];
     }
 #pragma unroll
     for (int l = 0; l < 2; ++l)
-      if (e2[l] != b2[l]) word[l] = rec[b2[l] * 8].w;
+      if (occ[l]) word[l] = rec[b2[l] * 8].w;
     const unsigned long long seams =
         __ballot((word[0] != 0 && word[0] != r_s + 1) || (word[1] != 0 && word[1] != r_s + 1));
     if (!seams) continue;
     for (int u = 0; u < kSubPerWave; ++u) {
       if (!((seams >> (16 * u)) & 0xFFFFull)) continue;
       if (seam_cnt && k == 0) atomicAdd(seam_cnt, 1ull);
-      seam_unite(list[s0 + u], list_xyz[s0 + u], k, o_dx, o_dy, o_dz, nx, ny, start, rec, co, r2, core, parent);
+      seam_unite(list[s0 + u], list_xyz[s0 + u], k, o_dx, o_dy, o_dz, nx, ny, dir, rec, co, r2, core, parent);
     }
   }
   });
@@ -561,9 +612,11 @@
 
 template <class CO>
 __global__ __launch_bounds__(256) void k_union_points(int n, Stencil st,
-                                                      const int32_t* __restrict__ start,
+                                                      const DirWord* __restrict__ dwords,
+                                                      const int32_t* __restrict__ dslots,
                                                       const int32_t* __restrict__ cell_of, CO co, double r2,
                                                       const uint8_t* __restrict__ core, int* parent) {
+  const CellDir dir{dwords, dslots};
   int p = blockIdx.x * 256 + threadIdx.x;
   if (p >= n || !core[p]) return;
   double x, y, z;
@@ -571,7 +624,7 @@
   const int c = cell_of[p];
   const volatile int* vparent = parent;
   int rp = find_root(parent, p);
-  FOR_STENCIL(c, st, start, q, {
+  FOR_STENCIL(c, st, dir, q, {
     if (q < p && core[q] && co.d2(q, x, y, z) <= r2) {
       if (vparent[q] != rp) {
         unite(parent, p, q);
@@ -823,7 +876,8 @@
 __global__ __launch_bounds__(kLabelThreads) void k_labels(int n, const int32_t* __restrict__ rest,
                                                           const int32_t* __restrict__ rest_cnt,
                                                           const GridPlan* __restrict__ plan,
-                                                          const int32_t* __restrict__ start,
+                                                          const DirWord* __restrict__ dwords,
+                                                          const int32_t* __restrict__ dslots,
                                                           const int32_t* __restrict__ cell_of, CO co, double r2,
                                                           const uint8_t* __restrict__ core,
                                                           const int* __restrict__ parent,
@@ -836,6 +890,7 @@
                                                           uint8_t* __restrict__ is_core,
     unsigned long long* __restrict__ st ) {
   stamped(st, [&] {
+  const CellDir dir{dwords, dslots};
   if (!plan->ok) return;
   constexpr int kWaves = kLabelThreads / 64;
   const int n_roots = *roots_cnt;
@@ -851,31 +906,43 @@
   }
   const int m = *rest_cnt;
   const Stencil sten = plan_stencil(plan);
-  const int first = blockIdx.x * kWaves + __builtin_amdgcn_readfirstlane(threadIdx.x >> 6);
-  for (int i = first; i < m; i += gridDim.x * kWaves) {
-    const int p = rest[i];
-    double x, y, z;
-    co.get(p, x, y, z);
-    const int c = __builtin_amdgcn_readfirstlane(cell_of[p]);
-    const Runs9 t = stencil_runs(c, sten, start);
-    int best = kNoRoot;
-    for (int g0 = 0; g0 < t.pre[9]; g0 += 64) {
-      const int g = g0 + lane;
-      if (g < t.pre[9]) {
-        const int q = t.at(g);
-        if (core[q] && co.d2(q, x, y, z) <= r2) {
-          const int mo = min_orig[parent[parent[q]]];
-          best = mo < best ? mo : best;
+  const int first = (blockIdx.x * kWaves + __builtin_amdgcn_readfirstlane(threadIdx.x >> 6)) * kRunBatch;
+  const int grp = lane / 18, j = lane % 18;
+  for (int i0 = first; i0 < m; i0 += gridDim.x * kWaves * kRunBatch) {
+    const bool act = grp < kRunBatch && i0 + grp < m;
+    double x = 0.0, y = 0.0, z = 0.0;
+    int p = 0, c = 0;
+    if (act) {
+      p = rest[i0 + grp];
+      co.get(p, x, y, z);
+      c = cell_of[p];
+    }
+    const int bound = lane_bound(act, c, j, sten, dir);
+#pragma unroll
+    for (int k = 0; k < kRunBatch; ++k) {
+      if (i0 + k >= m) break;
+      const Runs9 t = runs_of_lanes(bound, k);
+      const int pk = __builtin_amdgcn_readlane(p, 18 * k);
+      const double xk = __shfl(x, 18 * k, 64), yk = __shfl(y, 18 * k, 64), zk = __shfl(z, 18 * k, 64);
+      int best = kNoRoot;
+      for (int g0 = 0; g0 < t.pre[9]; g0 += 64) {
+        const int g = g0 + lane;
+        if (g < t.pre[9]) {
+          const int q = t.at(g);
+          if (core[q] && co.d2(q, xk, yk, zk) <= r2) {
+            const int mo = min_orig[parent[parent[q]]];
+            best = mo < best ? mo : best;
+          }
         }
       }
-    }
-#pragma unroll
-    for (int off = 32; off > 0; off >>= 1) {
-      const int o = __shfl_xor(best, off, 64);
-      best = o < best ? o : best;
-    }
-    if (lane == 0)
-      labels[order[p]] = best == kNoRoot ? int64_t(-1) : int64_t(cluster_number(best, n_roots, bits, wpre));
+#pragma unroll
+      for (int off = 32; off > 0; off >>= 1) {
+        const int o = __shfl_xor(best, off, 64);
+        best = o < best ? o : best;
+      }
+      if (lane == 0)
+        labels[order[pk]] = best == kNoRoot ? int64_t(-1) : int64_t(cluster_number(best, n_roots, bits, wpre));
+    }
   }
   });
 }
@@ -887,6 +954,7 @@
   const int N = int(n);
   const dim3 grid(ceil_div(n, 256)), block(256);
   const Stencil st{g.nx, g.nx * g.ny};
+  const CellDir dir = cell_dir(g);
   const double r2 = radius_inclusive ? eps * eps : nextafter(eps * eps, 0.0);
   uint8_t* core;
   int *parent, *min_orig;
@@ -924,7 +992,7 @@
     {
       const StampKernel pk(c, "k_core_tiled", grid.x);
       on_coords(g, [&](auto co) {
-        hipLaunchKernelGGL(k_core_tiled<decltype(co)>, grid, block, 0, c->stream, N, d_plan, g.start, g.cell_of, co, r2,
+        hipLaunchKernelGGL(k_core_tiled<decltype(co)>, grid, block, 0, c->stream, N, d_plan, dir.words, dir.slots, g.cell_of, co, r2,
                            min_pts, core, rest, rest_segs, seg_cap, parent, min_orig, flag, max_chunks, d_tests,
                            pk.slots);
       });
@@ -940,7 +1008,7 @@
     const dim3 gr(std::min<int64_t>(8192, ceil_div(n, 64)));
     unsigned long long* const st_rest = stamp_slots(c, gr.x);
     on_coords(g, [&](auto co) {
-      hipLaunchKernelGGL(k_core_rest<decltype(co)>, gr, block, 0, c->stream, rest, rest_segs, seg_cap, d_plan, g.start,
+      hipLaunchKernelGGL(k_core_rest<decltype(co)>, gr, block, 0, c->stream, rest, rest_segs, seg_cap, d_plan, dir.words, dir.slots,
                          g.cell_of, co, r2, min_pts, core, st_rest);
     });
     PQ_HIP(hipGetLastError());
@@ -975,7 +1043,7 @@
           const StampKernel pk(c, "k_hook_sub", gh.x);
           on_coords(g, [&](auto co) {
             hipLaunchKernelGGL(k_hook_sub<decltype(co)>, gh, block, 0, c->stream, list, list_xyz, list_cnt, d_plan,
-                               g.start, sub.rec, co, r2, core, parent, pk.slots);
+                               dir.words, dir.slots, sub.rec, co, r2, core, parent, pk.slots);
           });
         }
         if (trace) {
@@ -1019,7 +1087,7 @@
           const StampKernel pk(c, "k_union_sub", gu.x);
           on_coords(g, [&](auto co) {
             hipLaunchKernelGGL(k_union_sub<decltype(co)>, gu, block, 0, c->stream, list, list_xyz, list_cnt, d_plan,
-                               g.start, sub.rec, co, r2, core, parent, d_seams, pk.slots);
+                               dir.words, dir.slots, sub.rec, co, r2, core, parent, d_seams, pk.slots);
           });
         }
         if (trace) {
@@ -1035,7 +1103,7 @@
     } else {
       PQ_TRY(stamp_mark(c));
       on_coords(g, [&](auto co) {
-        hipLaunchKernelGGL(k_union_points<decltype(co)>, grid, block, 0, c->stream, N, st, g.start, g.cell_of, co,
+        hipLaunchKernelGGL(k_union_points<decltype(co)>, grid, block, 0, c->stream, N, st, dir.words, dir.slots, g.cell_of, co,
                            r2, core, parent);
       });
       hipLaunchKernelGGL(k_flatten, grid, block, 0, c->stream, N, core, parent, d_plan);
@@ -1055,7 +1123,7 @@
     unsigned long long* const st_labels = stamp_slots(c, gb.x);
     on_coords(g, [&](auto co) {
       hipLaunchKernelGGL(k_labels<decltype(co)>, gb, dim3(kLabelThreads), 0, c->stream, N, rest, list_cnt + 3, d_plan,
-                         g.start, g.cell_of, co, r2, core, parent, min_orig, roots_cnt, bits, wpre, g.order, labels,
+                         dir.words, dir.slots, g.cell_of, co, r2, core, parent, min_orig, roots_cnt, bits, wpre, g.order, labels,
                          is_core, st_labels);
     });
     PQ_HIP(hipGetLastError());
@@ -1086,8 +1154,14 @@
   return 0;
 }
 
+struct DirReadout {
+  int64_t cap;
+  int32_t* begin_host;
+  int32_t dims[3];
+};
 static int dbscan_device(Ctx* c, const double* xyz, int64_t n, double eps, int32_t min_pts,
-                         bool radius_inclusive, int64_t* labels, uint8_t* is_core, int64_t* n_clusters) {
+                         bool radius_inclusive, int64_t* labels, uint8_t* is_core, int64_t* n_clusters,
+                         DirReadout* readout = nullptr) {
   if (!(eps > 0) || !std::isfinite(eps)) return fail(PYQSM_EINVAL, "eps must be positive");
   if (n == 0) {
     if (n_clusters) *n_clusters = 0;
@@ -1123,7 +1197,8 @@
   if (speculate) {
     PQ_TRY(bin_octants_planned(c, xyz, n, cell, hint, d_plan, zeroed, &g, &sub));
     bin_scope.reset();
-    PQ_TRY(cluster_binned(c, n, eps, min_pts, radius_inclusive, g, sub, d_plan, labels, is_core, &count));
+    if (!readout)
+      PQ_TRY(cluster_binned(c, n, eps, min_pts, radius_inclusive, g, sub, d_plan, labels, is_core, &count));
   }
   PQ_TRY(wait_plan(c, h_plan, seq));
   const bool hit = speculate && h_plan[0].ok;
@@ -1136,11 +1211,29 @@
     PQ_TRY(stamp_mark(c));
     bin_scope.reset();
     if (next.valid) c->plan_hint = next;
-    PQ_TRY(cluster_binned(c, n, eps, min_pts, radius_inclusive, g, sub, d_plan + 1, labels, is_core, &count));
+    if (!readout)
+      PQ_TRY(cluster_binned(c, n, eps, min_pts, radius_inclusive, g, sub, d_plan + 1, labels, is_core, &count));
   }
   if (c->prof >= 1) {
     c->timers["dbscan_f32_records"].launches += g.p4 ? 1 : 0;
     c->timers[hit ? "dbscan_plan_hit" : "dbscan_plan_miss"].launches += 1;
+  }
+  if (readout) {
+    const GridPlan& pl = hit ? h_plan[0] : h_plan[1];
+    readout->dims[0] = pl.nx;
+    readout->dims[1] = pl.ny;
+    readout->dims[2] = pl.nz;
+    const int64_t entries = int64_t(pl.ncell) + 1;
+    if (entries > readout->cap)
+      return fail(PYQSM_ERANGE, "octant directory: %lld entries, room for %lld", (long long)entries,
+                  (long long)readout->cap);
+    int32_t* d_begin;
+    PQ_TRY(c->arena.get(size_t(entries), &d_begin));
+    read_directory(c, g, pl.ncell, d_begin);
+    PQ_HIP(hipGetLastError());
+    PQ_HIP(hipMemcpyAsync(readout->begin_host, d_begin, size_t(entries) * 4, hipMemcpyDeviceToHost, c->stream));
+    PQ_HIP(hipStreamSynchronize(c->stream));
+    return 0;
   }
   if (n_clusters) {
     int32_t h = 0;
@@ -1207,4 +1300,22 @@
   return 0;
 }
 
-}
+int pyqsm_octant_directory(const double* xyz, int64_t n, double eps, int32_t* dims_out, int32_t* begin_out,
+                           int64_t cap, int32_t device) {
+  PQ_API_RANGE("pyqsm_octant_directory");
+  if (n <= 0) return fail(PYQSM_EINVAL, "pyqsm_octant_directory: empty cloud");
+  if (!xyz || !dims_out || !begin_out) return fail(PYQSM_EINVAL, "pyqsm_octant_directory: NULL pointer");
+  Ctx* c = ctx_for(device);
+  if (!c) return PYQSM_ENODEV;
+  std::lock_guard<std::mutex> lk(c->mu);
+  c->arena.reset();
+  double* d_xyz;
+  PQ_TRY(c->arena.get(size_t(n) * 3, &d_xyz));
+  PQ_HIP(hipMemcpyAsync(d_xyz, xyz, size_t(n) * 24, hipMemcpyHostToDevice, c->stream));
+  DirReadout ro{cap, begin_out, {0, 0, 0}};
+  PQ_TRY(dbscan_device(c, d_xyz, n, eps, 1, true, nullptr, nullptr, nullptr, &ro));
+  for (int a = 0; a < 3; ++a) dims_out[a] = ro.dims[a];
+  return 0;
+}
+
+}
diff --git a/pyqsm_amd/csrc/grid.hip b/pyqsm_amd/csrc/grid.hip
--- a/pyqsm_amd/csrc/grid.hip
+++ b/pyqsm_amd/csrc/grid.hip
@@ -949,6 +949,7 @@
   int32_t cnt[1 << BITS];
   uint32_t big[(1 << BITS) / 32];
   int32_t wsum[16];
+  int32_t osum[16];
   int32_t any_big;
   int32_t btot[8], bbase[8];
   int32_t bw[(1 << BITS) / 512][8];
@@ -963,9 +964,10 @@
 
 template <int BITS, bool F32>
 __global__ __launch_bounds__((1 << BITS) / 8, BITS == 12 ? 6 : 4) void k_bk_sort(
-    int64_t ncell1 , const int32_t* __restrict__ bstart,
+    const int32_t* __restrict__ bstart,
     const typename BkRec<F32>::type* __restrict__ bucketed, const int32_t* __restrict__ keyb,
-    uint32_t* __restrict__ word_tmp, int32_t* __restrict__ rank_tmp, int32_t* __restrict__ start,
+    uint32_t* __restrict__ word_tmp, int32_t* __restrict__ rank_tmp,
+    DirWord* __restrict__ words , int32_t* __restrict__ slots ,
     int32_t* __restrict__ order, int32_t* __restrict__ cell_of, int32_t* __restrict__ sub_of,
     double* __restrict__ sx, double* __restrict__ sy, double* __restrict__ sz,
     float4* __restrict__ p4 , int4* __restrict__ rec,
@@ -979,24 +981,19 @@
   stamped(st, [&] {
   const int bk = blockIdx.x, t = threadIdx.x;
   if (!plan->ok || bk >= plan->nbk) return;
-  ncell1 = int64_t(plan->ncell) + 1;
   const int s = bstart[bk], e = bstart[bk + 1];
   const int64_t c0 = int64_t(bk) << BITS;
+  constexpr int WORDS = CELLS / 32;
+  DirWord* const wds = words + size_t(bk) * WORDS;
+  const uint32_t sb = uint32_t(s) + uint32_t(bk);
   if (s == e) {
-#pragma unroll
-    for (int k = 0; k < 2; ++k) {
-      const int64_t cidx = c0 + int64_t(k * T + t) * 4;
-      if (cidx + 3 < ncell1) {
-        *reinterpret_cast<int4*>(start + cidx) = make_int4(s, s, s, s);
-      } else {
-        for (int u = 0; u < 4; ++u)
-          if (cidx + u < ncell1) start[cidx + u] = s;
-      }
-    }
+    if (t < WORDS) wds[t] = DirWord{0u, sb};
+    if (t == 0) slots[sb] = s;
     return;
   }
   if (e - s <= 64) {
     int32_t* const cells = L.cnt;
+    int32_t* const dcell = L.cnt + 64;
     const int m = e - s;
     if (t < 64) {
       const bool live = t < m;
@@ -1013,7 +1010,7 @@
       }
       if (live) {
         const int cl = lk >> 3, o = lk & 7, b = s + below_cell, f = s + below_key;
-        cells[t] = cl;
+        cells[below_key] = cl;
         cell_of[f] = int(c0) + cl;
         sub_of[f] = b * 8 + o;
         if constexpr (F32) {
@@ -1037,20 +1034,31 @@
       }
     }
     __syncthreads();
-    int32_t pre[8] = {s, s, s, s, s, s, s, s};
-    for (int q = 0; q < m; ++q) {
-      const int d = cells[q] - 8 * t;
-#pragma unroll
-      for (int k = 0; k < 8; ++k) pre[k] += d < k ? 1 : 0;
-    }
-    const int64_t cidx = c0 + 8 * t;
-    if (cidx + 7 < ncell1) {
-      *reinterpret_cast<int4*>(start + cidx) = make_int4(pre[0], pre[1], pre[2], pre[3]);
-      *reinterpret_cast<int4*>(start + cidx + 4) = make_int4(pre[4], pre[5], pre[6], pre[7]);
-    } else {
-#pragma unroll
-      for (int k = 0; k < 8; ++k)
-        if (cidx + k < ncell1) start[cidx + k] = pre[k];
+    if (t < 64) {
+      const bool live = t < m;
+      const int ci = live ? cells[t] : -1;
+      const bool head = live && (t == 0 || cells[t - 1] != ci);
+      const unsigned long long hm = __ballot(head);
+      const int rk = __popcll(hm & ((1ull << t) - 1ull));
+      if (head) {
+        slots[sb + rk] = s + t;
+        dcell[rk] = ci;
+      }
+      if (t == 0) {
+        slots[sb + __popcll(hm)] = e;
+        L.wsum[0] = __popcll(hm);
+      }
+    }
+    __syncthreads();
+    if (t < WORDS) {
+      const int nd = L.wsum[0];
+      uint32_t bits = 0u, before = 0u;
+      for (int q = 0; q < nd; ++q) {
+        const int c = dcell[q];
+        before += c < 32 * t ? 1u : 0u;
+        bits |= (c >> 5) == t ? 1u << (c & 31) : 0u;
+      }
+      wds[t] = DirWord{bits, sb + before};
     }
     return;
   }
@@ -1109,17 +1117,30 @@
 #pragma unroll
     for (int k = 0; k < 8; ++k) tot += v[k];
   }
+  uint32_t occ8 = 0u;
+#pragma unroll
+  for (int k = 0; k < 8; ++k) occ8 |= v[k] ? 1u << k : 0u;
+  const int nocc = __popc(occ8);
   const int lane = t & 63, w = t >> 6;
-  int32_t incl = tot;
+  int32_t incl = tot, oincl = nocc;
 #pragma unroll
   for (int off = 1; off < 64; off <<= 1) {
-    const int32_t u = __shfl_up(incl, off, 64);
-    if (lane >= off) incl += u;
-  }
-  if (lane == 63) L.wsum[w] = incl;
-  __syncthreads();
-  int32_t run = incl - tot;
-  for (int q = 0; q < w; ++q) run += L.wsum[q];
+    const int32_t u = __shfl_up(incl, off, 64), uo = __shfl_up(oincl, off, 64);
+    if (lane >= off) {
+      incl += u;
+      oincl += uo;
+    }
+  }
+  if (lane == 63) {
+    L.wsum[w] = incl;
+    L.osum[w] = oincl;
+  }
+  __syncthreads();
+  int32_t run = incl - tot, orun = oincl - nocc;
+  for (int q = 0; q < w; ++q) {
+    run += L.wsum[q];
+    orun += L.osum[q];
+  }
   int32_t pre[8];
 #pragma unroll
   for (int k = 0; k < 8; ++k) {
@@ -1127,15 +1148,9 @@
     run += v[k];
   }
   {
-    const int64_t cidx = c0 + 8 * t;
-    if (cidx + 7 < ncell1) {
-      *reinterpret_cast<int4*>(start + cidx) = make_int4(s + pre[0], s + pre[1], s + pre[2], s + pre[3]);
-      *reinterpret_cast<int4*>(start + cidx + 4) = make_int4(s + pre[4], s + pre[5], s + pre[6], s + pre[7]);
-    } else {
-#pragma unroll
-      for (int k = 0; k < 8; ++k)
-        if (cidx + k < ncell1) start[cidx + k] = s + pre[k];
-    }
+    const uint32_t b1 = __shfl_down(occ8, 1, 64), b2 = __shfl_down(occ8, 2, 64), b3 = __shfl_down(occ8, 3, 64);
+    if ((t & 3) == 0) wds[t >> 2] = DirWord{occ8 | (b1 << 8) | (b2 << 16) | (b3 << 24), sb + uint32_t(orun)};
+    if (t == T - 1) slots[sb + uint32_t(orun + nocc)] = e;
   }
 #pragma unroll
   for (int k = 0; k < 8; ++k) {
@@ -1143,6 +1158,7 @@
     L.cnt[cl] = pre[k];
     if (v[k] == 0) continue;
     const int b = s + pre[k];
+    slots[sb + uint32_t(orun) + __popc(occ8 & ((1u << k) - 1u))] = b;
     if (v[k] > kBkBig) {
       atomicOr(&L.big[cl >> 5], 1u << (cl & 31));
       L.any_big = 1;
@@ -1629,17 +1645,18 @@
 int octant_zeroed_ints() { return 2 * kBkMax + 5 + kZeroedExtra; }
 
 template <int BITS, bool F32>
-static void launch_bk_sort(Ctx* c, int64_t ncell, int64_t nbk, const int32_t* bstart, const void* bucketed,
+static void launch_bk_sort(Ctx* c, int64_t nbk, const int32_t* bstart, const void* bucketed,
                            const int32_t* keyb, uint32_t* word_tmp, int32_t* rank_tmp, PointRec* keyed,
                            const GridPlan* d_plan, DevGrid* g, SubCells* sub) {
   unsigned long long* const st_sort = stamp_slots(c, nbk);
-  hipLaunchKernelGGL((k_bk_sort<BITS, F32>), dim3(unsigned(nbk)), dim3((1 << BITS) / 8), 0, c->stream, ncell + 1, bstart,
-                     static_cast<const typename BkRec<F32>::type*>(bucketed), keyb, word_tmp, rank_tmp, g->start, g->order,
+  hipLaunchKernelGGL((k_bk_sort<BITS, F32>), dim3(unsigned(nbk)), dim3((1 << BITS) / 8), 0, c->stream, bstart,
+                     static_cast<const typename BkRec<F32>::type*>(bucketed), keyb, word_tmp, rank_tmp, g->dir_words,
+                     g->dir_slots, g->order,
                      g->cell_of, sub->sub_of, g->sx, g->sy, g->sz, g->p4, sub->rec, keyed, d_plan, st_sort);
 }
 
 static int enqueue_bucketed(Ctx* c, const double* xyz, int64_t n, const GridParams& gp, const int raw[3],
-                            AxisMap am, bool mapped, int64_t ncell, int64_t nbk, int bits, bool f32,
+                            AxisMap am, bool mapped, int64_t nbk, int bits, bool f32,
                             int32_t* zeroed, const GridPlan* d_plan, DevGrid* g, SubCells* sub) {
   int32_t *cell_tmp, *keyb, *rank_tmp, *bstart;
   uint32_t* word_tmp;
@@ -1649,7 +1666,9 @@
   g->p4 = nullptr;
   g->sx = g->sy = g->sz = nullptr;
   sub->sub_cnt = sub->sub_beg = nullptr;
-  PQ_TRY(c->arena.get(size_t(ncell) + 1, &g->start));
+  g->start = nullptr;
+  PQ_TRY(c->arena.get(size_t(nbk) << (bits - 5), &g->dir_words));
+  PQ_TRY(c->arena.get(size_t(n) + size_t(nbk) + 1, &g->dir_slots));
   PQ_TRY(c->arena.get(size_t(n), &g->order));
   PQ_TRY(c->arena.get(size_t(n), &g->cell_of));
   if (f32) {
@@ -1677,17 +1696,53 @@
                d_plan);
   if (bits == 12) {
     if (f32)
-      launch_bk_sort<12, true>(c, ncell, nbk, bstart, bucketed, keyb, word_tmp, rank_tmp, keyed, d_plan, g, sub);
+      launch_bk_sort<12, true>(c, nbk, bstart, bucketed, keyb, word_tmp, rank_tmp, keyed, d_plan, g, sub);
     else
-      launch_bk_sort<12, false>(c, ncell, nbk, bstart, bucketed, keyb, word_tmp, rank_tmp, keyed, d_plan, g, sub);
+      launch_bk_sort<12, false>(c, nbk, bstart, bucketed, keyb, word_tmp, rank_tmp, keyed, d_plan, g, sub);
   } else {
     if (f32)
-      launch_bk_sort<13, true>(c, ncell, nbk, bstart, bucketed, keyb, word_tmp, rank_tmp, keyed, d_plan, g, sub);
+      launch_bk_sort<13, true>(c, nbk, bstart, bucketed, keyb, word_tmp, rank_tmp, keyed, d_plan, g, sub);
     else
-      launch_bk_sort<13, false>(c, ncell, nbk, bstart, bucketed, keyb, word_tmp, rank_tmp, keyed, d_plan, g, sub);
+      launch_bk_sort<13, false>(c, nbk, bstart, bucketed, keyb, word_tmp, rank_tmp, keyed, d_plan, g, sub);
   }
   PQ_HIP(hipGetLastError());
   return 0;
+}
+
+__global__ __launch_bounds__(256) void k_dir_from_dense(int64_t ncell, const int32_t* __restrict__ start,
+                                                        DirWord* __restrict__ words, int32_t* __restrict__ slots) {
+  const int64_t c = int64_t(blockIdx.x) * 256 + threadIdx.x;
+  const int lane = threadIdx.x & 63, half = lane >> 5;
+  const int a = start[c < ncell ? c : ncell];
+  const int b = start[c + 1 < ncell ? c + 1 : ncell];
+  const uint32_t bits = uint32_t(__ballot(b != a) >> (32 * half));
+  const int64_t w = c >> 5;
+  const uint32_t base = uint32_t(__shfl(a, half * 32, 64)) + uint32_t(w);
+  if (w > (ncell >> 5)) return;
+  if (b != a) slots[base + __popc(bits & ((1u << (lane & 31)) - 1u))] = a;
+  if ((lane & 31) == 31) slots[base + __popc(bits)] = b;
+  if ((lane & 31) == 0) words[w] = DirWord{bits, base};
+}
+
+static int dir_from_dense(Ctx* c, int64_t n, DevGrid* g) {
+  const int64_t nwords = (g->ncell >> 5) + 1;
+  PQ_TRY(c->arena.get(size_t(nwords), &g->dir_words));
+  PQ_TRY(c->arena.get(size_t(n) + size_t(nwords) + 1, &g->dir_slots));
+  hipLaunchKernelGGL(k_dir_from_dense, dim3(unsigned(ceil_div(nwords * 32, 256))), dim3(256), 0, c->stream, g->ncell,
+                     g->start, g->dir_words, g->dir_slots);
+  PQ_HIP(hipGetLastError());
+  return 0;
+}
+
+__global__ __launch_bounds__(256) void k_read_directory(int64_t ncell, const CellDir dir,
+                                                        int32_t* __restrict__ out) {
+  const int64_t c = int64_t(blockIdx.x) * 256 + threadIdx.x;
+  if (c <= ncell) out[c] = dir.begin(int(c));
+}
+
+void read_directory(Ctx* c, const DevGrid& g, int64_t ncell, int32_t* begin_out) {
+  hipLaunchKernelGGL(k_read_directory, dim3(unsigned(ceil_div(ncell + 1, 256))), dim3(256), 0, c->stream, ncell,
+                     cell_dir(g), begin_out);
 }
 
 int bin_octants_planned(Ctx* c, const double* xyz, int64_t n, double cell, const PlanHint& hint,
@@ -1699,8 +1754,8 @@
   g->ncell = hint.ncell;
   sub->zeroed4 = zeroed + 2 * kBkMax + 1;
   const int raw[3] = {0, 0, 0};
-  return enqueue_bucketed(c, xyz, n, GridParams{}, raw, AxisMap{nullptr, nullptr, nullptr}, false, hint.ncell,
-                          hint.nbk, 12, true, zeroed, d_plan, g, sub);
+  return enqueue_bucketed(c, xyz, n, GridParams{}, raw, AxisMap{nullptr, nullptr, nullptr}, false, hint.nbk, 12,
+                          true, zeroed, d_plan, g, sub);
 }
 
 static int upload_plan(Ctx* c, const GridPlan& p, GridPlan* h_up, GridPlan* d_plan) {
@@ -1738,6 +1793,7 @@
     int32_t* zeroed4 = sub->zeroed4;
     PQ_TRY(subsort_octants(c, g, n, sub));
     sub->zeroed4 = zeroed4;
+    PQ_TRY(dir_from_dense(c, n, g));
     hp.nx = g->nx;
     hp.ny = g->ny;
     hp.nz = g->nz;
@@ -1826,7 +1882,7 @@
   PQ_TRY(upload_plan(c, hp, h_up, d_plan));
   const GridParams gp = grid_params(*g);
   if (bucketed_path) {
-    PQ_TRY(enqueue_bucketed(c, xyz, n, gp, raw, am, mapped, g->ncell, nbk, bits, hp.all_f32, zeroed, d_plan, g, sub));
+    PQ_TRY(enqueue_bucketed(c, xyz, n, gp, raw, am, mapped, nbk, bits, hp.all_f32, zeroed, d_plan, g, sub));
     if (!mapped && cell == min_cell && bits == 12 && hp.all_f32) {
       int64_t ncell_h = std::min<int64_t>(g->ncell + g->ncell / 16, (int64_t(kBkMax) << 12) - 1);
       if (nbk <= kBkFusedScan) ncell_h = std::min<int64_t>(ncell_h, (int64_t(kBkFusedScan) << 12) - 1);
@@ -1872,7 +1928,7 @@
                      c->stream, big_list, big_cnt, g->start, keyed, g->order, g->cell_of, sub->sub_of,
                      g->sx, g->sy, g->sz, g->p4, sub->sub_cnt, sub->sub_beg, sub->rec, d_plan);
   PQ_HIP(hipGetLastError());
-  return 0;
+  return dir_from_dense(c, n, g);
 }
 
 
diff --git a/pyqsm_amd/csrc/grid.hpp b/pyqsm_amd/csrc/grid.hpp
--- a/pyqsm_amd/csrc/grid.hpp
+++ b/pyqsm_amd/csrc/grid.hpp
@@ -2,6 +2,26 @@
 #include "common.hpp"
 
 namespace pyqsm {
+
+struct alignas(8) DirWord {
+  uint32_t bits, base;
+};
+struct CellDir {
+  const DirWord* words;
+  const int32_t* slots;
+  __device__ __forceinline__ static int slot_of(const DirWord w, int c) {
+    return int(w.base) + __popc(w.bits & ((1u << (c & 31)) - 1u));
+  }
+  __device__ __forceinline__ int begin(int c) const { return slots[slot_of(words[c >> 5], c)]; }
+  template <int N>
+  __device__ __forceinline__ void begins(const int (&c)[N], int (&out)[N]) const {
+    DirWord w[N];
+#pragma unroll
+    for (int i = 0; i < N; ++i) w[i] = words[c[i] >> 5];
+#pragma unroll
+    for (int i = 0; i < N; ++i) out[i] = slots[slot_of(w[i], c[i])];
+  }
+};
 
 struct DevGrid {
   double minx, miny, minz;
@@ -10,6 +30,8 @@
   int nx, ny, nz;
   int64_t ncell;
   int32_t* start;
+  DirWord* dir_words = nullptr;
+  int32_t* dir_slots = nullptr;
   int32_t* order;
   int32_t* cell_of;
   double *sx, *sy, *sz;
@@ -22,6 +44,7 @@
   double minx, miny, minz, inv_cell;
   int nx, ny, nz;
 };
+inline CellDir cell_dir(const DevGrid& g) { return CellDir{g.dir_words, g.dir_slots}; }
 inline GridParams grid_params(const DevGrid& g) { return GridParams{g.minx, g.miny, g.minz, g.inv_cell, g.nx, g.ny, g.nz}; }
 
 __device__ __forceinline__ void clamped_cell(const GridParams& g, double x, double y, double z, int* cx, int* cy,
@@ -133,41 +156,49 @@
   int total;
 };
 
-__device__ __forceinline__ Tile wave_tile(int p0, int n, Stencil st, int ncell,
-                                          const int32_t* __restrict__ start,
+__device__ __forceinline__ Tile wave_tile(int p0, int n, Stencil st, int ncell, const CellDir& dir,
                                           const int32_t* __restrict__ cell_of) {
   Tile t;
   const int plast = p0 + 63 < n ? p0 + 63 : n - 1;
   const int c_first = __builtin_amdgcn_readfirstlane(cell_of[p0]);
   const int c_last = __builtin_amdgcn_readfirstlane(cell_of[plast]);
   int lo[9], hi[9];
-  int w = 0;
-  for (int dz = -1; dz <= 1; ++dz)
-    for (int dy = -1; dy <= 1; ++dy) {
-      const int o = dy * st.nx + dz * st.nxy;
-      int a = c_first + o - 1, b = c_last + o + 1;
-      a = a < 0 ? 0 : a;
-      b = b > ncell - 1 ? ncell - 1 : b;
-      int k = w++;
-      while (k > 0 && lo[k - 1] > a) {
-        lo[k] = lo[k - 1];
-        hi[k] = hi[k - 1];
-        --k;
-      }
-      lo[k] = a;
-      hi[k] = b;
+#pragma unroll
+  for (int w = 0; w < 9; ++w) {
+    const int o = (w % 3 - 1) * st.nx + (w / 3 - 1) * st.nxy;
+    const int a = c_first + o - 1, b = c_last + o + 1;
+    lo[w] = a < 0 ? 0 : a;
+    hi[w] = b > ncell - 1 ? ncell - 1 : b;
+  }
+#pragma unroll
+  for (int i = 1; i < 9; ++i)
+#pragma unroll
+    for (int k = i; k > 0; --k) {
+      const bool sw = lo[k - 1] > lo[k];
+      const int l0 = lo[k - 1], h0 = hi[k - 1];
+      lo[k - 1] = sw ? lo[k] : l0;
+      hi[k - 1] = sw ? hi[k] : h0;
+      lo[k] = sw ? l0 : lo[k];
+      hi[k] = sw ? h0 : hi[k];
     }
-  t.total = 0;
+  int cells[18], q[18];
   int prev_hi = -1;
+#pragma unroll
   for (int r = 0; r < 9; ++r) {
     const int a = lo[r] <= prev_hi ? prev_hi + 1 : lo[r];
+    cells[2 * r] = cells[2 * r + 1] = 0;
     if (a <= hi[r]) {
-      t.qb[r] = __builtin_amdgcn_readfirstlane(start[a]);
-      t.qe[r] = __builtin_amdgcn_readfirstlane(start[hi[r] + 1]);
+      cells[2 * r] = a;
+      cells[2 * r + 1] = hi[r] + 1;
       prev_hi = hi[r];
-    } else {
-      t.qb[r] = t.qe[r] = 0;
     }
+  }
+  dir.begins(cells, q);
+  t.total = 0;
+#pragma unroll
+  for (int r = 0; r < 9; ++r) {
+    t.qb[r] = __builtin_amdgcn_readfirstlane(q[2 * r]);
+    t.qe[r] = __builtin_amdgcn_readfirstlane(q[2 * r + 1]);
     t.total += t.qe[r] - t.qb[r];
   }
   return t;
@@ -215,6 +246,8 @@
                      int32_t* zeroed, GridPlan* h_up, GridPlan* d_plan, DevGrid* g, SubCells* sub,
                      PlanHint* hint_out);
 
+void read_directory(Ctx* c, const DevGrid& g, int64_t ncell, int32_t* begin_out);
+
 int coarsen_grid(Ctx* c, const DevGrid& fine, int64_t n, int factor, DevGrid* coarse);
 
 int radius_grid(Ctx* c, const double* d_src, int64_t n, double radius, DevGrid* g);
diff --git a/pyqsm_amd/hip.py b/pyqsm_amd/hip.py
--- a/pyqsm_amd/hip.py
+++ b/pyqsm_amd/hip.py
@@ -200,6 +200,15 @@
                                           int(bool(radius_inclusive)), labels_ptr, core_ptr,
                                           ctypes.byref(cnt) if want_count else None, int(device)))
     return int(cnt.value) if want_count else None
+
+
+def octant_directory(points, eps: float, device: int = 0, cap: int = 1 << 25):
+    pts = _points(points)
+    dims = np.zeros(3, dtype=np.int32)
+    begin = np.empty(int(cap), dtype=np.int32)
+    check(_lib.load().pyqsm_octant_directory(_p(pts), pts.shape[0], float(eps), _p(dims), _p(begin), int(cap),
+                                             int(device)))
+    return dims, begin[: int(np.prod(dims.astype(np.int64))) + 1].copy()
 
 
 def knn(points, k: int, exclude_self: bool = True, device: int = 0):
```

New measurement: 3252 Mpoints/s, median of 6. 1.4% higher.
